# RishWijewardhena/vision-textile-inspection

Measured on AMD Instinct MI355X. Metric: frames/sec whole-node, YOLOv8n-seg 640x640 bs=64; mask IoU vs CPU ref, higher is better.
Workload: dtype f16x2

## Files before the change

include/vti.h:

```cpp
#ifndef VTI_H
#define VTI_H

#include <stddef.h>
#include <stdint.h>

#ifdef __cplusplus
extern "C" {
#endif

typedef struct vti_ctx vti_ctx;

typedef enum {
    VTI_OK = 0,
    VTI_ERR_ARG = -1,
    VTI_ERR_STATE = -2,
    VTI_ERR_WEIGHTS = -3,
    VTI_ERR_HIP = -4,
    VTI_ERR_NOMEM = -5,
    VTI_ERR_UNSUPPORTED = -6
} vti_status;

enum { VTI_F16 = 0, VTI_F32 = 1, VTI_H2 = 2 };
enum { VTI_MASK_LOGIT = 0,
       VTI_MASK_SIGMOID = 1 };
enum { VTI_PACK_U8 = 0, VTI_PACK_BITS = 1 };
#define VTI_MASK_NATIVE 0x10
#define VTI_MASK_SLOTS_PER_FRAME 512

typedef struct {
    char scale;
    int32_t nc;
    int32_t nm;
    int32_t reg_max;
    int32_t H, W;
    int32_t max_batch;
    int32_t dtype;
} vti_desc;

typedef struct {
    char name[48];
    int32_t c1, c2, k, s, kind;
    int32_t h_in, w_in, h_out, w_out;
    int64_t macs;
    int32_t tile_h, tile_w;
    int32_t waves_n, nrep;
    int32_t lds_bytes;
    int32_t fused;
    int32_t persistent;
} vti_conv_info;

int32_t vti_create(const vti_desc* desc, vti_ctx** out);
void vti_destroy(vti_ctx* ctx);
const char* vti_last_error(const vti_ctx* ctx);

int32_t vti_num_convs(const vti_ctx* ctx);
int32_t vti_conv_at(const vti_ctx* ctx, int32_t i, vti_conv_info* out);
int32_t vti_num_anchors(const vti_ctx* ctx);
int64_t vti_fused_params(const vti_ctx* ctx);
int64_t vti_macs_per_frame(const vti_ctx* ctx);
int64_t vti_workspace_bytes(const vti_ctx* ctx);
int32_t vti_num_launches(const vti_ctx* ctx);

int32_t vti_load_weights(vti_ctx* ctx, const void* host_blob, size_t nbytes, int32_t device);
int32_t vti_set_workspace(vti_ctx* ctx, void* dev_ws, size_t nbytes);

int32_t vti_letterbox(vti_ctx* ctx, const uint8_t* dev_frames, int32_t B, int32_t H0, int32_t W0,
                      uint8_t* dev_input, void* stream);
int32_t vti_forward(vti_ctx* ctx, const uint8_t* dev_input, int32_t B, int32_t swap_rb,
                    float* dev_pred, void* dev_proto, void* stream);
int32_t vti_nms(vti_ctx* ctx, const float* dev_pred, int32_t B, float conf, double iou,
                int32_t max_det, int32_t agnostic, float* dev_dets, int32_t* dev_counts, void* stream);
int32_t vti_forward_scored(vti_ctx* ctx, const uint8_t* dev_input, int32_t B, int32_t swap_rb,
                           float* dev_pred, void* dev_proto, float* dev_anchor_best, void* stream);
int32_t vti_nms_scored(vti_ctx* ctx, const float* dev_pred, const float* dev_anchor_best, int32_t B, float conf, double iou,
                       int32_t max_det, int32_t agnostic, float* dev_dets, int32_t* dev_counts, void* stream);
int32_t vti_masks(vti_ctx* ctx, const float* dev_dets, const int32_t* dev_counts, const void* dev_proto,
                  int32_t B, int32_t max_det, int32_t mode, int32_t packing,
                  uint8_t* dev_masks, int32_t capacity, int32_t* dev_offsets, void* stream);
int32_t vti_masks_native(vti_ctx* ctx, const float* dev_dets, const float* dev_xyxy, const int32_t* dev_counts,
                         const void* dev_proto, int32_t B, int32_t max_det, int32_t H0, int32_t W0, int32_t mode,
                         int32_t packing, uint8_t* dev_masks, int32_t capacity, int32_t* dev_offsets, void* stream);
int32_t vti_mask_native_layout(const vti_ctx* ctx, int32_t H0, int32_t W0, int32_t packing, int32_t out[6]);
int32_t vti_scale_boxes(vti_ctx* ctx, const float* dev_dets, const int32_t* dev_counts, int32_t B,
                        int32_t max_det, int32_t H0, int32_t W0, float* dev_xyxy, void* stream);
int32_t vti_predict(vti_ctx* ctx, const uint8_t* dev_frames, int32_t B, int32_t H0, int32_t W0,
                    int32_t swap_rb, float conf, double iou, int32_t max_det, int32_t agnostic,
                    int32_t mask_mode, int32_t packing, uint8_t* dev_input_scratch,
                    float* dev_pred, void* dev_proto, float* dev_dets, int32_t* dev_counts,
                    uint8_t* dev_masks, int32_t capacity, int32_t* dev_offsets, float* dev_xyxy,
                    void* stream);

int32_t vti_mask_to_frame(vti_ctx* ctx, const uint8_t* dev_masks, int32_t n, int32_t H, int32_t W,
                          int32_t H0, int32_t W0, uint8_t* dev_bitmaps, int32_t* dev_nonzero, void* stream);
int32_t vti_union_envelope(vti_ctx* ctx, const uint8_t* dev_bitmaps, const int32_t* dev_select, int32_t nsel,
                           int32_t H0, int32_t W0, uint8_t* dev_union, int32_t* dev_envelope, void* stream);
int32_t vti_mask_stats(vti_ctx* ctx, const uint8_t* dev_bitmaps, int32_t n, int32_t H0, int32_t W0,
                       int64_t* dev_stats, void* stream);

int32_t vti_mask_stats_bits(vti_ctx* ctx, const uint8_t* dev_masks_bits, int32_t n, const int32_t* dev_n_live,
                            int32_t H, int32_t W, int32_t H0, int32_t W0, int64_t* dev_stats, void* stream);
int32_t vti_envelope_bits(vti_ctx* ctx, const uint8_t* dev_masks_bits, const int32_t* dev_offsets, const float* dev_dets,
// ... 85 lines not shown
enum { VTI_POLY_OK = 0,
       VTI_POLY_ERR_BOUND = 1,
       VTI_POLY_ERR_RANGE = 2 };
int64_t vti_mask_polygons_scratch_bytes(const vti_ctx* ctx, int32_t H, int32_t W, int32_t row_bytes);
int32_t vti_mask_polygons(vti_ctx* ctx, const uint8_t* dev_masks_bits, int32_t n, const int32_t* dev_n_live, int32_t H, int32_t W,
                          int32_t row_bytes, int32_t H0, int32_t W0, int32_t strategy, void* dev_scratch, size_t scratch_bytes,
                          int32_t* dev_point_offsets, float* dev_points, int64_t max_points, void* stream);

enum { VTI_ANNOTATE_OUTLINE_SKIPPED = 1 };
int64_t vti_annotate_scratch_bytes(const vti_ctx* ctx, int32_t n_sel, int32_t max_det, int32_t H0, int32_t W0, int32_t max_points);
int32_t vti_annotate(vti_ctx* ctx, const uint8_t* dev_frames, int32_t B, int32_t H0, int32_t W0, const void* dev_cameras,
                     int32_t n_cams, const int32_t* dev_camera_of_frame, const uint8_t* dev_masks, int32_t native,
                     const float* dev_dets, const float* dev_xyxy, const int32_t* dev_counts, const int32_t* dev_offsets,
                     int32_t max_det, int32_t capacity, const int32_t* frame_i32, const double* stitch_f64, const int32_t* stitch_i32,
                     const int32_t* host_select, const int32_t* dev_select, int32_t n_sel, int32_t max_points, uint8_t* dev_out,
                     int32_t* dev_status, void* dev_scratch, size_t scratch_bytes, void* stream);
int64_t vti_annotate_frames_scratch_bytes(const vti_ctx* ctx, const void* host_out_table, int32_t max_det, int32_t max_points);
int32_t vti_annotate_frames(vti_ctx* ctx, const uint8_t* dev_frames, const void* host_table, const void* dev_table, int32_t B,
                            const void* dev_cameras, int32_t n_cams, const int32_t* dev_camera_of_frame, const uint8_t* dev_masks,
                            int32_t native, const float* dev_dets, const float* dev_xyxy, const int32_t* dev_counts,
                            const int32_t* dev_offsets, int32_t max_det, int32_t capacity, const int32_t* frame_i32,
                            const double* stitch_f64, const int32_t* stitch_i32, const int32_t* host_select, const int32_t* dev_select,
                            int32_t n_sel, int32_t max_points, const void* host_out_table, const void* dev_out_table, uint8_t* dev_out,
                            int32_t* dev_status, void* dev_scratch, size_t scratch_bytes, void* stream);

int64_t vti_encode_jpeg_scratch_bytes(const vti_ctx* ctx, int32_t n, int32_t H0, int32_t W0);
int64_t vti_encode_jpeg_max_bytes(int32_t n, int32_t H0, int32_t W0);
int32_t vti_encode_jpeg(vti_ctx* ctx, const uint8_t* dev_frames, int32_t n, int32_t H0, int32_t W0, int32_t rgb, int32_t quality,
                        void* dev_scratch, size_t scratch_bytes, int64_t* dev_byte_offsets, uint8_t* dev_out, int64_t max_bytes,
                        void* stream);
int64_t vti_encode_jpeg_frames_scratch_bytes(const vti_ctx* ctx, const void* host_table);
int64_t vti_encode_jpeg_frames_max_bytes(const void* host_table);
int32_t vti_encode_jpeg_frames(vti_ctx* ctx, const uint8_t* dev_frames, const void* host_table, const void* dev_table, int32_t n,
                               int32_t rgb, int32_t quality, void* dev_scratch, size_t scratch_bytes, int64_t* dev_byte_offsets,
                               uint8_t* dev_out, int64_t max_bytes, void* stream);

int64_t vti_decode_jpeg_table_bytes(int32_t n);
int32_t vti_decode_jpeg_plan(vti_ctx* ctx, const uint8_t* host_files, const int64_t* host_file_offsets, int32_t n,
                             int32_t segment_bytes, int32_t layout, void* host_table, size_t nbytes, int32_t* out_H0,
                             int32_t* out_W0, int64_t* out_byte_offsets, int64_t* out_scratch_bytes);
enum { VTI_JPEG_CORRUPT = 1 };
int32_t vti_decode_jpeg(vti_ctx* ctx, const uint8_t* dev_files, const void* host_table, const void* dev_table, int32_t n, int32_t rgb,
                        uint8_t* dev_out, int64_t out_bytes, int32_t* dev_info, void* dev_scratch, size_t scratch_bytes, void* stream);

int32_t vti_debug_conv_output(vti_ctx* ctx, int32_t i, int32_t B, float* dev_out, void* stream);

int32_t vti_debug_conv2d(int32_t dtype, const void* dev_in, int32_t B, int32_t H, int32_t W, int32_t in_ld,
                         int32_t in_coff, int32_t c1, const float* host_w, const float* host_b, int32_t c2,
                         int32_t k, int32_t s, int32_t kind, const void* dev_res, int32_t res_ld, int32_t res_coff,
                         void* dev_out, int32_t out_ld, int32_t out_coff, int32_t out_f32, int32_t swap_rb,
                         int32_t tile_h, int32_t tile_w, int32_t waves_n, int32_t nrep, int32_t iters,
                         float* ms_out, int32_t* cfg_out, void* stream);

#ifdef __cplusplus
}
#endif
#endif
```

vision-textile-inspection_amd/_lib.py:

```python
import ctypes as C
import os

_HERE = os.path.dirname(os.path.abspath(__file__))
_VARIANT = os.environ.get("VTI_LIB_VARIANT", "")
LIB_PATH = os.path.join(_HERE, f"libvti_{_VARIANT}.so" if _VARIANT else "libvti.so")

VTI_F16, VTI_F32, VTI_H2 = 0, 1, 2
VTI_MASK_LOGIT, VTI_MASK_SIGMOID = 0, 1
VTI_PACK_U8, VTI_PACK_BITS = 0, 1
VTI_MASK_NATIVE = 0x10


class VtiDesc(C.Structure):
    _fields_ = [("scale", C.c_char), ("nc", C.c_int32), ("nm", C.c_int32), ("reg_max", C.c_int32),
                ("H", C.c_int32), ("W", C.c_int32), ("max_batch", C.c_int32), ("dtype", C.c_int32)]


class VtiConvInfo(C.Structure):
    _fields_ = [("name", C.c_char * 48), ("c1", C.c_int32), ("c2", C.c_int32), ("k", C.c_int32),
                ("s", C.c_int32), ("kind", C.c_int32), ("h_in", C.c_int32), ("w_in", C.c_int32),
                ("h_out", C.c_int32), ("w_out", C.c_int32), ("macs", C.c_int64),
                ("tile_h", C.c_int32), ("tile_w", C.c_int32), ("waves_n", C.c_int32), ("nrep", C.c_int32),
                ("lds_bytes", C.c_int32), ("fused", C.c_int32), ("persistent", C.c_int32)]


class VtiMeasureParams(C.Structure):
    _fields_ = [("K", C.c_double * 9), ("dist", C.c_double * 5), ("R", C.c_double * 9), ("t", C.c_double * 3),
                ("max_px_distance", C.c_double), ("two_row_threshold_px", C.c_double),
                ("stitch_id", C.c_int32), ("fabric_id", C.c_int32), ("roi_enabled", C.c_int32), ("roi", C.c_int32 * 4),
                ("min_stitches", C.c_int32), ("envelope_neighborhood", C.c_int32), ("skip_cluster", C.c_int32),
                ("kmeans_iters", C.c_int32), ("drop_empty", C.c_int32), ("frame_buffer", C.c_int32)]


VTI_MEASURE_OK, VTI_MEASURE_NO_FABRIC, VTI_MEASURE_NO_STITCHES, VTI_MEASURE_BAD_CAMERA = 0, 1, 2, 3
VTI_STITCH_KEPT, VTI_STITCH_MASK, VTI_STITCH_SELECTED, VTI_STITCH_NEAR, VTI_STITCH_DIST, VTI_STITCH_WIDTH = 1, 2, 4, 8, 16, 32
VTI_MEASURE_MAX_DET = 1000

VTI_POLY_LARGEST, VTI_POLY_CONCAT = 0, 1
VTI_POLY_OK, VTI_POLY_ERR_BOUND, VTI_POLY_ERR_RANGE = 0, 1, 2
VTI_ANNOTATE_OUTLINE_SKIPPED = 1
VTI_JPEG_CORRUPT = 1
VTI_ERR_ARG, VTI_ERR_UNSUPPORTED = -1, -6


class VtiError(RuntimeError):

    def __init__(self, code, msg):
        super().__init__(f"libvti error {code}: {msg}")
        self.code = code


_P, _I32, _I64, _F, _D, _SZ = C.c_void_p, C.c_int32, C.c_int64, C.c_float, C.c_double, C.c_size_t

SIGNATURES = {
    "vti_create": (_I32, [C.POINTER(VtiDesc), C.POINTER(_P)]),
    "vti_destroy": (None, [_P]),
    "vti_last_error": (C.c_char_p, [_P]),
    "vti_num_convs": (_I32, [_P]),
    "vti_conv_at": (_I32, [_P, _I32, C.POINTER(VtiConvInfo)]),
    "vti_num_anchors": (_I32, [_P]),
    "vti_fused_params": (_I64, [_P]),
    "vti_macs_per_frame": (_I64, [_P]),
    "vti_workspace_bytes": (_I64, [_P]),
    "vti_num_launches": (_I32, [_P]),
    "vti_load_weights": (_I32, [_P, _P, _SZ, _I32]),
    "vti_set_workspace": (_I32, [_P, _P, _SZ]),
    "vti_letterbox": (_I32, [_P, _P, _I32, _I32, _I32, _P, _P]),
    "vti_forward": (_I32, [_P, _P, _I32, _I32, _P, _P, _P]),
    "vti_nms": (_I32, [_P, _P, _I32, _F, _D, _I32, _I32, _P, _P, _P]),
    "vti_forward_scored": (_I32, [_P, _P, _I32, _I32, _P, _P, _P, _P]),
    "vti_nms_scored": (_I32, [_P, _P, _P, _I32, _F, _D, _I32, _I32, _P, _P, _P]),
    "vti_masks": (_I32, [_P, _P, _P, _P, _I32, _I32, _I32, _I32, _P, _I32, _P, _P]),
    "vti_masks_native": (_I32, [_P, _P, _P, _P, _P, _I32, _I32, _I32, _I32, _I32, _I32, _P, _I32, _P, _P]),
    "vti_mask_native_layout": (_I32, [_P, _I32, _I32, _I32, C.POINTER(_I32)]),
    "vti_scale_boxes": (_I32, [_P, _P, _P, _I32, _I32, _I32, _I32, _P, _P]),
    "vti_predict": (_I32, [_P, _P, _I32, _I32, _I32, _I32, _F, _D, _I32, _I32, _I32, _I32,
                           _P, _P, _P, _P, _P, _P, _I32, _P, _P, _P]),
    "vti_mask_to_frame": (_I32, [_P, _P, _I32, _I32, _I32, _I32, _I32, _P, _P, _P]),
    "vti_union_envelope": (_I32, [_P, _P, _P, _I32, _I32, _I32, _P, _P, _P]),
    "vti_mask_stats": (_I32, [_P, _P, _I32, _I32, _I32, _P, _P]),
    "vti_mask_stats_bits": (_I32, [_P, _P, _I32, _P, _I32, _I32, _I32, _I32, _P, _P]),
    "vti_envelope_bits": (_I32, [_P, _P, _P, _P, _I32, _I32, _I32, _I32, _I32, _I32, _P, _P]),
    "vti_pixels_to_world": (_I32, [_P, _P, _I32, _P, _P, _P, _P, _P, _P, _P]),
    "vti_kmeans1d2": (_I32, [_P, _P, _P, _I32, _I32, _I32, _P, _P, _P]),
    "vti_measure_scratch_bytes": (_I64, [_P, _I32, _I32, _I32]),
    "vti_measure": (_I32, [_P, C.POINTER(VtiMeasureParams), _P, _I32, _P, _P, _P, _P, _I32, _I32, _I32, _I32, _I32, _P, _SZ,
                           _P, _P, _P, _P, _P]),
    "vti_measure_cameras_bytes": (_I64, [_I32]),
    "vti_measure_pack_cameras": (_I32, [_P, C.POINTER(VtiMeasureParams), _I32, _P, _SZ]),
    "vti_measure_cameras": (_I32, [_P, _P, _I32, _P, _P, _I32, _P, _P, _P, _P, _I32, _I32, _I32, _I32, _I32, _P, _SZ,
                                   _P, _P, _P, _P, _P]),
    "vti_frame_table_bytes": (_I64, [_I32]),
    "vti_pack_frames": (_I32, [_P, _I32, _I32, _P, _P, _P, _I32, _I64, _P, _SZ]),
    "vti_frame_table_info": (_I32, [_P, _I32, _P, _P]),
    "vti_letterbox_frames": (_I32, [_P, _P, _P, _P, _I32, _P, _P]),
    "vti_scale_boxes_frames": (_I32, [_P, _P, _P, _P, _P, _I32, _I32, _P, _P]),
    "vti_predict_frames": (_I32, [_P, _P, _P, _P, _I32, _I32, _F, _D, _I32, _I32, _I32, _I32,
                                  _P, _P, _P, _P, _P, _P, _I32, _P, _P, _P]),
    "vti_measure_frames": (_I32, [_P, _P, _I32, _P, _P, _I32, _P, _P, _P, _P, _P, _P, _I32, _I32, _I32, _P, _SZ,
                                  _P, _P, _P, _P, _P]),
    "vti_mask_native_frames_bytes": (_I64, [_P, _P, _I32]),
    "vti_masks_native_frames": (_I32, [_P, _P, _P, _P, _P, _P, _P, _I32, _I32, _I32, _I32, _P, _I64, _P, _P, _P]),
    "vti_predict_frames_native": (_I32, [_P, _P, _P, _P, _I32, _I32, _F, _D, _I32, _I32, _I32, _I32,
                                         _P, _P, _P, _P, _P, _P, _I64, _P, _P, _P, _P]),
    "vti_measure_frames_native": (_I32, [_P, _P, _I32, _P, _P, _P, _I64, _P, _P, _P, _P, _P, _P, _I32, _I32, _I32, _P, _SZ,
                                         _P, _P, _P, _P, _P]),
    "vti_mask_polygons_scratch_bytes": (_I64, [_P, _I32, _I32, _I32]),
    "vti_mask_polygons": (_I32, [_P, _P, _I32, _P, _I32, _I32, _I32, _I32, _I32, _I32, _P, _SZ, _P, _P, _I64, _P]),
    "vti_annotate_scratch_bytes": (_I64, [_P, _I32, _I32, _I32, _I32, _I32]),
    "vti_annotate": (_I32, [_P, _P, _I32, _I32, _I32, _P, _I32, _P, _P, _I32, _P, _P, _P, _P, _I32, _I32, _P, _P, _P, _P, _P, _I32,
                            _I32, _P, _P, _P, _SZ, _P]),
    "vti_annotate_frames_scratch_bytes": (_I64, [_P, _P, _I32, _I32]),
    "vti_annotate_frames": (_I32, [_P, _P, _P, _P, _I32, _P, _I32, _P, _P, _I32, _P, _P, _P, _P, _I32, _I32, _P, _P, _P, _P, _P, _I32,
                                   _I32, _P, _P, _P, _P, _P, _SZ, _P]),
    "vti_encode_jpeg_scratch_bytes": (_I64, [_P, _I32, _I32, _I32]),
    "vti_encode_jpeg_max_bytes": (_I64, [_I32, _I32, _I32]),
    "vti_encode_jpeg": (_I32, [_P, _P, _I32, _I32, _I32, _I32, _I32, _P, _SZ, _P, _P, _I64, _P]),
    "vti_encode_jpeg_frames_scratch_bytes": (_I64, [_P, _P]),
    "vti_encode_jpeg_frames_max_bytes": (_I64, [_P]),
    "vti_encode_jpeg_frames": (_I32, [_P, _P, _P, _P, _I32, _I32, _I32, _P, _SZ, _P, _P, _I64, _P]),
    "vti_decode_jpeg_table_bytes": (_I64, [_I32]),
    "vti_decode_jpeg_plan": (_I32, [_P, _P, _P, _I32, _I32, _I32, _P, _SZ, _P, _P, _P, _P]),
    "vti_decode_jpeg": (_I32, [_P, _P, _P, _P, _I32, _I32, _P, _I64, _P, _P, _SZ, _P]),
    "vti_debug_conv_output": (_I32, [_P, _I32, _I32, _P, _P]),
    "vti_debug_conv2d": (_I32, [_I32, _P, _I32, _I32, _I32, _I32, _I32, _I32, _P, _P, _I32, _I32, _I32, _I32,
                                _P, _I32, _I32, _P, _I32, _I32, _I32, _I32, _I32, _I32, _I32, _I32, _I32,
                                _P, _P, _P]),
}

_lib = None


def lib():
    global _lib
    if _lib is None:
        if not os.path.exists(LIB_PATH):
            raise ImportError(f"{LIB_PATH} not found: build it with `python -c 'import __graft_entry__ as g; "
                              f"g.build()'` (hipcc --offload-arch=gfx950); there is no CPU fallback")
        L = C.CDLL(LIB_PATH)
        for name, (res, args) in SIGNATURES.items():
            fn = getattr(L, name)
            fn.restype, fn.argtypes = res, args
        _lib = L
    return _lib


def check(ctx, rc):
    if rc != 0:
        msg = lib().vti_last_error(ctx)
        raise VtiError(rc, msg.decode() if msg else "")
```

vision-textile-inspection_amd/api.py:

```python
from ._lib import LIB_PATH, SIGNATURES, VtiError, lib
from .engine import Engine, FrameTable, debug_conv2d, h2_decode, h2_encode, kmeans1d2, pixels_to_world, unpack_bits
from .feeder import FrameFeeder
from .model import YOLO, Boxes, Masks, Results, letterbox_shape
from .weights import pack_container, random_weights, unpack_container
from .convert import convert_checkpoint, convert_state_dict
from .measure import MeasureParams, MultiCameraMeasurer, StitchMeasurer
from . import annotate, consumer, dataparallel, jpeg

__all__ = ["LIB_PATH", "SIGNATURES", "VtiError", "lib", "Engine", "FrameTable", "debug_conv2d", "h2_decode", "h2_encode", "kmeans1d2", "pixels_to_world", "unpack_bits", "FrameFeeder", "YOLO", "Boxes", "Masks",
           "Results", "letterbox_shape", "pack_container", "random_weights", "unpack_container", "convert_checkpoint", "convert_state_dict",
           "MeasureParams", "MultiCameraMeasurer", "StitchMeasurer", "annotate", "consumer", "dataparallel", "jpeg"]
```

vision-textile-inspection_amd/csrc/conv.hip:

```cpp
#include <algorithm>
#include <cstdlib>
#include <type_traits>

#include "conv_dev.h"

namespace vti {

__host__ __device__ inline int patch_dim(int t, int ks, int s, int mode) { return mode == 1 ? t : (t - 1) * s + ks; }

size_t stem_lds_bytes(int TH, int TW);

size_t conv_lds_bytes(int ks, int stride, int mode, int TH, int TW, int WN, int NREP) {
    if (mode == 1) return stem_lds_bytes(TH, TW);
    const int npix = patch_dim(TH, ks, stride, mode) * patch_dim(TW, ks, stride, mode);
    const size_t plane = (size_t)((npix + 15) & ~15) * 16;
    const int taps = mode == 1 ? 1 : ks * ks;
    size_t raw = 0;
    if (mode == 1) raw = (((size_t)(2 * TH + 1) * (2 * TW + 1) * 3) + 15) & ~(size_t)15;
    return 4 * plane + (size_t)WN * NREP * taps * 1024 + raw;
}

template <typename T, int KS, int S, int NREP, int WN, int NREP2 = 0, int NT = 256>
__global__ __launch_bounds__(NT, NT == 512 ? 1 : 2) void conv_kernel(const ConvParams p) {
    using vec = typename Tr<T>::vec;
    constexpr int VEC = Tr<T>::VEC, KC = Tr<T>::KC;
    constexpr int TAPS = KS * KS, PAD = KS / 2;
    constexpr int NTB = WN * NREP;
    constexpr int PP = NT / 4;
    constexpr int AR = NT == 512 ? 6 : (S == 2 ? 12 : 8);
    constexpr int BR = (NTB * TAPS * 64 + NT - 1) / NT;
    constexpr unsigned OOB = 0xFFFFFFFFu;
    extern __shared__ __attribute__((aligned(16))) char smem[];

    const int tid = threadIdx.x, lane = tid & 63, wave = tid >> 6;
    const int wn = wave % WN, wm = wave / WN;
    int t = blockIdx.x;
    const int tx = t % p.tiles_x; t /= p.tiles_x;
    const int ty = t % p.tiles_y;
    const int b = t / p.tiles_y;
    const int oy0 = ty * p.TH, ox0 = tx * p.TW;
    const int PH = (p.TH - 1) * S + KS, PW = (p.TW - 1) * S + KS;
    const int npix = PH * PW;
    const int plane_bytes = ((npix + 15) & ~15) * 16;
    char* smA = smem;
    char* smB = smem + 4 * plane_bytes;
    const int nt0 = blockIdx.y * NTB;
    const int tile_px = p.TH * p.TW;
    VTI_STAMP(0);

    int abase[MREP], opy[MREP], opx[MREP];
    bool pvalid[MREP];
#pragma unroll
    for (int m = 0; m < MREP; ++m) {
        const int pp = (wm * MREP + m) * 16 + (lane & 15);
        const bool v = pp < tile_px;
        const int pc = v ? pp : 0;
        const int py = (int)__umulhi((unsigned)pc, p.tw_magic), px = pc - py * p.TW;
        opy[m] = oy0 + py; opx[m] = ox0 + px;
        pvalid[m] = v && opy[m] < p.Hout && opx[m] < p.Wout;
        abase[m] = (lane >> 4) * plane_bytes + ((py * S) * PW + px * S) * 16;
    }

    f32x4 acc[MREP][NREP];
#pragma unroll
    for (int m = 0; m < MREP; ++m)
#pragma unroll
        for (int n = 0; n < NREP; ++n) acc[m][n] = (f32x4){0.f, 0.f, 0.f, 0.f};

    const size_t frame_elems = (size_t)p.Hin * p.Win * p.in_ld;
    const __amdgpu_buffer_rsrc_t rsA = __builtin_amdgcn_make_buffer_rsrc(
        (void*)((const T*)p.in + (size_t)b * frame_elems), 0, (int)(frame_elems * sizeof(T)), 0x00020000);
    const __amdgpu_buffer_rsrc_t rsB = __builtin_amdgcn_make_buffer_rsrc((void*)p.wpk, 0, (int)p.wpk_bytes, 0x00020000);

    const int iy0 = oy0 * S - PAD, ix0 = ox0 * S - PAD;
    const int q = (tid >> 3) & 3;
    const int pix0 = (tid >> 5) * 8 + (tid & 7);
    const int ldsA0 = q * plane_bytes + pix0 * 16;
    const int cvalid = (p.Cin - q * VEC + KC - 1) / KC;
    unsigned aoff[AR];
#pragma unroll
    for (int u = 0; u < AR; ++u) {
        const int pix = pix0 + PP * u;
        const int py = (int)__umulhi((unsigned)pix, p.pw_magic), px = pix - py * PW;
        const int y = iy0 + py, x = ix0 + px;
        const bool ok = pix < npix && (unsigned)y < (unsigned)p.Hin && (unsigned)x < (unsigned)p.Win;
        aoff[u] = ok ? (unsigned)(((y * p.Win + x) * p.in_ld + p.in_coff + q * VEC) * (int)sizeof(T)) : OOB;
    }
    constexpr bool BPRE = NREP < 5 || NT == 512;
    constexpr int PD = (KS == 1 && BPRE) ? 2 : 1;
    vec ra[PD][AR], rb[PD][BR];
    auto loadB = [&](int c, vec (&rbs)[BR]) {
        const unsigned sB = (unsigned)(((size_t)c * p.ntiles_n + nt0) * (TAPS * 1024));
#pragma unroll
        for (int u = 0; u < BR; ++u)
            if (tid + u * NT < NTB * TAPS * 64) rbs[u] = buf_load16<vec>(rsB, (unsigned)(tid + u * NT) * 16u, sB);
    };
    auto issue = [&](int c, vec (&ras)[AR], vec (&rbs)[BR]) {
        const bool qok = c < cvalid;
#pragma unroll
        for (int u = 0; u < AR; ++u)
            if (pix0 + PP * u < ((npix + 7) & ~7))
                ras[u] = buf_load16<vec>(rsA, qok ? aoff[u] : OOB, (unsigned)(c * KC * (int)sizeof(T)));
        if constexpr (BPRE) loadB(c, rbs);
    };
    auto commit = [&](int c, vec (&ras)[AR], vec (&rbs)[BR]) {
        if constexpr (!BPRE) loadB(c, rbs);
#pragma unroll
        for (int u = 0; u < AR; ++u)
            if (pix0 + PP * u < npix) *(vec*)(smA + ldsA0 + u * (PP * 16)) = ras[u];
#pragma unroll
        for (int u = 0; u < BR; ++u)
            if (tid + u * NT < NTB * TAPS * 64) *(vec*)(smB + (tid + u * NT) * 16) = rbs[u];
    };
    auto chunk = [&](int c, auto set_c) {
        constexpr int SET = decltype(set_c)::value;
        if (c < 2) VTI_STAMP(1 + 5 * c);
        commit(c, ra[SET], rb[SET]);
        if (c < 2) VTI_STAMP(3 + 5 * c);
        __syncthreads();
        if (c < 2) VTI_STAMP(4 + 5 * c);
        if (c + PD < p.nchunks) issue(c + PD, ra[SET], rb[SET]);
        {
            constexpr int NSTEP = TAPS * MREP;
            constexpr int XD = NREP >= 5 ? 2 : 3;
            constexpr int WD = NREP >= 5 ? 1 : 2;
            vec xq[XD];
            vec wq[WD][NREP];
            auto ldx = [&](int s_) -> vec {
                const int tp = s_ / MREP, mm = s_ % MREP;
                const int toff = ((tp / KS) * PW + (tp % KS)) * 16;
                return *(const vec*)(smA + abase[mm] + toff);
            };
            auto ldw = [&](int tp, vec (&w)[NREP]) {
#pragma unroll
                for (int n = 0; n < NREP; ++n)
                    w[n] = *(const vec*)(smB + ((wn * NREP + n) * TAPS + tp) * 1024 + lane * 16);
            };
            if constexpr (Tr<T>::H2 && TAPS > 1 && (NREP <= 3 || (NREP == 4 && NT == 512))) {
                auto ldw1 = [&](int tp, int n) -> vec { return *(const vec*)(smB + ((wn * NREP + n) * TAPS + tp) * 1024 + lane * 16); };
                h2_taps<NREP, MREP, TAPS, 3>(acc, ldx, ldw1);
            } else {
            ldw(0, wq[0]);
            xq[0] = ldx(0);
            if (XD > 2 && NSTEP > 1) xq[1] = ldx(1);
#pragma unroll
            for (int s_ = 0; s_ < NSTEP; ++s_) {
                const int tp = s_ / MREP, mm = s_ % MREP;
                if (s_ + XD - 1 < NSTEP) xq[(s_ + XD - 1) % XD] = ldx(s_ + XD - 1);
                if (WD == 2 && mm == 0 && tp + 1 < TAPS) ldw(tp + 1, wq[(tp + 1) % WD]);
                __builtin_amdgcn_sched_barrier(0);
#pragma unroll
                for (int n = 0; n < NREP; ++n) acc[mm][n] = mma(wq[tp % WD][n], xq[s_ % XD], acc[mm][n]);
                __builtin_amdgcn_sched_barrier(0);
                if (WD == 1 && mm == MREP - 1 && tp + 1 < TAPS) ldw(tp + 1, wq[0]);
            }
            }
        }
        if (c < 2) VTI_STAMP(5 + 5 * c);
        if (c + 1 < p.nchunks) __syncthreads();
    };

    issue(0, ra[0], rb[0]);
    if constexpr (PD == 2) {
        if (p.nchunks > 1) issue(1, ra[1], rb[1]);
        for (int c = 0; c < p.nchunks; c += 2) {
            chunk(c, std::integral_constant<int, 0>{});
            if (c + 1 < p.nchunks) chunk(c + 1, std::integral_constant<int, 1>{});
        }
    } else {
        for (int c = 0; c < p.nchunks; ++c) chunk(c, std::integral_constant<int, 0>{});
    }

    VTI_STAMP(11);
    if constexpr (NREP2 == 0) {
        conv_epilogue<T, NREP>(p, acc, pvalid, opy, opx, b, nt0, wn, lane);
    } else {
        static_assert(WN == 1, "fused stage needs the whole Cout in one wave");
        conv_stage2<T, NREP, NREP2>(p, acc, pvalid, opy, opx, b, lane);
    }
    VTI_STAMP(12);
}

size_t convfold_lds_bytes(int TH, int TW) {
    const int npix = (TH + 2) * (TW + 2);
    return 4 * (size_t)((npix + 15) & ~15) * 16 + (size_t)16 * 4 * 1024;
}
bool convfold_supported(int c_in, int c_mid, int c_out, int ntiles2) {
    return c_in == c_mid && c_mid % 16 == 0 && c_out == 64 && c_in % 16 == 0 && c_in <= 64 && combo_has(FoldN2{}, ntiles2);
}

template <typename T, int NREP2, int NT = 256>
__global__ __launch_bounds__(NT, NT == 512 ? 1 : 2) void convfold_kernel(const ConvParams p) {
    using vec = typename Tr<T>::vec;
    constexpr int VEC = Tr<T>::VEC, KC = Tr<T>::KC;
    constexpr int NREP = 4, TAPS = 4, NTB = 16, AR = 8;
    constexpr int BR = NTB * TAPS * 64 / NT;
    constexpr int PPP = NT / 4;
    constexpr unsigned OOB = 0xFFFFFFFFu;
    extern __shared__ __attribute__((aligned(16))) char smem[];

    const int tid = threadIdx.x, lane = tid & 63, wave = (tid >> 6) & 3, mgrp = tid >> 8;
    const int py = wave >> 1, px = wave & 1;
    int t = blockIdx.x;
    const int tx = t % p.tiles_x; t /= p.tiles_x;
    const int ty = t % p.tiles_y;
    const int b = t / p.tiles_y;
    const int oy0 = ty * p.TH, ox0 = tx * p.TW;
    const int PH = p.TH + 2, PW = p.TW + 2;
    const int npix = PH * PW;
    const int plane_bytes = ((npix + 15) & ~15) * 16;
    char* smA = smem;
    char* smB = smem + 4 * plane_bytes;
    const int tile_px = p.TH * p.TW;

    int abase[MREP], opy[MREP], opx[MREP];
    bool pvalid[MREP];
#pragma unroll
    for (int m = 0; m < MREP; ++m) {
        const int pp = (mgrp * MREP + m) * 16 + (lane & 15);
        const bool v = pp < tile_px;
        const int pc = v ? pp : 0;
        const int ly = (int)__umulhi((unsigned)pc, p.tw_magic), lx = pc - ly * p.TW;
        pvalid[m] = v && oy0 + ly < p.Hout && ox0 + lx < p.Wout;
        opy[m] = 2 * (oy0 + ly) + py; opx[m] = 2 * (ox0 + lx) + px;
        abase[m] = (lane >> 4) * plane_bytes + ((ly + py) * PW + lx + px) * 16;
    }
    f32x4 acc[MREP][NREP];
#pragma unroll
    for (int m = 0; m < MREP; ++m)
#pragma unroll
        for (int n = 0; n < NREP; ++n) acc[m][n] = (f32x4){0.f, 0.f, 0.f, 0.f};
// ... 424 lines not shown
        const int pp = (wave * MREP + m) * 16 + (lane & 15);
        const int py = pp / SL_TW, px = pp - py * SL_TW;
        opy[m] = oy0 + py; opx[m] = ox0 + px;
        pvalid[m] = opy[m] < p.Hout && opx[m] < p.Wout;
        sbase[m] = ((2 * py) * SL_SW + 2 * px) * 16 * ES;
    }
    f32x4 acc[MREP][2];
#pragma unroll
    for (int m = 0; m < MREP; ++m) { acc[m][0] = (f32x4){0.f, 0.f, 0.f, 0.f}; acc[m][1] = (f32x4){0.f, 0.f, 0.f, 0.f}; }
#pragma unroll
    for (int s = 0; s < NS1; ++s) {
        const int tap = sizeof(T) == 2 ? 2 * s + (g >> 1) : s;
        const int tc = tap < 9 ? tap : 8;
        const int toff = ((tc / 3) * SL_SW + (tc % 3)) * 16 * ES + (sizeof(T) == 2 ? (g & 1) * 8 : g * 4) * ES;
        vec w1[2];
#pragma unroll
        for (int n = 0; n < 2; ++n) w1[n] = w1all[s][n];
#pragma unroll
        for (int m = 0; m < MREP; ++m) {
            const vec x = *(const vec*)(sout + sbase[m] + toff);
#pragma unroll
            for (int n = 0; n < 2; ++n) acc[m][n] = mma(w1[n], x, acc[m][n]);
        }
    }
    VTI_STAMP(3);
    if (p.out2) conv_stage2<T, 2, 2, false, true>(p, acc, pvalid, opy, opx, b, lane, &s2r);
    else conv_epilogue<T, 2>(p, acc, pvalid, opy, opx, b, 0, 0, lane);
    VTI_STAMP(12);
    }
}

void stem_l1_tile(int* th, int* tw) { *th = SL_TH; *tw = SL_TW; }

int stem_l1_grid(int dtype, int ntiles) {
    const int wgpc = (int)std::min<size_t>(2, (160 * 1024) / stem_l1_lds_bytes(dtype));
    const char* np = getenv("VTI_STEM_NOT_PERSISTENT");
    if (np && np[0] == '1') return ntiles;
    return std::min(ntiles, 256 * std::max(1, wgpc));
}

hipError_t launch_stem_l1(int dtype, const ConvParams& p, hipStream_t st) {
    dim3 grid((unsigned)stem_l1_grid(dtype, p.B * p.tiles_y * p.tiles_x));
    if (grid.x == 0) return hipSuccess;
    const size_t lds = stem_l1_lds_bytes(dtype);
    return with_conv_type(dtype, [&](auto t) { return launch_lds<stem_l1_kernel<typename decltype(t)::type>>(grid, dim3(256), lds, st, p); });
}

size_t stem_lds_bytes(int TH, int TW) { return 1024 + (size_t)(2 * TH + 1) * ((((2 * TW + 1) * 3 + 6) >> 2) * 4); }

using ConvTile3 = Combos<Ints<1, 1>, Ints<2, 1>, Ints<3, 1>, Ints<4, 1>, Ints<5, 1>, Ints<1, 2>, Ints<2, 2>, Ints<1, 4>>;
using ConvTile1 = decltype(concat(ConvTile3{}, Combos<Ints<3, 2>, Ints<4, 2>, Ints<5, 2>, Ints<2, 4>, Ints<3, 4>, Ints<4, 4>, Ints<5, 4>>{}));
using StemNrep = Combos<Ints<1>, Ints<2>, Ints<3>, Ints<4>, Ints<5>>;

bool conv_cfg_fits(int ks, int stride, int mode, int TH, int TW, int WN, int NREP, int threads) {
    if (mode == 1) return WN == 1 && (2 * TH + 1) * (((2 * TW + 1) * 3 + 6) >> 2) < 65536;
    if (threads != 256 && !(threads == 512 && ks == 3 && stride == 1 && WN == 1)) return false;
    const int AR = threads == 512 ? 6 : (stride == 2 ? 12 : 8);
    const int npix = patch_dim(TH, ks, stride, mode) * patch_dim(TW, ks, stride, mode);
    if (((npix + 7) / 8) * 32 > threads * AR) return false;
    return ks == 1 ? combo_has(ConvTile1{}, NREP, WN) : combo_has(ConvTile3{}, NREP, WN);
}

bool conv_fusable(int nrep, int nrep2) { return combo_has(FusedPairs{}, nrep, nrep2); }

template <typename T, int KS, int S>
static hipError_t launch_ks(int nrep, const ConvParams& p, dim3 grid, size_t lds, hipStream_t st) {
    return combo_dispatch(std::conditional_t<KS == 1, ConvTile1, ConvTile3>{}, [&](auto c) {
        using C = decltype(c);
        return launch_lds<conv_kernel<T, KS, S, C::v[0], C::v[1]>>(grid, dim3(256), lds, st, p);
    }, nrep, p.WN);
}

template <typename T>
static hipError_t launch_t(int ks, int stride, int nrep, int mode, const ConvParams& p, dim3 grid, size_t lds,
                           hipStream_t st) {
    if (p.ntiles2 > 0) {
        if (!(ks == 3 && stride == 1 && p.WN == 1 && mode == 0)) return hipErrorInvalidValue;
        return combo_dispatch(FusedPairs{}, [&](auto c) {
            using C = decltype(c);
            return p.nt == 512 ? launch_lds<conv_kernel<T, 3, 1, C::v[0], 1, C::v[1], 512>>(grid, dim3(512), lds, st, p)
                               : launch_lds<conv_kernel<T, 3, 1, C::v[0], 1, C::v[1]>>(grid, dim3(256), lds, st, p);
        }, nrep, p.ntiles2);
    }
    if (mode == 1)
        return combo_dispatch(StemNrep{}, [&](auto c) {
            hipLaunchKernelGGL((stem_kernel<T, decltype(c)::v[0]>), grid, dim3(256), lds, st, p);
            return hipGetLastError();
        }, nrep);
    if (ks == 1 && stride == 1) return launch_ks<T, 1, 1>(nrep, p, grid, lds, st);
    if (ks == 3 && stride == 1) return launch_ks<T, 3, 1>(nrep, p, grid, lds, st);
    if (ks == 3 && stride == 2) return launch_ks<T, 3, 2>(nrep, p, grid, lds, st);
    return hipErrorInvalidValue;
}

hipError_t launch_conv(int dtype, int ks, int stride, int nrep, int mode, const ConvParams& p, size_t lds_bytes,
                       hipStream_t st) {
    if (p.pk == 4) return launch_conv_pk2(dtype, nrep, p, lds_bytes, st);
    if (p.pk == 3) return launch_bneck_pk(dtype, nrep, p, lds_bytes, st);
    if (p.pk == 2) return launch_conv1_pk(dtype, nrep, p, lds_bytes, st);
    if (p.pk) return launch_conv_pk(dtype, nrep, p, lds_bytes, st);
    const int NTB = p.WN * nrep;
    dim3 grid((unsigned)(p.B * p.tiles_y * p.tiles_x), (unsigned)((p.ntiles_n + NTB - 1) / NTB));
    if (grid.x == 0) return hipSuccess;
    const int nwaves = p.nt == 512 ? 8 : 4;
    if ((p.nt != 256 && p.nt != 512) || (p.nt == 512 && p.ntiles2 == 0)) return hipErrorInvalidValue;
    if (p.TH * p.TW > (nwaves / p.WN) * MREP * 16 || (p.WN != 1 && p.WN != 2 && p.WN != 4)) return hipErrorInvalidValue;
    return with_conv_type(dtype, [&](auto t) { return launch_t<typename decltype(t)::type>(ks, stride, nrep, mode, p, grid, lds_bytes, st); });
}

}
```

vision-textile-inspection_amd/csrc/conv_dev.h:

```cpp
#pragma once
#include "vti_internal.h"

namespace vti {

typedef _Float16 half_t;
typedef _Float16 half8 __attribute__((ext_vector_type(8)));
typedef _Float16 half4 __attribute__((ext_vector_type(4)));
typedef float f32x4 __attribute__((ext_vector_type(4)));

typedef unsigned u32x4 __attribute__((ext_vector_type(4)));

struct h2_t { unsigned u; };
struct h2x4 { u32x4 u; };
constexpr float H2_SX = 16.0f;

template <typename T> struct Tr;
template <> struct Tr<half_t> { typedef half8 vec; static constexpr int VEC = 8, KC = 32; static constexpr bool H16 = true, F32 = false, H2 = false; };
template <> struct Tr<float> { typedef f32x4 vec; static constexpr int VEC = 4, KC = 16; static constexpr bool H16 = false, F32 = true, H2 = false; };
template <> struct Tr<h2_t> { typedef h2x4 vec; static constexpr int VEC = 4, KC = 16; static constexpr bool H16 = false, F32 = false, H2 = true; };

typedef _Float16 half2v __attribute__((ext_vector_type(2)));
__device__ __forceinline__ unsigned h2_enc(float v) {
    half2v p;
    p[0] = (half_t)__builtin_fmaf(v, H2_SX, 0.0f);
// ... 3 lines not shown
__device__ __forceinline__ float h2_dec(unsigned u) {
    const half2v p = __builtin_bit_cast(half2v, u);
    return ((float)p[0] + (float)p[1]) * (1.0f / H2_SX);
}
template <typename T> __device__ __forceinline__ T to_T(float v) {
    if constexpr (Tr<T>::H2) return h2_t{h2_enc(v)};
    else return (T)v;
}
template <typename T> __device__ __forceinline__ void vset(typename Tr<T>::vec& x, int j, T e) {
    if constexpr (Tr<T>::H2) x.u[j] = e.u;
    else x[j] = e;
}
template <typename T> __device__ __forceinline__ u32x4 pack4(f32x4 v) {
    if constexpr (Tr<T>::H2) return (u32x4){h2_enc(v[0]), h2_enc(v[1]), h2_enc(v[2]), h2_enc(v[3])};
    else return __builtin_bit_cast(u32x4, v);
}
template <typename T> __device__ __forceinline__ f32x4 unpack4(u32x4 u) {
    if constexpr (Tr<T>::H2) return (f32x4){h2_dec(u[0]), h2_dec(u[1]), h2_dec(u[2]), h2_dec(u[3])};
    else return __builtin_bit_cast(f32x4, u);
}
template <typename T> __device__ __forceinline__ f32x4 acc_bias(f32x4 acc, f32x4 bias, float alpha) {
    if constexpr (Tr<T>::H2) return acc * (f32x4){alpha, alpha, alpha, alpha} + bias;
    else return acc + bias;
}

__device__ __forceinline__ f32x4 mma(half8 w, half8 x, f32x4 c) {
    return __builtin_amdgcn_mfma_f32_16x16x32_f16(w, x, c, 0, 0, 0);
}
__device__ __forceinline__ f32x4 mma(f32x4 w, f32x4 x, f32x4 c) {
    c = __builtin_amdgcn_mfma_f32_16x16x4f32(w[0], x[0], c, 0, 0, 0);
    c = __builtin_amdgcn_mfma_f32_16x16x4f32(w[1], x[1], c, 0, 0, 0);
    c = __builtin_amdgcn_mfma_f32_16x16x4f32(w[2], x[2], c, 0, 0, 0);
    c = __builtin_amdgcn_mfma_f32_16x16x4f32(w[3], x[3], c, 0, 0, 0);
    return c;
}

__device__ __forceinline__ f32x4 mma(h2x4 w, h2x4 x, f32x4 c) {
    u32x4 wh, wl;
#pragma unroll
    for (int i = 0; i < 4; ++i) {
        wh[i] = __builtin_amdgcn_perm(w.u[i], w.u[i], 0x01000100u);
        wl[i] = w.u[i] >> 16;
    }
    const half8 xv = __builtin_bit_cast(half8, x.u);
    c = __builtin_amdgcn_mfma_f32_16x16x32_f16(__builtin_bit_cast(half8, wh), xv, c, 0, 0, 0);
    c = __builtin_amdgcn_mfma_f32_16x16x32_f16(__builtin_bit_cast(half8, wl), xv, c, 0, 0, 0);
    return c;
}

template <int NREP, int M, int TAPS, int XD, class LDX, class LDW>
__device__ __forceinline__ void h2_taps(f32x4 (&acc)[M][NREP], LDX ldx, LDW ldw) {
    constexpr int NSTEP = TAPS * M;
    constexpr unsigned SEL_H = 0x01000100u;
    h2x4 xq[XD];
    u32x4 wraw[NREP];
    u32x4 wh[2][NREP], wl[2][NREP];
#pragma unroll
    for (int n = 0; n < NREP; ++n) wraw[n] = ldw(0, n).u;
#pragma unroll
    for (int i = 0; i < XD - 1; ++i) xq[i] = ldx(i);
#pragma unroll
    for (int n = 0; n < NREP; ++n)
#pragma unroll
        for (int i = 0; i < 4; ++i) {
            wh[0][n][i] = __builtin_amdgcn_perm(wraw[n][i], wraw[n][i], SEL_H);
            wl[0][n][i] = wraw[n][i] >> 16;
        }
#pragma unroll
    for (int s_ = 0; s_ < NSTEP; ++s_) {
        const int tp = s_ / M, mm = s_ % M, cur = tp & 1, nxt = cur ^ 1;
#ifdef H2_EXP_NOXREAD
        if (s_ + XD - 1 < NSTEP && s_ < XD) xq[(s_ + XD - 1) % XD] = ldx(s_ + XD - 1);
#else
        if (s_ + XD - 1 < NSTEP) xq[(s_ + XD - 1) % XD] = ldx(s_ + XD - 1);
#endif
        if (mm == 0 && tp + 1 < TAPS) {
#pragma unroll
            for (int n = 0; n < NREP; ++n) wraw[n] = ldw(tp + 1, n).u;
        }
        __builtin_amdgcn_sched_barrier(0);
        const half8 xv = __builtin_bit_cast(half8, xq[s_ % XD].u);
#pragma unroll
        for (int j = 0; j < 2 * NREP; ++j) {
            const int n = j >> 1;
#ifdef H2_EXP_SKIP
            if (!((j & 1) && (tp & 1)))
#endif
            acc[mm][n] = __builtin_amdgcn_mfma_f32_16x16x32_f16(__builtin_bit_cast(half8, (j & 1) ? wl[cur][n] : wh[cur][n]), xv, acc[mm][n], 0, 0, 0);
            const int k = (mm - 1) * 2 * NREP + j;
#ifdef H2_EXP_NOPERM
            if (mm == 1 && j == 0 && tp + 1 < TAPS) {
#pragma unroll
                for (int n2 = 0; n2 < NREP; ++n2) { wh[nxt][n2] = wraw[n2]; wl[nxt][n2] = wraw[n2]; }
            }
            if (false) {
#else
            if (mm >= 1 && k < 8 * NREP && tp + 1 < TAPS) {
#endif
                const int pn = k >> 3, r = k & 7, i = r & 3;
                if (r < 4) wh[nxt][pn][i] = __builtin_amdgcn_perm(wraw[pn][i], wraw[pn][i], SEL_H);
                else wl[nxt][pn][i] = wraw[pn][i] >> 16;
                __builtin_amdgcn_sched_group_barrier(0x008, 1, 0);
                __builtin_amdgcn_sched_group_barrier(0x002, 1, 0);
            }
        }
        __builtin_amdgcn_sched_barrier(0);
    }
}

template <int NREP, int M, int TAPS, class LDX, class LDW>
__device__ __forceinline__ void h2_taps_nmajor(f32x4 (&acc)[M][NREP], LDX ldx, LDW ldw) {
    constexpr int NU = TAPS * NREP;
    h2x4 x[2][M];
    u32x4 wraw[2], wh[2], wl[2];
#pragma unroll
    for (int m = 0; m < M; ++m) x[0][m] = ldx(m);
    wraw[0] = ldw(0, 0).u;
    if (NU > 1) wraw[1] = ldw(1 / NREP, 1 % NREP).u;
#pragma unroll
    for (int i = 0; i < 4; ++i) { wh[0][i] = __builtin_amdgcn_perm(wraw[0][i], wraw[0][i], 0x01000100u); wl[0][i] = wraw[0][i] >> 16; }
#pragma unroll
    for (int u = 0; u < NU; ++u) {
        const int tp = u / NREP, n = u % NREP, cur = u & 1, nxt = cur ^ 1;
        if (n == NREP - 1 && tp + 1 < TAPS) {
#pragma unroll
            for (int m = 0; m < M; ++m) x[(tp + 1) & 1][m] = ldx((tp + 1) * M + m);
        }
        const u32x4 wnext = wraw[nxt];
        if (u + 2 < NU) wraw[cur] = ldw((u + 2) / NREP, (u + 2) % NREP).u;
        __builtin_amdgcn_sched_barrier(0);
#pragma unroll
        for (int j = 0; j < 2 * M; ++j) {
            const int m = j >> 1;
            acc[m][n] = __builtin_amdgcn_mfma_f32_16x16x32_f16(__builtin_bit_cast(half8, (j & 1) ? wl[cur] : wh[cur]),
                                                               __builtin_bit_cast(half8, x[tp & 1][m].u), acc[m][n], 0, 0, 0);
            if (j < 8 && u + 1 < NU) {
                const int i = j & 3;
                if (j < 4) wh[nxt][i] = __builtin_amdgcn_perm(wnext[i], wnext[i], 0x01000100u);
                else wl[nxt][i] = wnext[i] >> 16;
                __builtin_amdgcn_sched_group_barrier(0x008, 1, 0);
                __builtin_amdgcn_sched_group_barrier(0x002, 1, 0);
            }
        }
        __builtin_amdgcn_sched_barrier(0);
    }
}

template <bool FAST> __device__ __forceinline__ float silu(float x) {
    if constexpr (FAST) return x * __builtin_amdgcn_rcpf(1.0f + __builtin_amdgcn_exp2f(x * -1.4426950408889634f));
    else return x / (1.0f + expf(-x));
}

template <bool FAST> __device__ __forceinline__ f32x4 silu4(f32x4 x) {
    if constexpr (FAST) {
        const f32x4 y = x * (f32x4){-1.4426950408889634f, -1.4426950408889634f, -1.4426950408889634f, -1.4426950408889634f};
        f32x4 e;
#pragma unroll
        for (int j = 0; j < 4; ++j) e[j] = __builtin_amdgcn_exp2f(y[j]);
        e = e + (f32x4){1.0f, 1.0f, 1.0f, 1.0f};
#pragma unroll
        for (int j = 0; j < 4; ++j) e[j] = __builtin_amdgcn_rcpf(e[j]);
        return x * e;
    } else {
        f32x4 r;
#pragma unroll
        for (int j = 0; j < 4; ++j) r[j] = silu<false>(x[j]);
        return r;
    }
}

constexpr int MREP = 5;

#ifdef VTI_STAMPS
#define VTI_STAMP(i)                                                                              \
    do {                                                                                          \
        if (p.stamps && tid == 0) {                                                               \
            unsigned long long t_;                                                                \
            asm volatile("s_memtime %0\n\ts_waitcnt lgkmcnt(0)" : "=s"(t_)::"memory");            \
            p.stamps[(size_t)(blockIdx.y * gridDim.x + blockIdx.x) * 16 + (i)] = t_;              \
            if ((i) == 0 || (i) == 12) {                                                          \
                asm volatile("s_memrealtime %0\n\ts_waitcnt lgkmcnt(0)" : "=s"(t_)::"memory");    \
                p.stamps[(size_t)(blockIdx.y * gridDim.x + blockIdx.x) * 16 + ((i) == 0 ? 14 : 15)] = t_; \
            }                                                                                     \
        }                                                                                         \
    } while (0)
#else
#define VTI_STAMP(i) do { } while (0)
#endif

template <typename T, int NREP>
__device__ __forceinline__ void conv_epilogue(const ConvParams& p, f32x4 (&acc)[MREP][NREP], const bool (&pvalid)[MREP],
                                              const int (&opy)[MREP], const int (&opx)[MREP], int b, int nt0, int wn,
                                              int lane) {
    constexpr bool FAST = !Tr<T>::F32;
    const int crun = (nt0 + wn * NREP) * 16 + (lane >> 4) * 4 * NREP;
    f32x4 bias_r[NREP];
#pragma unroll
    for (int n = 0; n < NREP; ++n) {
        const int cb = crun + 4 * n < p.ntiles_n * 16 ? crun + 4 * n : 0;
        bias_r[n] = *(const f32x4*)(p.bias + cb);
    }
    if (!p.scalar_store && !p.out_f32 && !p.deconv_c) {
        const bool has_res = __builtin_amdgcn_readfirstlane(p.has_res) != 0;
#pragma unroll
        for (int m = 0; m < MREP; ++m) {
            if (!pvalid[m]) continue;
            const size_t opix = ((size_t)(b * p.Hout + opy[m])) * p.Wout + opx[m];
            T* op = (T*)p.out + opix * p.out_ld + p.out_coff + crun;
            f32x4 res_r[NREP];
            if (has_res) {
                const T* rp = (const T*)p.res + opix * p.res_ld + p.res_coff + crun;
#pragma unroll
                for (int n = 0; n < NREP; ++n) {
                    res_r[n] = (f32x4){0.f, 0.f, 0.f, 0.f};
                    if (crun + 4 * n < p.Cout) {
                        if constexpr (sizeof(T) == 2) {
                            const half4 r = *(const half4*)(rp + 4 * n);
#pragma unroll
                            for (int j = 0; j < 4; ++j) res_r[n][j] = (float)r[j];
                        } else {
                            res_r[n] = unpack4<T>(*(const u32x4*)(rp + 4 * n));
                        }
                    }
                }
            }
            f32x4 v[NREP];
#pragma unroll
            for (int n = 0; n < NREP; ++n) {
                v[n] = acc_bias<T>(acc[m][n], bias_r[n], p.alpha);
                if (p.act) v[n] = silu4<FAST>(v[n]);
                if (has_res) v[n] += res_r[n];
            }
            if constexpr (sizeof(T) == 2) {
                if constexpr (NREP % 2 == 0) {
#pragma unroll
                    for (int n = 0; n < NREP; n += 2) {
                        if (crun + 4 * n + 8 <= p.Cout) {
                            half8 hv;
#pragma unroll
                            for (int j = 0; j < 4; ++j) { hv[j] = (half_t)v[n][j]; hv[4 + j] = (half_t)v[n + 1][j]; }
                            *(half8*)(op + 4 * n) = hv;
                        } else if (crun + 4 * n + 4 <= p.Cout) {
                            half4 hv;
#pragma unroll
                            for (int j = 0; j < 4; ++j) hv[j] = (half_t)v[n][j];
                            *(half4*)(op + 4 * n) = hv;
                        }
                    }
                } else {
#pragma unroll
                    for (int n = 0; n < NREP; ++n) {
                        if (crun + 4 * n >= p.Cout) continue;
                        half4 hv;
#pragma unroll
                        for (int j = 0; j < 4; ++j) hv[j] = (half_t)v[n][j];
                        *(half4*)(op + 4 * n) = hv;
                    }
                }
            } else {
#pragma unroll
                for (int n = 0; n < NREP; ++n)
                    if (crun + 4 * n < p.Cout) *(u32x4*)(op + 4 * n) = pack4<T>(v[n]);
            }
        }
        return;
    }
    if constexpr (sizeof(T) == 2 && NREP % 2 == 0) {
        if (p.deconv_c && !p.scalar_store && !p.out_f32 && !p.has_res) {
            const int qd = crun / p.deconv_c, co = crun - qd * p.deconv_c;
#pragma unroll
            for (int m = 0; m < MREP; ++m) {
                if (!pvalid[m] || crun >= p.Cout) continue;
                const size_t opix = ((size_t)(b * 2 * p.Hout + 2 * opy[m] + (qd >> 1))) * (2 * p.Wout) + 2 * opx[m] + (qd & 1);
                T* op = (T*)p.out + opix * p.out_ld + p.out_coff + co;
#pragma unroll
                for (int n = 0; n < NREP; n += 2) {
                    half8 hv;
#pragma unroll
                    for (int j = 0; j < 4; ++j) {
                        float a0 = acc[m][n][j] + bias_r[n][j], a1 = acc[m][n + 1][j] + bias_r[n + 1][j];
                        if (p.act) { a0 = silu<FAST>(a0); a1 = silu<FAST>(a1); }
                        hv[j] = (half_t)a0; hv[4 + j] = (half_t)a1;
                    }
                    *(half8*)(op + 4 * n) = hv;
                }
            }
            return;
        }
    }
#pragma unroll
    for (int m = 0; m < MREP; ++m) {
        if (!pvalid[m]) continue;
#pragma unroll
        for (int n = 0; n < NREP; ++n) {
            const int cout0 = crun + 4 * n;
            if (cout0 >= p.Cout) continue;
            f32x4 v = acc_bias<T>(acc[m][n], bias_r[n], p.alpha);
            if (p.act) v = silu4<FAST>(v);
            size_t opix;
            int co = cout0;
            if (p.deconv_c) {
                const int q = cout0 / p.deconv_c;
                co = cout0 - q * p.deconv_c;
                opix = ((size_t)(b * 2 * p.Hout + 2 * opy[m] + (q >> 1))) * (2 * p.Wout) + 2 * opx[m] + (q & 1);
            } else {
                opix = ((size_t)(b * p.Hout + opy[m])) * p.Wout + opx[m];
            }
            if (p.has_res) {
                const T* rp = (const T*)p.res + opix * p.res_ld + p.res_coff + co;
                if constexpr (sizeof(T) == 2) {
                    const half4 r = *(const half4*)rp;
#pragma unroll
                    for (int j = 0; j < 4; ++j) v[j] += (float)r[j];
                } else {
                    v += unpack4<T>(*(const u32x4*)rp);
                }
            }
            const size_t o = opix * p.out_ld + p.out_coff + co;
            if (p.scalar_store) {
#pragma unroll
                for (int j = 0; j < 4; ++j) {
                    if (cout0 + j < p.Cout) {
                        if (p.out_f32) ((float*)p.out)[o + j] = v[j];
                        else if constexpr (Tr<T>::H2) ((unsigned*)p.out)[o + j] = h2_enc(v[j]);
                        else ((T*)p.out)[o + j] = (T)v[j];
                    }
                }
            } else if (p.out_f32 || Tr<T>::F32) {
                *(f32x4*)((float*)p.out + o) = v;
            } else if constexpr (Tr<T>::H2) {
                *(u32x4*)((unsigned*)p.out + o) = pack4<T>(v);
            } else {
                half4 hv;
#pragma unroll
                for (int j = 0; j < 4; ++j) hv[j] = (half_t)v[j];
                *(half4*)((half_t*)p.out + o) = hv;
            }
        }
    }
}

template <typename V> __device__ __forceinline__ V buf_load16(__amdgpu_buffer_rsrc_t r, unsigned voff, unsigned soff) {
    const u32x4 v = __builtin_amdgcn_raw_buffer_load_b128(r, voff, soff, 0);
    return __builtin_bit_cast(V, v);
}

template <typename T, int NREP, int NREP2> struct Stage2Regs {
    using vec = typename Tr<T>::vec;
    static constexpr int KT = sizeof(T) == 2 ? (NREP + 1) / 2 : NREP;
    vec w2[KT][NREP2];
    f32x4 bias1[NREP];
    f32x4 bias2[NREP2];
};

template <typename T, int NREP, int NREP2>
__device__ __forceinline__ void stage2_preload(const ConvParams& p, int lane, bool fold, Stage2Regs<T, NREP, NREP2>& r) {
    using vec = typename Tr<T>::vec;
    const __amdgpu_buffer_rsrc_t rsW2 = __builtin_amdgcn_make_buffer_rsrc(
        (void*)p.w2, 0, (int)(Stage2Regs<T, NREP, NREP2>::KT * p.ntiles2 * 1024), 0x00020000);
#pragma unroll
    for (int t2 = 0; t2 < Stage2Regs<T, NREP, NREP2>::KT; ++t2)
#pragma unroll
        for (int n = 0; n < NREP2; ++n) r.w2[t2][n] = buf_load16<vec>(rsW2, (unsigned)(((t2 * p.ntiles2 + n) * 64 + lane) * 16), 0u);
    const float* b1 = p.bias + (fold ? 4 * (16 * NREP) : 0) + (lane >> 4) * 4 * NREP;
#pragma unroll
    for (int n = 0; n < NREP; ++n) r.bias1[n] = *(const f32x4*)(b1 + 4 * n);
    const int crun2 = p.nat2 ? (lane >> 4) * 4 : (lane >> 4) * 4 * NREP2, cstep2 = p.nat2 ? 16 : 4;
#pragma unroll
    for (int n = 0; n < NREP2; ++n) r.bias2[n] = *(const f32x4*)(p.bias2 + crun2 + cstep2 * n);
}

template <typename T, int NREP, int NREP2, bool FOLD = false, bool PRE = false>
__device__ __forceinline__ void conv_stage2(const ConvParams& p, f32x4 (&acc)[MREP][NREP], const bool (&pvalid)[MREP],
                                            const int (&opy)[MREP], const int (&opx)[MREP], int b, int lane,
                                            const Stage2Regs<T, NREP, NREP2>* pre = nullptr, bool interior = false) {
    const int OW = FOLD ? 2 * p.Wout : p.Wout;
    using vec = typename Tr<T>::vec;
    constexpr bool FAST = !Tr<T>::F32;
    constexpr int KT = sizeof(T) == 2 ? (NREP + 1) / 2 : NREP;
    const __amdgpu_buffer_rsrc_t rsW2 = __builtin_amdgcn_make_buffer_rsrc(
        (void*)p.w2, 0, (int)(KT * p.ntiles2 * 1024), 0x00020000);
    f32x4 bias1[FOLD ? MREP : 1][NREP];
    if (PRE && (!FOLD || interior)) {
#pragma unroll
        for (int m = 0; m < (FOLD ? MREP : 1); ++m)
#pragma unroll
            for (int n = 0; n < NREP; ++n) bias1[m][n] = pre->bias1[n];
    } else if constexpr (FOLD) {
#pragma unroll
        for (int m = 0; m < MREP; ++m) {
            const int cy = opy[m] == 0 ? 0 : (opy[m] == 2 * p.Hout - 1 ? 2 : 1), cx = opx[m] == 0 ? 0 : (opx[m] == OW - 1 ? 2 : 1);
            const float* bt = p.bias + (cy * 3 + cx) * (16 * NREP) + (lane >> 4) * 4 * NREP;
#pragma unroll
            for (int n = 0; n < NREP; ++n) bias1[m][n] = *(const f32x4*)(bt + 4 * n);
        }
    } else {
#pragma unroll
        for (int n = 0; n < NREP; ++n) bias1[0][n] = *(const f32x4*)(p.bias + (lane >> 4) * 4 * NREP + 4 * n);
    }
    f32x4 acc2[MREP][NREP2];
#pragma unroll
    for (int m = 0; m < MREP; ++m)
#pragma unroll
        for (int n = 0; n < NREP2; ++n) acc2[m][n] = (f32x4){0.f, 0.f, 0.f, 0.f};
#pragma unroll
    for (int t2 = 0; t2 < KT; ++t2) {
        vec w2[NREP2];
#pragma unroll
        for (int n = 0; n < NREP2; ++n) {
            if constexpr (PRE) w2[n] = pre->w2[t2][n];
            else w2[n] = buf_load16<vec>(rsW2, (unsigned)(((t2 * p.ntiles2 + n) * 64 + lane) * 16), 0u);
        }
#pragma unroll
        for (int m = 0; m < MREP; ++m) {
            vec x;
            if constexpr (sizeof(T) == 2) {
#pragma unroll
                for (int h = 0; h < 2; ++h) {
                    const int n1 = 2 * t2 + h;
                    f32x4 v = {0.f, 0.f, 0.f, 0.f};
                    if (n1 < NREP) {
                        v = acc_bias<T>(acc[m][n1 < NREP ? n1 : 0], bias1[FOLD ? m : 0][n1 < NREP ? n1 : 0], p.alpha);
                        if (p.act) v = silu4<FAST>(v);
                    }
#pragma unroll
                    for (int j = 0; j < 4; ++j) x[h * 4 + j] = (T)v[j];
                }
            } else {
                f32x4 v = acc_bias<T>(acc[m][t2], bias1[FOLD ? m : 0][t2], p.alpha);
                if (p.act) v = silu4<FAST>(v);
                if constexpr (Tr<T>::H2) x.u = pack4<T>(v);
                else {
#pragma unroll
                    for (int j = 0; j < 4; ++j) x[j] = v[j];
                }
            }
#pragma unroll
            for (int n = 0; n < NREP2; ++n) acc2[m][n] = mma(w2[n], x, acc2[m][n]);
        }
    }
    [[maybe_unused]] const int tid = threadIdx.x;
    VTI_STAMP(13);
    f32x4 bias2[NREP2];
    const int crun2 = p.nat2 ? (lane >> 4) * 4 : (lane >> 4) * 4 * NREP2;
    const int cstep2 = p.nat2 ? 16 : 4;
#pragma unroll
    for (int n = 0; n < NREP2; ++n) {
        if constexpr (PRE) bias2[n] = pre->bias2[n];
        else bias2[n] = *(const f32x4*)(p.bias2 + crun2 + cstep2 * n);
    }
    if constexpr (NREP2 == 4) {
        if (p.act2 == 3) {
            const int g = lane >> 4;
#pragma unroll
            for (int m = 0; m < MREP; ++m) {
                float d4[4];
#pragma unroll
                for (int n = 0; n < 4; ++n) {
                    const f32x4 v = acc_bias<T>(acc2[m][n], bias2[n], p.alpha2);
                    float mx = fmaxf(fmaxf(v[0], v[1]), fmaxf(v[2], v[3]));
                    mx = fmaxf(mx, __shfl_xor(mx, 16));
                    mx = fmaxf(mx, __shfl_xor(mx, 32));
                    float e[4];
#pragma unroll
                    for (int j = 0; j < 4; ++j) {
                        if constexpr (FAST) e[j] = __builtin_amdgcn_exp2f((v[j] - mx) * 1.4426950408889634f);
                        else e[j] = expf(v[j] - mx);
                    }
                    float s = (e[0] + e[1]) + (e[2] + e[3]);
                    float w = (e[0] * (float)(4 * g) + e[1] * (float)(4 * g + 1)) + (e[2] * (float)(4 * g + 2) + e[3] * (float)(4 * g + 3));
                    s += __shfl_xor(s, 16); w += __shfl_xor(w, 16);
                    s += __shfl_xor(s, 32); w += __shfl_xor(w, 32);
                    d4[n] = w / s;
                }
                const float ax = (float)opx[m] + 0.5f, ay = (float)opy[m] + 0.5f;
                const float x1 = ax - d4[0], y1 = ay - d4[1], x2 = ax + d4[2], y2 = ay + d4[3];
                const float comp = g == 0 ? ((x1 + x2) / 2.0f) * p.dfl_stride : g == 1 ? ((y1 + y2) / 2.0f) * p.dfl_stride
                                 : g == 2 ? (x2 - x1) * p.dfl_stride : (y2 - y1) * p.dfl_stride;
                if (pvalid[m])
                    ((float*)p.out2)[((size_t)b * p.out2_bstride + (size_t)opy[m] * OW + opx[m]) * p.out2_ld + p.out2_coff + g] = comp;
            }
            return;
        }
    }
    if constexpr (sizeof(T) == 2 && NREP2 % 2 == 0) {
        if (!p.nat2 && !p.out2_f32 && !p.scalar_store2 && (p.Cout2 & 7) == 0 && ((p.out2_ld | p.out2_coff) & 7) == 0) {
#pragma unroll
            for (int m = 0; m < MREP; ++m) {
                if (!pvalid[m]) continue;
                half_t* op = (half_t*)p.out2 + ((size_t)b * p.out2_bstride + (size_t)opy[m] * OW + opx[m]) * p.out2_ld + p.out2_coff + crun2;
#pragma unroll
                for (int n = 0; n < NREP2; n += 2) {
                    if (crun2 + 4 * n >= p.Cout2) continue;
                    f32x4 v0 = acc_bias<T>(acc2[m][n], bias2[n], p.alpha2), v1 = acc_bias<T>(acc2[m][n + 1], bias2[n + 1], p.alpha2);
                    if (p.act2 == 1) { v0 = silu4<FAST>(v0); v1 = silu4<FAST>(v1); }
                    half8 hv;
#pragma unroll
                    for (int j = 0; j < 4; ++j) { hv[j] = (half_t)v0[j]; hv[4 + j] = (half_t)v1[j]; }
                    *(half8*)(op + 4 * n) = hv;
                }
            }
            return;
        }
    }
    const bool want_best = p.act2 == 2 && p.best != nullptr;
#pragma unroll
    for (int m = 0; m < MREP; ++m) {
        const size_t pix = (size_t)b * p.out2_bstride + (size_t)opy[m] * OW + opx[m];
        const size_t o0 = pix * p.out2_ld + p.out2_coff;
        float bv = -INFINITY;
        int bc = 0x7fffffff;
        if (!want_best && !pvalid[m]) continue;
#pragma unroll
        for (int n = 0; n < NREP2; ++n) {
            const int cout0 = crun2 + cstep2 * n;
            if (cout0 >= p.Cout2) continue;
            f32x4 v = acc_bias<T>(acc2[m][n], bias2[n], p.alpha2);
            if (p.act2 == 1) v = silu4<FAST>(v);
            else if (p.act2 == 2) {
#pragma unroll
                for (int j = 0; j < 4; ++j) {
                    if constexpr (FAST) v[j] = __builtin_amdgcn_rcpf(1.0f + __builtin_amdgcn_exp2f(v[j] * -1.4426950408889634f));
                    else v[j] = 1.0f / (1.0f + expf(-v[j]));
                }
                if (want_best) {
                    if ((p.Cout2 & 3) == 0) {
#pragma unroll
                        for (int j = 0; j < 4; ++j)
                            if (v[j] > bv) { bv = v[j]; bc = cout0 + j; }
                    } else {
#pragma unroll
                        for (int j = 0; j < 4; ++j)
                            if (cout0 + j < p.Cout2 && v[j] > bv) { bv = v[j]; bc = cout0 + j; }
                    }
                }
            }
            if (!pvalid[m]) continue;
            const size_t o = o0 + cout0;
            if (p.scalar_store2) {
#pragma unroll
                for (int j = 0; j < 4; ++j) {
                    if (cout0 + j < p.Cout2) {
                        if (p.out2_f32) ((float*)p.out2)[o + j] = v[j];
                        else if constexpr (Tr<T>::H2) ((unsigned*)p.out2)[o + j] = h2_enc(v[j]);
                        else ((T*)p.out2)[o + j] = (T)v[j];
                    }
                }
            } else if (p.out2_f32 || Tr<T>::F32) {
                *(f32x4*)((float*)p.out2 + o) = v;
            } else if constexpr (Tr<T>::H2) {
                *(u32x4*)((unsigned*)p.out2 + o) = pack4<T>(v);
            } else {
                half4 hv;
#pragma unroll
                for (int j = 0; j < 4; ++j) hv[j] = (half_t)v[j];
                *(half4*)((half_t*)p.out2 + o) = hv;
            }
        }
        if (want_best) {
#pragma unroll
// ... 34 lines not shown
```

vision-textile-inspection_amd/csrc/plan.cpp:

```cpp
#include <algorithm>
#include <cmath>
#include <cstdio>
#include <cstdlib>
#include <cstring>

#include "vti_internal.h"

namespace vti {

namespace {

struct Scale { char tag; double depth, width; int maxc; };
const Scale kScales[] = {{'n', 0.33, 0.25, 1024}, {'s', 0.33, 0.50, 1024}, {'m', 0.67, 0.75, 768},
                         {'l', 1.00, 1.00, 512},  {'x', 1.00, 1.25, 512}};

int make_divisible(double x, int d) { return (int)std::ceil(x / d) * d; }
int py_round(double x) { return (int)std::nearbyint(x); }

struct Builder {
    Plan& P;
    int maxB;
    std::vector<Op>* cur;
    int lane = 0;
    explicit Builder(Plan& p) : P(p), maxB(p.desc.max_batch), cur(&p.ops) {}
// ... 194 lines not shown
    const long total_px = (long)max_batch * (deconv ? r.h_in * r.w_in : r.h_out * r.w_out);
    double best = 1e30;
    bool found = false;
    for (int WN = 1; WN <= 4; WN *= 2) {
        if (fwn && WN != fwn) continue;
        for (int NREP = 1; NREP <= 5; ++NREP) {
            if (fnrep && NREP != fnrep) continue;
            if (!conv1_pk_instantiated(NREP, WN)) continue;
            if (deconv && r.c2 % (16 * NREP)) continue;
            const int NTB = WN * NREP;
            const int gy = (c.ntiles_n + NTB - 1) / NTB;
            const double n_eff = (double)c.ntiles_n / (gy * NTB);
            if (n_eff < 0.74 && !fnrep) continue;
            for (int nwm = 1; nwm <= 4; ++nwm) {
                if (fth && nwm != fth) continue;
                const int ncomp = nwm * WN;
                if (ncomp > 4) continue;
                static const size_t wstat_max = getenv("VTI_PK1_WSTAT_KB") ? (size_t)atoi(getenv("VTI_PK1_WSTAT_KB")) * 1024 : 96 * 1024;
                const int wstat = (size_t)c.nchunks * NTB * 1024 <= wstat_max ? 1 : 0;
                static const bool no_w2 = getenv("VTI_PK1_NO_WGPC2") && getenv("VTI_PK1_NO_WGPC2")[0] == '1';
                static const bool force_w2 = getenv("VTI_PK1_FORCE_WGPC2") && getenv("VTI_PK1_FORCE_WGPC2")[0] == '1';
                for (int wgpc = (esize == 4 && force_w2) ? 2 : 1; wgpc <= ((esize == 4 && !no_w2) ? 2 : 1); ++wgpc) {
                    int depth = 0;
                    for (int dd = 8; dd >= 2; --dd)
                        if (conv1_pk_fits(nwm, WN, NREP, c.nchunks, dd, wstat, cps) &&
                            conv1_pk_lds_bytes(nwm, WN, NREP, c.nchunks, dd, wstat, cps) <= (size_t)(160 * 1024) / wgpc) { depth = dd; break; }
                    if (!depth) continue;
                    const long NT = (total_px + nwm * 80 - 1) / (nwm * 80);
                    const long G = pk_grid(NT, wgpc, gy);
                    const long rounds = (NT + G - 1) / G;
                    const double solo = esize == 4 ? ((ncomp * wgpc > 4) ? 1.1 : 1.45) : 1.0;
                    const double step_cyc = 5.0 * NREP * 16 * solo * (esize == 4 ? 2.0 : 1.0) + 250.0 / cps;
                    const double t_comp = rounds * (c.nchunks * step_cyc + 1100.0 * NREP) * ((ncomp * wgpc + 3) / 4) / 1.9e9;
                    const double bytes = (double)total_px * ((double)gy * r.c1 + (double)c.gemm_n) * esize +
                                         (wstat ? 0.0 : (double)NT * gy * c.nchunks * NTB * 1024 * 0.25);
                    const double inflight = (double)wgpc * (depth - 1) * nwm * 80 * 64 * cps;
                    static const double inflight_full = getenv("VTI_PK1_INFLIGHT_KB") ? atof(getenv("VTI_PK1_INFLIGHT_KB")) * 1e3 : 50e3;
                    const double t_mem = bytes / (5.0e12 * std::min(1.0, inflight / inflight_full));
                    const double cost = std::max(t_comp, t_mem) + 0.15 * std::min(t_comp, t_mem) + 4e-6;
                    if (cost < best) {
                        best = cost; found = true;
                        c.TH = nwm; c.TW = 80; c.WN = WN; c.NREP = NREP; c.pk = 2; c.pk_wgpc = wgpc; c.pk_depth = depth; c.pk_wstat = wstat; c.pk_cps = cps;
                        c.lds = conv1_pk_lds_bytes(nwm, WN, NREP, c.nchunks, depth, wstat, cps);
                    }
                }
            }
        }
    }
    if (found) c.ntiles_n = (c.ntiles_n + c.WN * c.NREP - 1) / (c.WN * c.NREP) * (c.WN * c.NREP);
    return found;
}

void choose_conv_cfg(int dtype, const ConvRow& r, bool conv0, int max_batch, ConvCfg& c, int fth, int ftw, int fwn,
                     int fnrep, bool allow_pk) {
    const bool f16 = dtype == VTI_F16;
    const int KC = f16 ? 32 : 16;
    const bool deconv = r.kind == 2;
    c.gemm_n = deconv ? 4 * r.c2 : r.c2;
    c.ntiles_n = (c.gemm_n + 15) / 16;
    c.nchunks = conv0 ? (32 / KC) : (r.c1 + KC - 1) / KC;
    c.pk = 0;
    if (allow_pk && !conv0 && (!ftw || ftw == 80) && (!fth || fth <= 4) && choose_pk1_cfg(f16 ? 2 : 4, r, max_batch, c, fth, fwn, fnrep)) return;
    c.pk_wstat = 0;
    if (allow_pk && !conv0 && (!ftw || ftw == 20) && (!fth || fth % 4 == 0) && choose_pk_cfg(dtype, r, max_batch, c, fth, fwn, fnrep)) {
        return;
    }
    if (allow_pk && !conv0 && (!ftw || ftw == 20) && (!fth || fth % 4 == 0) && choose_pk2_cfg(dtype, r, max_batch, c, fth, fwn, fnrep)) return;
    const int ks = deconv ? 1 : r.k, st = deconv ? 1 : r.s;
    const int Ho = deconv ? r.h_in : r.h_out, Wo = deconv ? r.w_in : r.w_out;
    c.TH = c.TW = 0;

    double best = -1;
    for (int WN = 1; WN <= 4; WN *= 2) {
        if (fwn && WN != fwn) continue;
        for (int NREP = 1; NREP <= 5; ++NREP) {
            if (fnrep && NREP != fnrep) continue;
            if (deconv && r.c2 % (16 * NREP)) continue;
            const int BN = WN * NREP;
            const int gy = (c.ntiles_n + BN - 1) / BN;
            const double n_eff = (double)c.ntiles_n / (gy * BN);
            if (n_eff < 0.74 && !fnrep) continue;
            const int BM = (4 / WN) * 80;
            for (int TW = std::min(Wo, BM); TW >= 1; --TW) {
                if (ftw && TW != ftw) continue;
                int TH = std::min(Ho, BM / TW);
                if (fth) { if (fth * TW > BM) continue; TH = fth; }
                if (TH < 1) continue;
                const int tiles = ((Ho + TH - 1) / TH) * ((Wo + TW - 1) / TW);
                const double m_eff = (double)Ho * Wo / ((double)tiles * BM);
                const int PH = conv0 ? TH : (TH - 1) * st + ks, PW = conv0 ? TW : (TW - 1) * st + ks;
                const size_t lds = conv_lds_bytes(ks, st, conv0 ? 1 : 0, TH, TW, WN, NREP);
                if (lds > ((fth || ftw) ? 160u : 80u) * 1024) continue;
                if (!conv_cfg_fits(ks, st, conv0 ? 1 : 0, TH, TW, WN, NREP)) continue;
                const double halo = conv0 ? (double)(4 * TH * TW) / ((2 * TH + 1) * (2 * TW + 1))
                                          : (double)(TH * TW * st * st) / (PH * PW);
                const double lds_traffic = 1.0 / NREP + 1.0 / 5;
                const double rowb = std::min(1.0, (double)TW * 64.0 / 1024.0);
                double score = m_eff * n_eff * (0.6 + 0.4 * halo) * (0.8 + 0.2 * rowb) / (0.35 + lds_traffic);
                if (lds > 64 * 1024) score *= 0.9;
                if (ks == 1 && WN >= 2) score *= 1.12;
                const double wgs = (double)tiles * gy * max_batch;
                if (wgs < 512) score *= 0.5 + 0.5 * wgs / 512;
                if (score > best) {
                    best = score;
                    c.TH = TH; c.TW = TW; c.WN = WN; c.NREP = NREP; c.lds = lds;
                }
            }
        }
    }
    if (c.TH) c.ntiles_n = (c.ntiles_n + c.NREP - 1) / c.NREP * c.NREP;
}

std::string Plan::build(const vti_desc& d) {
    desc = d;
    const Scale* sc = nullptr;
    for (const Scale& s : kScales) if (s.tag == d.scale) sc = &s;
    if (!sc) return "unknown scale (expected one of n,s,m,l,x)";
    if (d.nc < 1 || d.nm < 1 || d.reg_max < 1 || d.nm % 4 || d.nm > 64) return "bad nc/nm/reg_max";
    if (d.reg_max != 16) return "only reg_max=16 is supported";
    if (d.H < 32 || d.W < 32 || d.H % 32 || d.W % 32) return "H and W must be positive multiples of 32";
    if (d.max_batch < 1) return "max_batch must be >= 1";
    if (d.dtype != VTI_F16 && d.dtype != VTI_F32 && d.dtype != VTI_H2) return "dtype must be VTI_F16, VTI_F32 or VTI_H2";
    esize = d.dtype == VTI_F16 ? 2 : 4;

    auto ch = [&](int c) { return make_divisible(std::min(c, sc->maxc) * sc->width, 8); };
    auto rep = [&](int n) { return std::max(py_round(n * sc->depth), 1); };
    const int c0 = ch(64), c1 = ch(128), c2 = ch(256), c3 = ch(512), c4 = ch(1024);
    const int r0 = rep(3), r1 = rep(6), r2 = rep(6), r3 = rep(3), rn = rep(3);
    const int npr = ch(256);
    const int c_box = std::max(std::max(16, c2 / 4), 4 * d.reg_max);
    const int c_cls = std::max(c2, std::min(d.nc, 100));
    const int c_mc = std::max(c2 / 4, d.nm);
    for (int c : {c0, c1, c2, c3, c4, npr, c_box, c_cls, c_mc})
        if (c % 16) return "channel count not a multiple of 16 for this scale";

    Builder b(*this);
    std::vector<Op> g_p3, g_proto, g_head[3], g_p4, g_p5;
    b.cur = &g_p3;
    const int H = d.H, W = d.W;
    const int in_u8 = b.new_buf(3, H, W, EL_U8);
    const int B0 = b.new_buf(c0, H / 2, W / 2);
    const int B1 = b.new_buf(c1, H / 4, W / 4);
    const int B2 = b.new_buf(c1, H / 4, W / 4);
    const int B3 = b.new_buf(c2, H / 8, W / 8);
    const int CAT14 = b.new_buf(c3 + c2, H / 8, W / 8);
    const int B5 = b.new_buf(c3, H / 16, W / 16);
    const int CAT11 = b.new_buf(c4 + c3, H / 16, W / 16);
    const int B7 = b.new_buf(c4, H / 32, W / 32);
    const int B8 = b.new_buf(c4, H / 32, W / 32);
    const int SP = b.new_buf(2 * c4, H / 32, W / 32);
    const int CAT20 = b.new_buf(c3 + c4, H / 32, W / 32);
    const int CAT17 = b.new_buf(c2 + c3, H / 16, W / 16);
    const int P3 = b.new_buf(c2, H / 8, W / 8);
    const int P4 = b.new_buf(c3, H / 16, W / 16);
    const int P5 = b.new_buf(c4, H / 32, W / 32);

    b.conv("model.0", b.whole(in_u8), b.whole(B0), 3, 2, 0);
    b.conv("model.1", b.whole(B0), b.whole(B1), 3, 2, 0);
// ... 258 lines not shown
                    op.pred_mode = 3; op.pred_cbase = 0; op.pred_a0 = a0[l]; op.dfl_stride = levels[l].stride;
                    conv_out[op.fused].buf = -1;
                }
                for (size_t i = 0; i < ops.size(); ++i)
                    if (ops[i].kind == OP_DECODE) { ops.erase(ops.begin() + i); break; }
            }
        }
    }

    macs = 0; fused_params = d.reg_max;
    size_t woff = 0, boff = 0;
    for (Op& op : ops) {
        if (op.kind != OP_CONV && op.kind != OP_CONV0) continue;
        const ConvRow& r = convs[op.conv];
        macs += r.macs(); fused_params += r.fused_params();
        size_t pk_limit = 0x80000000ull;
        if (const char* pl = getenv("VTI_PK_LIMIT_BYTES")) pk_limit = (size_t)atoll(pl);
        const bool pk_ok = bufs[op.in.buf].bytes < pk_limit && bufs[op.out.buf].bytes < pk_limit &&
                           (!op.has_res || bufs[op.res.buf].bytes < pk_limit);
        if (op.pair >= 0) {
            const ConvRow& rb = convs[op.pair];
            macs += rb.macs(); fused_params += rb.fused_params();
            const int KC = d.dtype == VTI_F16 ? 32 : 16;
            op.cfg = ConvCfg();
            const long tiles16 = (long)d.max_batch * ((r.h_out + 15) / 16) * ((r.w_out + 19) / 20);
            op.cfg.TH = tiles16 >= 256 ? 16 : 8; op.cfg.TW = 20; op.cfg.WN = 1; op.cfg.NREP = r.c2 / 16;
            op.cfg.nchunks = (r.c1 + KC - 1) / KC; op.cfg.gemm_n = r.c2; op.cfg.ntiles_n = r.c2 / 16;
            op.cfg.pk = 3; op.cfg.pk_wgpc = 1;
            op.cfg.pk_depth = bneck_pk_depth(op.cfg.TH, op.cfg.NREP);
            op.cfg.lds = bneck_pk_lds_bytes(op.cfg.TH, op.cfg.NREP, op.cfg.pk_depth);
            if (!bneck_pk_fits(op.cfg.TH, op.cfg.NREP) || op.cfg.nchunks != 1) return "no launch configuration for the fused bottleneck " + r.name;
        }
        else if (op.fold >= 0) {
            const ConvRow& ru = convs[op.fold];
            macs += ru.macs(); fused_params += ru.fused_params();
            const int KC = d.dtype == VTI_F16 ? 32 : 16;
            op.cfg = ConvCfg();
            op.cfg.TH = 4; op.cfg.TW = 20; op.cfg.WN = 4; op.cfg.NREP = r.c2 / 16;
            op.cfg.nchunks = (ru.c1 + KC - 1) / KC; op.cfg.gemm_n = 4 * r.c2; op.cfg.ntiles_n = 4 * (r.c2 / 16);
            const char* f8 = getenv("VTI_FOLD512");
            const char* nf8 = getenv("VTI_NO_FOLD512");
            const bool fold8 = f8 ? f8[0] == '1' : (d.dtype == VTI_H2 && !(nf8 && nf8[0] == '1'));
            if (d.dtype != VTI_F16 && fold8 && ru.h_in >= 8) { op.cfg.TH = 8; op.cfg.threads = 512; }
            op.cfg.lds = convfold_lds_bytes(op.cfg.TH, op.cfg.TW);
            const char* npf = getenv("VTI_NO_PK_FOLD");
            if (pk_ok && op.cfg.nchunks <= 2 && !(npf && npf[0] == '1')) { op.cfg.pk = 1; op.cfg.pk_wgpc = 1; op.cfg.pk_depth = conv_pk_fold_depth(op.cfg.nchunks);
                                                                          op.cfg.lds = conv_pk_fold_lds_bytes(op.cfg.nchunks, op.cfg.pk_depth); }
        }
        else if (op.fused_l1 >= 0) choose_conv_cfg(d.dtype, r, true, d.max_batch, op.cfg, 0, 0, 1, 1);
        else if (op.fused >= 0) {
            const char* pf = getenv("VTI_PK_FUSED");
            const bool pkf = pf ? (pf[0] == '1' || (pf[0] == '2' && r.c2 / 16 <= 4)) : (d.dtype == VTI_H2 && r.c2 / 16 == 4);
            choose_conv_cfg(d.dtype, r, false, d.max_batch, op.cfg, 0, 0, 1, r.c2 / 16, pk_ok && pkf);
            const char* n5 = getenv("VTI_NO_T512");
            if (!(n5 && n5[0] == '1') && !op.cfg.pk && op.cfg.TH && r.k == 3 && r.s == 1 && r.kind == 0) {
                const int TH = 16, TW = 40;
                const double eff_now = (double)r.h_out * r.w_out / ((double)((r.h_out + op.cfg.TH - 1) / op.cfg.TH) * ((r.w_out + op.cfg.TW - 1) / op.cfg.TW) * op.cfg.TH * op.cfg.TW);
                const double eff_512 = (double)r.h_out * r.w_out / ((double)((r.h_out + TH - 1) / TH) * ((r.w_out + TW - 1) / TW) * TH * TW);
                const size_t lds = conv_lds_bytes(3, 1, 0, TH, TW, 1, op.cfg.NREP);
                const size_t wgs = (size_t)((r.h_out + TH - 1) / TH) * ((r.w_out + TW - 1) / TW) * d.max_batch;
                if (eff_512 >= eff_now - 1e-9 && lds <= 160 * 1024 && wgs >= 512 && conv_cfg_fits(3, 1, 0, TH, TW, 1, op.cfg.NREP, 512)) {
                    op.cfg.TH = TH; op.cfg.TW = TW; op.cfg.threads = 512; op.cfg.lds = lds;
                }
            }
        }
        else choose_conv_cfg(d.dtype, r, op.kind == OP_CONV0, d.max_batch, op.cfg, 0, 0, 0, 0, pk_ok);
        if (op.cfg.TH == 0) return "no launch configuration for conv " + r.name;
        op.nat2 = (op.fused >= 0 && op.fused_l1 < 0 && (op.pred_mode || op.out2_f32)) ? 1 : 0;
        op.cfg.wpk_off = woff;
        op.cfg.bias_off = boff;
        if (op.fold >= 0) { woff += packed_fold_bytes(op.cfg); boff += (size_t)9 * r.c2; }
        else if (op.kind == OP_CONV0 && op.fused_l1 >= 0) { woff += packed_stem_toeplitz_bytes(d.dtype); boff += 16; }
        else { woff += packed_conv_bytes(r, op.kind == OP_CONV0, op.cfg); boff += (size_t)op.cfg.ntiles_n * 16; }
        if (op.pair >= 0) {
            op.cfg.wpk_off2 = woff; op.cfg.bias_off2 = boff;
            woff += packed_conv_bytes(convs[op.pair], false, op.cfg);
            boff += (size_t)op.cfg.ntiles_n * 16;
        }
        if (op.tail >= 0) {
            const ConvRow& rt = convs[op.tail];
            macs += rt.macs(); fused_params += rt.fused_params();
            op.cfg.wpk_off3 = woff; op.cfg.bias_off3 = boff;
            woff += (d.dtype == VTI_F16 ? 4 : 6) * 1024; boff += 32;
        }
        if (op.fused_l1 >= 0) {
            const ConvRow& r1 = convs[op.fused_l1];
            macs += r1.macs(); fused_params += r1.fused_params();
            op.cfg.wpk_off2 = woff; op.cfg.bias_off2 = boff;
            woff += packed_l1pairs_bytes(d.dtype);
            boff += 32;
        }
        if (op.fused >= 0) {
            const ConvRow& r2 = convs[op.fused];
            macs += r2.macs(); fused_params += r2.fused_params();
            op.cfg.ntiles2 = (r2.c2 + 15) / 16; op.cfg.gemm_n2 = r2.c2;
            if (op.fused_l1 >= 0) {
                op.cfg.wpk_off3 = woff; op.cfg.bias_off3 = boff;
                woff += packed_stage2_bytes(d.dtype, r2, 2);
            } else {
                op.cfg.wpk_off2 = woff; op.cfg.bias_off2 = boff;
                woff += packed_stage2_bytes(d.dtype, r2, op.cfg.NREP);
            }
            boff += (size_t)op.cfg.ntiles2 * 16;
        }
    }
    wpk_bytes = woff; bias_floats = boff;

    {
// ... 28 lines not shown
```

vision-textile-inspection_amd/csrc/vti_api.cpp:

```cpp
#include <algorithm>
#include <cmath>
#include <cstdio>
#include <cstdlib>
#include <cstring>
#include <new>

#include "vti_internal.h"

using namespace vti;

struct vti_ctx {
    Plan plan;
    std::string err;
    int device = -1;
    void* d_wpk = nullptr;
    float* d_bias = nullptr;
    std::vector<float> alpha;
    char* ws = nullptr;
    size_t ws_bytes = 0;
    size_t act_bytes = 0;
    const void* last_input = nullptr;
    void* last_proto = nullptr;
    hipStream_t side[kNumLanes] = {};
    hipEvent_t ev_fork[kNumLanes] = {};
    hipEvent_t ev_join[kNumLanes] = {};
    bool multi_stream = false;
};

static std::string g_create_err;
static const int kMaskSlotsPerFrame = VTI_MASK_SLOTS_PER_FRAME;

static int32_t fail(vti_ctx* c, int32_t code, const std::string& msg) {
    if (c) c->err = msg; else g_create_err = msg;
    return code;
}
static int32_t hip_fail(vti_ctx* c, hipError_t e, const char* what) {
    return fail(c, VTI_ERR_HIP, std::string(what) + ": " + hipGetErrorString(e));
}
#define VTI_HIP(c, call, what) do { hipError_t e_ = (call); if (e_ != hipSuccess) return hip_fail((c), e_, (what)); } while (0)

#ifdef VTI_STAMPS
static void report_stamps(const std::vector<unsigned long long>& h, size_t nwg, bool pk) {
    const char* names[16] = {"start", "c0:top", "c0:A staged", "c0:B staged", "c0:barrier", "c0:mfma done",
                             "c1:top", "c1:A staged", "c1:B staged", "c1:barrier", "c1:mfma done", "epilogue start", "end", "stage2: mfma done", "stage2: stores issued", ""};
    const char* pkn[16] = {"start", "c0:before barrier", "c0:after barrier", "c0:sub-tile A done", "c0:sub-tile B done",
                           "c1:before barrier", "c1:after barrier", "c1:sub-tile A done", "c1:sub-tile B done", "", "", "epilogue start", "end", "", "", ""};
    if (pk) for (int i = 0; i < 16; ++i) names[i] = pkn[i];
    fprintf(stderr, "[stamps] %zu workgroups; median cycles since previous stamp (100 MHz s_memtime ticks x clock)\n", nwg);
    int prev = 0;
    const int order[13] = {1, 2, 3, 4, 5, 6, 7, 8, 9, 10, 11, 13, 12};
    for (int oi = 0; oi < 13; ++oi) {
        const int i = order[oi];
        std::vector<long long> d;
        for (size_t w = 0; w < nwg; ++w) if (h[w * 16 + i] && h[w * 16 + prev]) d.push_back((long long)(h[w * 16 + i] - h[w * 16 + prev]));
        if (d.empty()) continue;
        std::sort(d.begin(), d.end());
        fprintf(stderr, "[stamps] %-16s median %8lld  p10 %8lld  p90 %8lld\n", names[i], d[d.size() / 2], d[d.size() / 10], d[d.size() * 9 / 10]);
        prev = i;
    }
    std::vector<long long> tot;
    for (size_t w = 0; w < nwg; ++w) tot.push_back((long long)(h[w * 16 + 12] - h[w * 16]));
    std::sort(tot.begin(), tot.end());
    fprintf(stderr, "[stamps] whole workgroup   median %8lld\n", tot[tot.size() / 2]);
    std::vector<double> clk;
    for (size_t w = 0; w < nwg; ++w)
        if (h[w * 16 + 15] > h[w * 16 + 14]) clk.push_back((double)(h[w * 16 + 12] - h[w * 16]) / (double)(h[w * 16 + 15] - h[w * 16 + 14]) * 0.1);
    if (!clk.empty()) { std::sort(clk.begin(), clk.end()); fprintf(stderr, "[stamps] in-kernel clock    median %.3f GHz (p10 %.3f, p90 %.3f)\n", clk[clk.size() / 2], clk[clk.size() / 10], clk[clk.size() * 9 / 10]); }
}

template <typename L>
static bool stamped_launch(ConvParams& p, size_t nwg, bool pk, hipStream_t st, const char* header, L&& launch) {
    unsigned long long* d_st = nullptr;
    if (hipMalloc((void**)&d_st, nwg * 16 * 8) != hipSuccess) return false;
    (void)hipMemset(d_st, 0, nwg * 16 * 8);
    p.stamps = d_st;
    (void)launch();
    (void)hipStreamSynchronize(st);
    std::vector<unsigned long long> h(nwg * 16);
    (void)hipMemcpy(h.data(), d_st, nwg * 16 * 8, hipMemcpyDeviceToHost);
    (void)hipFree(d_st);
    p.stamps = nullptr;
    if (header) fprintf(stderr, "%s\n", header);
    report_stamps(h, nwg, pk);
    return true;
}

static size_t conv_workgroups(const ConvParams& p, const ConvCfg& g, int B) {
    const int NTB = g.WN * g.NREP;
    return (p.pk ? (size_t)p.pk_wgs : (size_t)B * p.tiles_y * p.tiles_x) * ((g.ntiles_n + NTB - 1) / NTB);
}
#endif

extern "C" {

int32_t vti_create(const vti_desc* desc, vti_ctx** out) {
    if (!desc || !out) return fail(nullptr, VTI_ERR_ARG, "vti_create: null argument");
    *out = nullptr;
    vti_ctx* c = new (std::nothrow) vti_ctx();
    if (!c) return fail(nullptr, VTI_ERR_NOMEM, "vti_create: out of host memory");
    std::string e;
    try { e = c->plan.build(*desc); } catch (const std::exception& ex) { e = ex.what(); }
    if (!e.empty()) { delete c; return fail(nullptr, VTI_ERR_ARG, "vti_create: " + e); }
    c->act_bytes = c->plan.ws_bytes;
    *out = c;
    return VTI_OK;
}

void vti_destroy(vti_ctx* c) {
    if (!c) return;
    if (c->d_wpk) (void)hipFree(c->d_wpk);
    if (c->d_bias) (void)hipFree(c->d_bias);
    for (int l = 1; l < kNumLanes; ++l) {
        if (c->side[l]) (void)hipStreamDestroy(c->side[l]);
        if (c->ev_fork[l]) (void)hipEventDestroy(c->ev_fork[l]);
        if (c->ev_join[l]) (void)hipEventDestroy(c->ev_join[l]);
    }
    delete c;
}

const char* vti_last_error(const vti_ctx* c) { return c ? c->err.c_str() : g_create_err.c_str(); }

int32_t vti_num_convs(const vti_ctx* c) { return c ? (int32_t)c->plan.convs.size() : 0; }

int32_t vti_conv_at(const vti_ctx* c, int32_t i, vti_conv_info* o) {
    if (!c || !o || i < 0 || i >= (int32_t)c->plan.convs.size()) return VTI_ERR_ARG;
    const ConvRow& r = c->plan.convs[i];
    memset(o, 0, sizeof *o);
    snprintf(o->name, sizeof o->name, "%s", r.name.c_str());
    o->c1 = r.c1; o->c2 = r.c2; o->k = r.k; o->s = r.s; o->kind = r.kind;
    o->h_in = r.h_in; o->w_in = r.w_in; o->h_out = r.h_out; o->w_out = r.w_out;
    o->macs = r.macs();
    for (const Op& op : c->plan.ops) {
        if (op.kind != OP_CONV && op.kind != OP_CONV0) continue;
        if (op.conv == i) {
            o->tile_h = op.cfg.TH; o->tile_w = op.cfg.TW; o->waves_n = op.cfg.WN; o->nrep = op.cfg.NREP;
            o->lds_bytes = (int32_t)op.cfg.lds; o->persistent = op.cfg.pk;
        } else if (op.tail == i) {
            o->tile_h = op.cfg.TH; o->tile_w = op.cfg.TW; o->waves_n = 1; o->nrep = 2; o->lds_bytes = 0; o->fused = 1; o->persistent = 1;
        } else if (op.pair == i) {
            o->tile_h = op.cfg.TH; o->tile_w = op.cfg.TW; o->waves_n = 1; o->nrep = op.cfg.NREP; o->lds_bytes = 0; o->fused = 1;
            o->persistent = 1;
        } else if (op.fold == i) {
            o->tile_h = op.cfg.TH; o->tile_w = op.cfg.TW; o->persistent = op.cfg.pk; o->waves_n = 4; o->nrep = op.cfg.NREP; o->lds_bytes = 0;
        } else if (op.fused_l1 == i) {
            stem_l1_tile(&o->tile_h, &o->tile_w); o->waves_n = 1; o->nrep = 2; o->lds_bytes = 0; o->fused = 1;
        } else if (op.fused == i) {
            o->tile_h = op.cfg.TH; o->tile_w = op.cfg.TW; o->waves_n = 1; o->nrep = op.cfg.ntiles2;
            if (op.fused_l1 >= 0) stem_l1_tile(&o->tile_h, &o->tile_w);
            o->lds_bytes = 0; o->fused = 1;
        }
    }
    return VTI_OK;
}

int32_t vti_num_anchors(const vti_ctx* c) { return c ? c->plan.num_anchors : 0; }
int64_t vti_fused_params(const vti_ctx* c) { return c ? c->plan.fused_params : 0; }
int64_t vti_macs_per_frame(const vti_ctx* c) { return c ? c->plan.macs : 0; }
int64_t vti_workspace_bytes(const vti_ctx* c) {
    if (!c) return 0;
    const vti_desc& d = c->plan.desc;
    return (int64_t)(c->plan.ws_bytes + nms_workspace_bytes(d.max_batch, c->plan.num_anchors) +
                     masks_workspace_bytes(d.max_batch * kMaskSlotsPerFrame, d.H, d.W));
}
int32_t vti_num_launches(const vti_ctx* c) {
    if (!c) return 0;
    int32_t n = 0;
    for (const Op& op : c->plan.ops) n += (op.kind != OP_FORK && op.kind != OP_JOIN);
    return n;
}

int32_t vti_load_weights(vti_ctx* c, const void* blob, size_t nbytes, int32_t device) {
    if (!c) return VTI_ERR_ARG;
    std::vector<uint8_t> wpk;
    std::vector<float> bias;
    std::string e;
    try { e = pack_weights(c->plan, blob, nbytes, wpk, bias, c->alpha); } catch (const std::exception& ex) { e = ex.what(); }
    if (!e.empty()) return fail(c, VTI_ERR_WEIGHTS, e);
    VTI_HIP(c, hipSetDevice(device), "hipSetDevice");
    if (c->d_wpk) { (void)hipFree(c->d_wpk); c->d_wpk = nullptr; }
    if (c->d_bias) { (void)hipFree(c->d_bias); c->d_bias = nullptr; }
    VTI_HIP(c, hipMalloc(&c->d_wpk, wpk.size()), "hipMalloc(weights)");
    VTI_HIP(c, hipMalloc((void**)&c->d_bias, bias.size() * sizeof(float)), "hipMalloc(bias)");
    VTI_HIP(c, hipMemcpy(c->d_wpk, wpk.data(), wpk.size(), hipMemcpyHostToDevice), "hipMemcpy(weights)");
    VTI_HIP(c, hipMemcpy(c->d_bias, bias.data(), bias.size() * sizeof(float), hipMemcpyHostToDevice), "hipMemcpy(bias)");
    c->device = device;
    const char* ss = getenv("VTI_SINGLE_STREAM");
    if (!(ss && ss[0] == '1') && !c->side[1]) {
        bool ok = true;
        for (int l = 1; l < kNumLanes && ok; ++l) {
            ok = hipStreamCreateWithFlags(&c->side[l], hipStreamNonBlocking) == hipSuccess &&
                 hipEventCreateWithFlags(&c->ev_fork[l], hipEventDisableTiming) == hipSuccess &&
                 hipEventCreateWithFlags(&c->ev_join[l], hipEventDisableTiming) == hipSuccess;
        }
        c->multi_stream = ok;
    }
    return VTI_OK;
}

int32_t vti_set_workspace(vti_ctx* c, void* dev_ws, size_t nbytes) {
    if (!c) return VTI_ERR_ARG;
// ... 113 lines not shown
    char msg[200];
    auto bad = [&](const char* what) { snprintf(msg, sizeof msg, "%s: %s", fn, what); return fail(c, VTI_ERR_ARG, msg); };
    if (!c) return VTI_ERR_ARG;
    if (!host_table || !dev_table) return bad("null frame table (host copy or device copy)");
    if ((uintptr_t)dev_table & 15) return bad("the device frame table must be 16-byte aligned");
    int32_t frame;
    if (B < 1) {
        memcpy(&h, host_table, sizeof h);
        return bad(h.magic != kFrameTableMagic ? "host_table is not a table of vti_pack_frames" : "the frame table was packed for another B");
    }
    if (const char* e = frame_table_problem(c, host_table, B, h, frame)) {
        if (frame < 0) return bad(e);
        snprintf(msg, sizeof msg, "%s: frame %d of host_table: %s", fn, frame, e);
        return fail(c, VTI_ERR_ARG, msg);
    }
    return VTI_OK;
}

static const FrameRow* frame_rows(const void* dev_table) { return (const FrameRow*)((const char*)dev_table + sizeof(FrameTableHeader)); }

int32_t vti_letterbox_frames(vti_ctx* c, const uint8_t* frames, const void* host_table, const void* dev_table, int32_t B,
                             uint8_t* out, void* stream) {
    FrameTableHeader h;
    if (int32_t rc = frames_check("vti_letterbox_frames", c, host_table, dev_table, B, h)) return rc;
    if (!frames || !out) return fail(c, VTI_ERR_ARG, "vti_letterbox_frames: null frames or output");
    if (((uintptr_t)frames & 15) || ((uintptr_t)out & 3))
        return fail(c, VTI_ERR_ARG, "vti_letterbox_frames: dev_frames must be 16-byte aligned, dev_input 4-byte aligned");
    if (B > c->plan.desc.max_batch) return fail(c, VTI_ERR_ARG, "vti_letterbox_frames: B above max_batch");
    if (int32_t drc = check_device(c, "vti_letterbox_frames")) return drc;
    VTI_HIP(c, launch_letterbox(frames, B, 0, 0, frame_rows(dev_table), out, h.H, h.W, (hipStream_t)stream), "letterbox kernel");
    return VTI_OK;
}

static void* buf_ptr(vti_ctx* c, int buf, const void* input, void* proto) {
    if (buf == 0) return (void*)input;
    if (buf == c->plan.proto_buf_c) return proto;
    return c->ws + c->plan.bufs[buf].off;
}

static int stagger_units(int dtype) {
    static const int v = getenv("VTI_PK_STAGGER") ? std::max(0, std::min(255, atoi(getenv("VTI_PK_STAGGER")))) : -1;
    return v >= 0 ? v : (dtype == VTI_H2 ? 10 : 0);
}

static int pk_linear_map() {
    static const int v = getenv("VTI_PK_LINEAR_MAP") && getenv("VTI_PK_LINEAR_MAP")[0] == '1';
    return v;
}

static int scalar_store(int n, int ld, int coff) { return (n % 4 || ld % 4 || coff % 4) ? 1 : 0; }

static void fill_conv_params(int conv_elem_size, ConvParams& p, const ConvRow& r, const ConvCfg& g, int B, const void* in, int in_ld,
                             int in_coff, void* out, int out_ld, int out_coff, const void* res, int res_ld,
                             int res_coff, const void* wpk, const float* bias, bool out_f32, int swap_rb) {
    const bool deconv = r.kind == 2;
    memset(&p, 0, sizeof p);
    p.in = in; p.out = out; p.wpk = wpk; p.bias = bias;
    p.B = B; p.Hin = r.h_in; p.Win = r.w_in;
    p.Hout = deconv ? r.h_in : r.h_out; p.Wout = deconv ? r.w_in : r.w_out;
    p.Cin = r.c1; p.in_ld = in_ld; p.in_coff = in_coff;
    p.Cout = g.gemm_n; p.out_ld = out_ld; p.out_coff = out_coff;
    if (res) { p.res = res; p.res_ld = res_ld; p.res_coff = res_coff; p.has_res = 1; }
    p.TH = g.TH; p.TW = g.TW;
    p.tiles_y = (p.Hout + g.TH - 1) / g.TH; p.tiles_x = (p.Wout + g.TW - 1) / g.TW;
    p.WN = g.WN;
    p.nt = g.threads;
    p.pk_lin = pk_linear_map();
    p.act = r.kind == 0; p.out_f32 = out_f32 ? 1 : 0;
    p.deconv_c = deconv ? r.c2 : 0;
    p.swap_rb = swap_rb ? 1 : 0;
    p.nchunks = g.nchunks; p.ntiles_n = g.ntiles_n;
    p.scalar_store = scalar_store(g.gemm_n, out_ld, out_coff);
    const bool conv0 = r.c1 == 3;
    const int ks = deconv ? 1 : r.k, st = deconv ? 1 : r.s;
    const unsigned PW = conv0 ? (unsigned)g.TW : (unsigned)((g.TW - 1) * st + ks);
    p.pw_magic = (unsigned)((0x100000000ull + PW - 1) / PW);
    const unsigned RWD = ((unsigned)(2 * g.TW + 1) * 3 + 6) >> 2;
    p.rw_magic = (unsigned)((0x100000000ull + RWD - 1) / RWD);
    p.tw_magic = (unsigned)((0x100000000ull + (unsigned)g.TW - 1) / (unsigned)g.TW);
    p.wpk_bytes = (unsigned)packed_conv_bytes(r, conv0, g);
    if (g.pk == 2) {
        const size_t es = conv_elem_size;
        const size_t npx = (size_t)B * p.Hout * p.Wout;
        const size_t ib = npx * in_ld * es;
        const size_t ob = (deconv ? 4 * npx : npx) * out_ld * (out_f32 ? 4 : es);
        p.pk = (ib < 0x80000000ull && ob < 0x80000000ull && !res) ? 2 : 0;
        p.in_bytes = (unsigned)ib; p.out_bytes = (unsigned)ob; p.res_bytes = 0;
        p.pk_depth = g.pk_depth; p.pk_wstat = g.pk_wstat; p.pk_cps = g.pk_cps;
        p.pk_tiles = (int)((npx + (size_t)g.TH * 80 - 1) / ((size_t)g.TH * 80));
        p.pk_wgs = pk_grid(p.pk_tiles, g.pk_wgpc, g.ntiles_n / (g.WN * g.NREP), getenv("VTI_PK_MAX_WGS"));
        p.pk_xcd = p.pk_wgs >= 8 ? 1 : 0;
    } else if (g.pk) {
        const size_t es = conv_elem_size;
        const size_t ib = (size_t)B * r.h_in * r.w_in * in_ld * es, ob = (size_t)B * p.Hout * p.Wout * out_ld * (out_f32 ? 4 : es);
        const size_t rb = res ? (size_t)B * p.Hout * p.Wout * res_ld * es : 0;
        p.pk = (ib < 0x80000000ull && ob < 0x80000000ull && rb < 0x80000000ull) ? g.pk : 0;
        p.in_bytes = (unsigned)ib; p.out_bytes = (unsigned)ob; p.res_bytes = (unsigned)rb;
        p.pk_tiles = B * p.tiles_y * p.tiles_x;
        p.pk_depth = g.pk_depth; p.pk_wstat = g.pk_wstat;
        const int gy = g.ntiles_n / (g.WN * g.NREP);
        p.pk_wgs = pk_grid(p.pk_tiles, g.pk_wgpc, gy, getenv("VTI_PK_MAX_WGS"));
        p.pk_xcd = p.pk_wgs >= 8 ? 1 : 0;
        p.pk_stagger = ((g.pk == 1 || g.pk == 4) && p.pk_tiles >= std::max(1, 256 * g.pk_wgpc / gy) && p.pk_wgs >= 16) ? 1 : 0;
    }
}

static void fill_stage2(vti_ctx* c, ConvParams& p, const Op& op, const void* input, void* proto) {
    const Plan& P = c->plan;
    const ConvCfg& g = op.cfg;
    const Buf& o2 = P.bufs[op.out2.buf];
    p.w2 = (const char*)c->d_wpk + g.wpk_off2; p.bias2 = c->d_bias + g.bias_off2; p.alpha2 = c->alpha[op.fused];
    p.out2 = buf_ptr(c, op.out2.buf, input, proto);
    p.Cout2 = g.gemm_n2; p.ntiles2 = g.ntiles2; p.out2_ld = o2.C; p.out2_coff = op.out2.coff;
    p.act2 = P.convs[op.fused].kind == 0; p.out2_f32 = op.out2_f32 ? 1 : 0;
    p.scalar_store2 = scalar_store(g.gemm_n2, o2.C, op.out2.coff);
    p.nat2 = op.nat2;
    p.out2_bstride = P.convs[op.conv].h_out * P.convs[op.conv].w_out;
}

static int32_t forward_impl(vti_ctx* c, const uint8_t* input, int32_t B, int32_t swap_rb, float* pred, void* proto, float* best, void* stream);

int32_t vti_forward(vti_ctx* c, const uint8_t* input, int32_t B, int32_t swap_rb, float* pred, void* proto, void* stream) {
    return forward_impl(c, input, B, swap_rb, pred, proto, nullptr, stream);
}

int32_t vti_forward_scored(vti_ctx* c, const uint8_t* input, int32_t B, int32_t swap_rb, float* pred, void* proto, float* anchor_best,
                           void* stream) {
    if (!anchor_best) return fail(c, VTI_ERR_ARG, "vti_forward_scored: null pointer");
    return forward_impl(c, input, B, swap_rb, pred, proto, anchor_best, stream);
}

static int32_t forward_impl(vti_ctx* c, const uint8_t* input, int32_t B, int32_t swap_rb, float* pred, void* proto, float* best, void* stream) {
    int32_t rc = check_ready(c, B, "vti_forward");
    if (rc) return rc;
    if (!input || !pred || !proto) return fail(c, VTI_ERR_ARG, "vti_forward: null pointer");
    if (B == 0) return VTI_OK;
    const Plan& P = c->plan;
    hipStream_t main_st = (hipStream_t)stream;
    const int dt = P.desc.dtype;
    static const bool list_ops = getenv("VTI_LIST_OPS") != nullptr;
    if (list_ops) {
        int i = 0;
        for (const Op& op : P.ops) {
            if (op.kind == OP_FORK || op.kind == OP_JOIN) continue;
            const bool cv = op.kind == OP_CONV || op.kind == OP_CONV0;
            fprintf(stderr, "[op %2d] lane %d %s%s%s\n", i++, op.lane,
                    cv ? P.convs[op.conv].name.c_str() : op.kind == OP_POOL ? "sppf_pool" : op.kind == OP_UP2 ? "upsample2x" : "decode",
                    cv && op.fused_l1 >= 0 ? (" + " + P.convs[op.fused_l1].name).c_str() : cv && op.fold >= 0 ? (" (folded: " + P.convs[op.fold].name + ")").c_str() : cv && op.pair >= 0 ? (" + " + P.convs[op.pair].name + (op.tail >= 0 ? " + " + P.convs[op.tail].name : "")).c_str() : "",
                    cv && op.fused >= 0 ? (" + " + P.convs[op.fused].name).c_str() : "");
        }
    }
    for (const Op& op : P.ops) {
        hipStream_t st = (c->multi_stream && op.lane > 0) ? c->side[op.lane] : main_st;
        switch (op.kind) {
// ... 12 lines not shown
        case OP_CONV0:
        case OP_CONV: {
            const ConvRow& r = P.convs[op.conv];
            const ConvCfg& g = op.cfg;
            const Buf& ib = P.bufs[op.in.buf];
            const Buf& ob = P.bufs[op.out.buf];
            if (op.fused_l1 >= 0) {
                const ConvRow& r1 = P.convs[op.fused_l1];
                const Buf& o1 = P.bufs[op.out2.buf];
                ConvParams q;
                memset(&q, 0, sizeof q);
                q.in = input; q.B = B; q.Hin = r.h_in; q.Win = r.w_in; q.Hout = r1.h_out; q.Wout = r1.w_out;
                q.Cin = 16; q.Cout = r1.c2; q.ntiles_n = 2; q.act = 1; q.swap_rb = swap_rb ? 1 : 0;
                q.out = buf_ptr(c, op.out2.buf, input, proto); q.out_ld = o1.C; q.out_coff = op.out2.coff;
                q.wpk = (const char*)c->d_wpk + g.wpk_off2; q.bias = c->d_bias + g.bias_off2;
                q.w0 = (const char*)c->d_wpk + g.wpk_off; q.bias0 = c->d_bias + g.bias_off;
                q.alpha = c->alpha[op.fused_l1]; q.alpha0 = c->alpha[op.conv]; q.alpha2 = op.fused >= 0 ? c->alpha[op.fused] : 1.f;
                if (op.fused >= 0) {
                    q.out = nullptr;
                    q.w2 = (const char*)c->d_wpk + g.wpk_off3; q.bias2 = c->d_bias + g.bias_off3;
                    q.out2 = buf_ptr(c, op.out2.buf, input, proto);
                    q.Cout2 = g.gemm_n2; q.ntiles2 = g.ntiles2; q.out2_ld = o1.C; q.out2_coff = op.out2.coff;
                    q.act2 = 1; q.out2_bstride = r1.h_out * r1.w_out;
                    q.scalar_store2 = scalar_store(g.gemm_n2, o1.C, op.out2.coff);
                }
                stem_l1_tile(&q.TH, &q.TW);
                q.tiles_y = (q.Hout + q.TH - 1) / q.TH; q.tiles_x = (q.Wout + q.TW - 1) / q.TW; q.WN = 1;
                q.scalar_store = scalar_store(q.Cout, q.out_ld, q.out_coff);
#ifdef VTI_STAMPS
                if (const char* so = getenv("VTI_STAMP_OP"); so && r.name == so)
                    stamped_launch(q, (size_t)stem_l1_grid(dt, B * q.tiles_y * q.tiles_x), false, st,
                                   ("[stamps] op " + r.name + " + layer 1 (1: patch staged, 2: stem done, 3: layer-1 MFMAs done, 12: end)").c_str(),
                                   [&] { return launch_stem_l1(dt, q, st); });
#endif
                VTI_HIP(c, launch_stem_l1(dt, q, st), "stem + layer 1");
                break;
            }
            if (op.fold >= 0) {
                const ConvRow& ru = P.convs[op.fold];
                ConvParams q;
                memset(&q, 0, sizeof q);
                q.in = buf_ptr(c, op.in.buf, input, proto); q.B = B; q.Hin = ru.h_in; q.Win = ru.w_in; q.Hout = ru.h_in; q.Wout = ru.w_in;
                q.Cin = ru.c1; q.in_ld = ib.C; q.in_coff = op.in.coff; q.Cout = g.gemm_n; q.act = 1; q.fold = 1; q.pk_lin = pk_linear_map();
                q.TH = g.TH; q.TW = g.TW; q.tiles_y = (q.Hout + g.TH - 1) / g.TH; q.tiles_x = (q.Wout + g.TW - 1) / g.TW; q.WN = 4; q.nt = g.threads;
                q.nchunks = g.nchunks; q.ntiles_n = g.ntiles_n;
                q.pw_magic = (unsigned)((0x100000000ull + (unsigned)(g.TW + 2) - 1) / (unsigned)(g.TW + 2));
                q.tw_magic = (unsigned)((0x100000000ull + (unsigned)g.TW - 1) / (unsigned)g.TW);
                q.wpk = (const char*)c->d_wpk + g.wpk_off; q.bias = c->d_bias + g.bias_off; q.wpk_bytes = (unsigned)packed_fold_bytes(g);
                q.alpha = c->alpha[op.conv]; q.alpha0 = 1.f;
                fill_stage2(c, q, op, input, proto);
                if (g.pk) {
                    q.pk = 1; q.pk_depth = g.pk_depth; q.in_bytes = (unsigned)((size_t)B * q.Hin * q.Win * q.in_ld * P.esize);
                    q.pk_tiles = B * q.tiles_y * q.tiles_x;
                    q.pk_wgs = pk_grid(q.pk_tiles, 1, 1, getenv("VTI_PK_MAX_WGS"));
                    q.pk_xcd = q.pk_wgs >= 8 ? 1 : 0;
                    VTI_HIP(c, launch_conv_pk_fold(dt, q, g.lds, st), r.name.c_str());
                } else {
                    VTI_HIP(c, launch_convfold(dt, q, g.lds, st), r.name.c_str());
                }
                break;
            }
            ConvParams p;
            fill_conv_params(P.esize, p, r, g, B, buf_ptr(c, op.in.buf, input, proto), ib.C, op.in.coff,
                             buf_ptr(c, op.out.buf, input, proto), ob.C, op.out.coff,
                             op.has_res ? buf_ptr(c, op.res.buf, input, proto) : nullptr,
                             op.has_res ? P.bufs[op.res.buf].C : 0, op.res.coff,
                             (const char*)c->d_wpk + g.wpk_off, c->d_bias + g.bias_off, op.out_f32, swap_rb);
            p.alpha = c->alpha[op.conv]; p.alpha0 = 1.f;
            p.pk_stagger *= stagger_units(dt);
            p.alpha2 = op.pair >= 0 ? c->alpha[op.pair] : 1.f;
            if (op.fused >= 0) {
                fill_stage2(c, p, op, input, proto);
                if (op.pred_mode) {
                    const int no = 4 + P.desc.nc + P.desc.nm;
                    p.out2 = pred + (size_t)op.pred_a0 * no;
                    p.out2_ld = no; p.out2_coff = op.pred_cbase; p.out2_f32 = 1; p.out2_bstride = P.num_anchors;
                    p.act2 = op.pred_mode == 2 ? 2 : op.pred_mode == 3 ? 3 : 0;
                    p.dfl_stride = (float)op.dfl_stride;
                    p.scalar_store2 = scalar_store(g.gemm_n2, no, op.pred_cbase);
                    p.best = (op.pred_mode == 2 && best) ? best + (size_t)op.pred_a0 * 2 : nullptr;
                }
            }
            if (op.pair >= 0) {
                p.w2 = (const char*)c->d_wpk + g.wpk_off2;
                p.bias2 = c->d_bias + g.bias_off2;
                if (p.pk != 3) return fail(c, VTI_ERR_UNSUPPORTED, "fused bottleneck needs the persistent kernel (tensor too large?)");
                if (op.tail >= 0) {
                    const Buf& o2 = P.bufs[op.out2.buf];
                    if (dt == VTI_F16) p.in_coff -= r.c1;
                    p.alpha0 = c->alpha[op.tail];
                    p.w0 = (const char*)c->d_wpk + g.wpk_off3; p.bias0 = c->d_bias + g.bias_off3;
                    p.out2 = buf_ptr(c, op.out2.buf, input, proto); p.out2_ld = o2.C; p.out2_coff = op.out2.coff; p.Cout2 = P.convs[op.tail].c2;
                    const size_t o2b = (size_t)B * p.Hout * p.Wout * o2.C * P.esize;
                    if (o2b >= 0x80000000ull) return fail(c, VTI_ERR_UNSUPPORTED, "fused bottleneck tail: output tensor too large");
                    p.out2_bytes = (unsigned)o2b;
                }
            }
            if (op.up_C > 0) {
                const Buf& ub = P.bufs[op.up_src.buf];
                p.in2 = buf_ptr(c, op.up_src.buf, input, proto); p.in2_ld = ub.C; p.in2_coff = op.up_src.coff; p.up_C = op.up_C;
                p.in2_bytes = (unsigned)((size_t)B * ub.H * ub.W * ub.C * P.esize);
                if (p.pk != 2) return fail(c, VTI_ERR_UNSUPPORTED, "folded upsample needs the persistent 1x1 kernel (tensor too large?)");
            }
            const bool deconv = r.kind == 2;
            const int ks = deconv ? 1 : r.k, s = deconv ? 1 : r.s;
#ifdef VTI_STAMPS
            if (const char* so = getenv("VTI_STAMP_OP"); so && r.name == so &&
                stamped_launch(p, conv_workgroups(p, g, B), p.pk != 0, st, ("[stamps] op " + r.name).c_str(),
                               [&] { return launch_conv(dt, ks, s, g.NREP, op.kind == OP_CONV0 ? 1 : 0, p, g.lds, st); }))
                break;
#endif
            VTI_HIP(c, launch_conv(dt, ks, s, g.NREP, op.kind == OP_CONV0 ? 1 : 0, p, g.lds, st), r.name.c_str());
            break;
        }
        case OP_POOL: {
            const Buf& ib = P.bufs[op.in.buf];
            PoolParams p;
            p.in = buf_ptr(c, op.in.buf, input, proto); p.out = p.in ? (void*)p.in : nullptr;
            p.B = B; p.H = ib.H; p.W = ib.W; p.C = op.in.C; p.ld = ib.C; p.in_coff = op.in.coff; p.out_coff = op.out.coff;
            VTI_HIP(c, launch_sppf_pool(dt, p, st), "sppf pool");
// ... 794 lines not shown
int32_t vti_debug_conv_output(vti_ctx* c, int32_t i, int32_t B, float* out, void* stream) {
    int32_t rc = check_ready(c, B, "vti_debug_conv_output");
    if (rc) return rc;
    if (i < 0 || i >= (int32_t)c->plan.convs.size() || !out) return fail(c, VTI_ERR_ARG, "vti_debug_conv_output: bad argument");
    const View& v = c->plan.conv_out[i];
    if (v.buf < 0) return fail(c, VTI_ERR_UNSUPPORTED, "vti_debug_conv_output: this conv is fused into the next one; its output is never materialised");
    const Buf& b = c->plan.bufs[v.buf];
    const void* src = buf_ptr(c, v.buf, c->last_input, c->last_proto);
    if (!src) return fail(c, VTI_ERR_STATE, "vti_debug_conv_output: run vti_forward first");
    const int is_f32 = (b.elem == EL_F32 || (b.elem == EL_T && c->plan.desc.dtype == VTI_F32)) ? 1
                       : (b.elem == EL_T && c->plan.desc.dtype == VTI_H2) ? 2 : 0;
    VTI_HIP(c, launch_debug_nchw(is_f32, src, B, b.H, b.W, v.C, b.C, v.coff, out, (hipStream_t)stream), "debug copy");
    return VTI_OK;
}

int32_t vti_debug_conv2d(int32_t dtype, const void* dev_in, int32_t B, int32_t H, int32_t W, int32_t in_ld, int32_t in_coff,
                         int32_t c1, const float* host_w, const float* host_b, int32_t c2, int32_t k, int32_t s, int32_t kind,
                         const void* dev_res, int32_t res_ld, int32_t res_coff, void* dev_out, int32_t out_ld, int32_t out_coff,
                         int32_t out_f32, int32_t swap_rb, int32_t tile_h, int32_t tile_w, int32_t waves_n, int32_t nrep,
                         int32_t iters, float* ms_out, int32_t* cfg_out, void* stream) {
    if (!dev_in || !host_w || !host_b || !dev_out || B < 1 || H < 1 || W < 1 || c1 < 1 || c2 < 1 || iters < 1)
        return fail(nullptr, VTI_ERR_ARG, "vti_debug_conv2d: bad argument");
    if ((dtype != VTI_F16 && dtype != VTI_F32 && dtype != VTI_H2) || (kind < 0 || kind > 2))
        return fail(nullptr, VTI_ERR_ARG, "vti_debug_conv2d: bad dtype/kind");
    const bool conv0 = (c1 == 3);
    if (conv0 ? !(k == 3 && s == 2 && kind == 0) : (c1 % 16 != 0))
        return fail(nullptr, VTI_ERR_ARG, "vti_debug_conv2d: c1 must be 3 (stem) or a multiple of 16");
    if (!((k == 1 && s == 1) || (k == 3 && (s == 1 || s == 2)) || (kind == 2 && k == 2 && s == 2)))
        return fail(nullptr, VTI_ERR_ARG, "vti_debug_conv2d: unsupported kernel/stride");
    ConvRow r;
    r.name = "debug"; r.c1 = c1; r.c2 = c2; r.k = k; r.s = s; r.kind = kind; r.h_in = H; r.w_in = W;
    if (kind == 2) { r.h_out = 2 * H; r.w_out = 2 * W; }
    else { r.h_out = (H + 2 * (k / 2) - k) / s + 1; r.w_out = (W + 2 * (k / 2) - k) / s + 1; }
    ConvCfg g;
    choose_conv_cfg(dtype, r, conv0, B, g, tile_h, tile_w, waves_n, nrep);
    if (g.TH == 0) return fail(nullptr, VTI_ERR_ARG, "vti_debug_conv2d: no launch configuration fits");
    if (cfg_out) { cfg_out[0] = g.TH; cfg_out[1] = g.TW; cfg_out[2] = g.WN; cfg_out[3] = g.NREP; cfg_out[4] = (int32_t)g.lds * (g.pk ? -1 : 1); }
    std::vector<uint8_t> wpk(packed_conv_bytes(r, conv0, g));
    std::vector<float> bias((size_t)g.ntiles_n * 16);
    float alpha = 1.f;
    pack_conv(dtype, r, conv0, g, host_w, host_b, wpk.data(), bias.data(), 0, &alpha);
    void* d_w = nullptr; float* d_b = nullptr;
    hipStream_t st = (hipStream_t)stream;
    VTI_HIP(nullptr, hipMalloc(&d_w, wpk.size()), "hipMalloc");
    hipError_t e = hipMalloc((void**)&d_b, bias.size() * 4);
    if (e == hipSuccess) e = hipMemcpy(d_w, wpk.data(), wpk.size(), hipMemcpyHostToDevice);
    if (e == hipSuccess) e = hipMemcpy(d_b, bias.data(), bias.size() * 4, hipMemcpyHostToDevice);
    hipEvent_t e0 = nullptr, e1 = nullptr;
    if (e == hipSuccess) e = hipEventCreate(&e0);
    if (e == hipSuccess) e = hipEventCreate(&e1);
    if (e == hipSuccess) {
        ConvParams p;
        fill_conv_params(dtype == VTI_F16 ? 2 : 4, p, r, g, B, dev_in, in_ld, in_coff, dev_out, out_ld, out_coff, dev_res, res_ld, res_coff, d_w, d_b,
                         out_f32 != 0, swap_rb);
        p.alpha = alpha; p.alpha2 = p.alpha0 = 1.f;
        p.pk_stagger *= stagger_units(dtype);
        const int ks = kind == 2 ? 1 : k, ss = kind == 2 ? 1 : s;
#ifdef VTI_STAMPS
        (void)launch_conv(dtype, ks, ss, g.NREP, conv0 ? 1 : 0, p, g.lds, st);
        stamped_launch(p, conv_workgroups(p, g, B), p.pk != 0, st, nullptr,
                       [&] { return launch_conv(dtype, ks, ss, g.NREP, conv0 ? 1 : 0, p, g.lds, st); });
#endif
        e = launch_conv(dtype, ks, ss, g.NREP, conv0 ? 1 : 0, p, g.lds, st);
        if (e == hipSuccess) e = hipEventRecord(e0, st);
        for (int i = 1; i < iters && e == hipSuccess; ++i) e = launch_conv(dtype, ks, ss, g.NREP, conv0 ? 1 : 0, p, g.lds, st);
        if (e == hipSuccess) e = hipEventRecord(e1, st);
        if (e == hipSuccess) e = hipStreamSynchronize(st);
        float ms = 0.f;
        if (e == hipSuccess && iters > 1) e = hipEventElapsedTime(&ms, e0, e1);
        if (ms_out) *ms_out = iters > 1 ? ms / (iters - 1) : 0.f;
    }
    if (e0) (void)hipEventDestroy(e0);
    if (e1) (void)hipEventDestroy(e1);
    (void)hipFree(d_w);
    if (d_b) (void)hipFree(d_b);
    if (e != hipSuccess) return hip_fail(nullptr, e, "vti_debug_conv2d");
    return VTI_OK;
}

}
```

vision-textile-inspection_amd/csrc/vti_internal.h:

```cpp
#pragma once
#include <hip/hip_runtime.h>
#include <stddef.h>
#include <stdint.h>
#include <algorithm>
#include <cstdlib>
#include <string>
#include <vector>

#include "../../include/vti.h"
#include "jpeg_decode_dev.h"

namespace vti {

constexpr int kMaxDevices = 64;
inline int current_device_slot() { int d = 0; (void)hipGetDevice(&d); return (unsigned)d < (unsigned)kMaxDevices ? d : 0; }

template <auto K, typename... A>
hipError_t launch_lds(dim3 grid, dim3 block, size_t lds, hipStream_t st, const A&... args) {
    static size_t opted_dev[kMaxDevices] = {};
    size_t& opted = opted_dev[current_device_slot()];
    if (lds > 64 * 1024 && lds > opted) {
        hipError_t e = hipFuncSetAttribute((const void*)K, hipFuncAttributeMaxDynamicSharedMemorySize, (int)lds);
        if (e != hipSuccess) return e;
        opted = lds;
    }
    hipLaunchKernelGGL(K, grid, block, lds, st, args...);
    return hipGetLastError();
}

template <auto K>
int resident_per_cu(int threads, int fallback, int cap) {
    static int per_cu_dev[kMaxDevices] = {};
    int& per_cu = per_cu_dev[current_device_slot()];
    if (!per_cu) {
        int nb = 0;
        if (hipOccupancyMaxActiveBlocksPerMultiprocessor(&nb, (const void*)K, threads, 0) != hipSuccess || nb < 1) nb = fallback;
        per_cu = nb > cap ? cap : nb;
    }
    return per_cu;
}

inline int pk_grid(long tiles, int wgpc, int gy, const char* cap = nullptr) {
    long G = std::min<long>(tiles, std::max(1, 256 * wgpc / gy));
    if (cap) G = std::max<long>(1, std::min<long>(G, atoi(cap)));
    return (int)(G >= 8 ? G & ~7L : G);
}

enum ElemKind { EL_T = 0, EL_F32 = 1, EL_U8 = 2 };

struct Buf {
    int C, H, W;
    int elem;
    size_t off;
    size_t bytes;
};

struct View {
    int buf = -1, coff = 0, C = 0;
};

struct ConvRow {
    std::string name;
    int c1, c2, k, s, kind;
    int h_in, w_in, h_out, w_out;
    int64_t macs() const {
        const int64_t hw = (kind == 2) ? (int64_t)h_in * w_in : (int64_t)h_out * w_out;
        return hw * c1 * c2 * k * k;
    }
    int64_t fused_params() const { return (int64_t)c1 * c2 * k * k + c2; }
};

enum OpKind { OP_CONV0, OP_CONV, OP_POOL, OP_UP2, OP_DECODE, OP_FORK, OP_JOIN };
constexpr int kNumLanes = 10;

struct ConvCfg {
    int TH = 0, TW = 0;
    int WN = 1;
    int NREP = 1;
    int nchunks = 0;
    int ntiles_n = 0;
    int gemm_n = 0;
    size_t lds = 0;
    size_t wpk_off = 0;
    size_t bias_off = 0;
    int ntiles2 = 0, gemm_n2 = 0;
    size_t wpk_off2 = 0, bias_off2 = 0;
    size_t wpk_off3 = 0, bias_off3 = 0;
    int pk = 0, pk_wgpc = 1;
    int pk_depth = 2, pk_wstat = 0;
    int pk_cps = 1;
    int threads = 256;
};

struct Op {
    OpKind kind;
    int conv = -1;
    View in, out, res;
    bool has_res = false;
    bool out_f32 = false;
    int fused = -1;
    int tail = -1;
    int pair = -1;
    int fold = -1;
    int fused_l1 = -1;
    int pred_mode = 0, pred_cbase = 0, pred_a0 = 0;
    int dfl_stride = 0;
    int nat2 = 0;
    View out2;
    bool out2_f32 = false;
    View up_src; int up_C = 0;
    int lane = 0;
    ConvCfg cfg;
};

struct Level { int C, H, W, stride; int box_buf, cls_buf, mc_buf; };

struct Plan {
    vti_desc desc;
    int esize = 2;
    std::vector<ConvRow> convs;
    std::vector<View> conv_out;
    std::vector<Buf> bufs;
    std::vector<Op> ops;
    std::vector<Level> levels;
    int proto_buf_c = 0;
    View proto_src;
    int num_anchors = 0;
    bool pred_scatter = false;
    bool dfl_fused = false;
    size_t ws_bytes = 0;
    size_t wpk_bytes = 0, bias_floats = 0;
    int64_t macs = 0, fused_params = 0;
    std::string build(const vti_desc& d);
};

struct ConvParams {
    const void* in; void* out; const void* res; const void* wpk; const float* bias;
    int B, Hin, Win, Hout, Wout;
    int Cin, in_ld, in_coff;
    int Cout;
    int out_ld, out_coff, res_ld, res_coff;
    int TH, TW, tiles_y, tiles_x, WN;
    int act, out_f32, deconv_c, swap_rb, nchunks, ntiles_n, has_res, scalar_store;
    unsigned pw_magic, rw_magic, tw_magic;
    unsigned wpk_bytes;
    const void* w2; const float* bias2; void* out2;
    int Cout2, ntiles2, out2_ld, out2_coff, act2 , out2_f32, scalar_store2, nat2, out2_bstride;
    int nt;
    float* best;
    float dfl_stride;
    int pk, pk_tiles, pk_wgs, pk_xcd, pk_depth, pk_wstat, pk_lin ;
    int pk_cps;
    int pk_stagger;
    unsigned in_bytes, out_bytes, res_bytes, out2_bytes;
    const void* in2; int in2_ld, in2_coff, up_C; unsigned in2_bytes;
    int fold;
    const void* w0; const float* bias0;
    float alpha, alpha2, alpha0;
    unsigned long long* stamps;
};

hipError_t launch_conv(int dtype, int ks, int stride, int nrep, int mode, const ConvParams& p,
                       size_t lds_bytes, hipStream_t st);
bool conv_fusable(int nrep, int nrep2);
size_t conv_lds_bytes(int ks, int stride, int mode, int TH, int TW, int WN, int NREP);
bool conv_cfg_fits(int ks, int stride, int mode, int TH, int TW, int WN, int NREP, int threads = 256);
hipError_t launch_stem_l1(int dtype, const ConvParams& p, hipStream_t st);
size_t stem_l1_lds_bytes(int dtype);
void stem_l1_tile(int* th, int* tw);
int stem_l1_grid(int dtype, int ntiles);
void pack_stem_toeplitz(int dtype, const ConvRow& r0, const float* w, const float* b, uint8_t* dst_w, float* dst_b, float* alpha = nullptr);
size_t packed_stem_toeplitz_bytes(int dtype);
hipError_t launch_convfold(int dtype, const ConvParams& p, size_t lds_bytes, hipStream_t st);
size_t convfold_lds_bytes(int TH, int TW);
bool convfold_supported(int c_in, int c_mid, int c_out, int ntiles2);
void pack_conv_fold(int dtype, const ConvRow& rU, const ConvRow& rV, const ConvCfg& c, const float* wU, const float* bU,
                    const float* wV, const float* bV, uint8_t* dst_w, float* dst_b, float* alpha = nullptr);
size_t packed_fold_bytes(const ConvCfg& c);
hipError_t launch_conv_pk_fold(int dtype, const ConvParams& p, size_t lds_bytes, hipStream_t st);
size_t conv_pk_fold_lds_bytes(int nchunks, int depth);
int conv_pk_fold_depth(int nchunks);
void pack_conv_l1pairs(int dtype, const ConvRow& r1, const float* w, const float* b, uint8_t* dst_w, float* dst_b, float* alpha = nullptr);
size_t packed_l1pairs_bytes(int dtype);
hipError_t launch_conv_pk(int dtype, int nrep, const ConvParams& p, size_t lds_bytes, hipStream_t st);
size_t conv_pk_lds_bytes(int TH, int WN, int NREP, int nchunks);
size_t conv_pk_lds_bytes(int TH, int WN, int NREP, int nchunks, int depth, int wstat = 0);
int conv_pk_depth(int TH, int WN, int NREP, int nchunks, int wstat = 0);
hipError_t launch_conv_pk2(int dtype, int nrep, const ConvParams& p, size_t lds_bytes, hipStream_t st);
size_t conv_pk2_lds_bytes(int TH, int WN, int NREP, int nchunks, int depth, int wstat = 0);
bool conv_pk2_fits(int TH, int WN, int NREP, int nchunks, int wstat = 0);
bool conv_pk2_instantiated(int nrep, int wn);
int conv_pk2_depth(int TH, int WN, int NREP, int nchunks, int wstat = 0);
bool conv_pk_fits(int TH, int WN, int NREP, int nchunks, int wstat = 0);
bool conv_pk_instantiated(int nrep, int wn);
hipError_t launch_conv1_pk(int dtype, int nrep, const ConvParams& p, size_t lds_bytes, hipStream_t st);
size_t conv1_pk_lds_bytes(int nwm, int WN, int NREP, int nchunks, int depth, int wstat, int cps = 1);
bool conv1_pk_fits(int nwm, int WN, int NREP, int nchunks, int depth, int wstat, int cps = 1);
bool conv1_pk_instantiated(int nrep, int wn);
hipError_t launch_bneck_pk(int dtype, int nrep, const ConvParams& p, size_t lds_bytes, hipStream_t st);
size_t bneck_pk_lds_bytes(int TH, int NREP);
size_t bneck_pk_lds_bytes(int TH, int NREP, int depth);
int bneck_pk_depth(int TH, int NREP);
bool bneck_pk_fits(int TH, int NREP);

struct PoolParams { const void* in; void* out; int B, H, W, C, ld, in_coff, out_coff; };
hipError_t launch_sppf_pool(int dtype, const PoolParams& p, hipStream_t st);

struct Up2Params { const void* in; void* out; int B, H, W, C, in_ld, in_coff, out_ld, out_coff; };
hipError_t launch_upsample2x(int dtype, const Up2Params& p, hipStream_t st);

struct DecodeParams {
    const float* box[3]; const float* cls[3]; const float* mc[3];
    int H[3], W[3], stride[3], a0[3];
    int B, A, nc, nm, reg_max;
    float* pred;
};
hipError_t launch_decode(const DecodeParams& p, hipStream_t st);
hipError_t launch_box_decode(const DecodeParams& p, hipStream_t st);

// ... 66 lines not shown
#define VTI_POLY_WORKGROUPS 128
struct PolyLayout {
    int WW;
    bool in_lds;
    size_t img_bytes, off_runs, off_rows, off_img, area_bytes, total;
};
void mask_polygons_layout(int H, int W, int row_bytes, PolyLayout& L);
hipError_t launch_mask_polygons(const uint8_t* masks, int n, const int* n_live, int H, int W, int row_bytes, double gain,
                                double padx, double pady, int H0, int W0, int strategy, void* scratch, int* offsets, float* points,
                                long long max_points, hipStream_t st);

struct AnnotateLayout {
    int WW;
    bool in_lds;
    size_t off_recs, off_meta, off_env, off_cont, off_union, off_areas, area_bytes, off_runs, off_rows, total;
};
void annotate_layout(int n_sel, int max_det, int H0, int W0, int max_points, AnnotateLayout& L);
struct AnnotateFrames { const FrameRow* rows_in; const FrameRow* rows_out; bool any_lds, any_global; long long max_px; };
hipError_t launch_annotate(const uint8_t* frames, int B, int H0, int W0, const void* cameras, int n_cams, const int* cam_of_frame,
                           const uint8_t* masks, int native, const float* dets, const float* xyxy, const int* counts,
                           const int* offsets, int max_det, int nm, int capacity, int H, int W, const int* frame_i32,
                           const double* stitch_f64, const int* stitch_i32, const int* select, int n_sel, int max_points, uint8_t* out,
                           int* status, void* scratch, hipStream_t st, const AnnotateFrames* fr = nullptr);

struct JpegLayout {
    int mr, mc;
    long long nblk;
    long long stream_bytes;
    long long NC;
    long long max_file;
    size_t off_fbits, off_fsize, off_coef, off_bitpos, off_stream, off_chunk, total;
};
bool encode_jpeg_layout(long long n, int H0, int W0, JpegLayout& L);
void encode_jpeg_header(int H0, int W0, int quality, uint8_t out[624]);
hipError_t launch_encode_jpeg(const uint8_t* frames, int n, int H0, int W0, int rgb, int quality, void* scratch, long long* offsets,
                              uint8_t* out, long long max_bytes, hipStream_t st);
struct JpegFramesLayout {
    int n;
    long long n_mcu, n_chunk;
    long long max_bytes;
    size_t off_pm, off_pc, off_fbits, off_fsize, off_coef, off_bitpos, off_stream, off_chunk, total;
};
bool encode_jpeg_frames_layout(const void* host_table, JpegFramesLayout& L);
hipError_t launch_encode_jpeg_frames(const uint8_t* frames, const void* host_table, const FrameRow* rows, int rgb, int quality,
                                     void* scratch, long long* offsets, uint8_t* out, long long max_bytes, hipStream_t st);

int decode_jpeg_parse(const uint8_t* d, long long n, JpegDecRow& R, std::string& err);
size_t decode_jpeg_scratch_of(JpegDecRow& R, size_t at);
bool decode_jpeg_row_ok(const JpegDecRow& R, const JpegDecHeader& H, size_t& scratch_at, std::string& why);
hipError_t launch_decode_jpeg(const uint8_t* files, const void* host_table, const void* dev_table, int n, int rgb, uint8_t* out, int* info,
                              void* scratch, hipStream_t st);

void choose_conv_cfg(int dtype, const ConvRow& r, bool conv0, int max_batch, ConvCfg& c,
                     int th = 0, int tw = 0, int wn = 0, int nrep = 0, bool allow_pk = true);
void pack_conv(int dtype, const ConvRow& r, bool conv0, const ConvCfg& c, const float* w, const float* b,
               uint8_t* dst_w, float* dst_b, int cin_off = 0, float* alpha = nullptr);
size_t packed_conv_bytes(const ConvRow& r, bool conv0, const ConvCfg& c);
void pack_conv_stage2(int dtype, const ConvRow& r2, int nrep1, const float* w, const float* b, uint8_t* dst_w, float* dst_b,
                      bool natural_rows = false, float* alpha = nullptr);
size_t packed_stage2_bytes(int dtype, const ConvRow& r2, int nrep1);
std::string pack_weights(const Plan& plan, const void* blob, size_t nbytes,
                         std::vector<uint8_t>& wpk, std::vector<float>& bias, std::vector<float>& alpha);

}
```

vision-textile-inspection_amd/engine.py:

```python
import ctypes as C

import numpy as np
import torch

from . import _lib
from ._lib import VtiConvInfo, VtiDesc, VtiMeasureParams, check, lib

DTYPES = {"fp16": _lib.VTI_F16, "f16": _lib.VTI_F16, "half": _lib.VTI_F16,
          "fp32": _lib.VTI_F32, "f32": _lib.VTI_F32, "float": _lib.VTI_F32,
          "h2": _lib.VTI_H2, "fp16x2": _lib.VTI_H2, "split": _lib.VTI_H2}
_DTYPE_NAME = {_lib.VTI_F16: "fp16", _lib.VTI_F32: "fp32", _lib.VTI_H2: "h2"}
MASK_MODES = {"logit": _lib.VTI_MASK_LOGIT, "sigmoid": _lib.VTI_MASK_SIGMOID}
PACKINGS = {"u8": _lib.VTI_PACK_U8, "bits": _lib.VTI_PACK_BITS}
POLY_STRATEGIES = {"largest": _lib.VTI_POLY_LARGEST, "concat": _lib.VTI_POLY_CONCAT}


def _ptr(t):
    return C.c_void_p(t.data_ptr()) if t is not None else C.c_void_p(0)


def _stream():
    return C.c_void_p(torch.cuda.current_stream().cuda_stream)


class FrameTable:

    def __init__(self, host, dev, shapes, byte_offsets, total_bytes, H, W):
        self.host, self.dev, self.shapes, self.byte_offsets, self.total_bytes = host, dev, shapes, byte_offsets, total_bytes
        self.H, self.W, self.B = H, W, len(shapes)
        self.max_H0, self.max_W0 = max(h for h, _ in shapes), max(w for _, w in shapes)

    def _ptrs(self):
        return C.c_void_p(self.host.data_ptr()), C.c_void_p(self.dev.data_ptr())

    def row(self, b):
        i32, f64 = (C.c_int32 * 8)(), (C.c_double * 5)()
        check(None, lib().vti_frame_table_info(C.c_void_p(self.host.data_ptr()), int(b), i32, f64))
        d = dict(zip(("H0", "W0", "new_h", "new_w", "top", "left"), (int(v) for v in i32[:6])))
        d["offset"] = (i32[6] & 0xFFFFFFFF) | (i32[7] << 32)
        d.update(zip(("scale_x", "scale_y", "gain", "padx", "pady"), (float(v) for v in f64)))
        return d


class Engine:

    def __init__(self, scale="n", nc=80, nm=32, reg_max=16, H=640, W=640, max_batch=1, dtype="fp16"):
        self.scale, self.nc, self.nm, self.reg_max = scale, nc, nm, reg_max
        self.H, self.W, self.max_batch = H, W, max_batch
        self.dtype = _DTYPE_NAME[DTYPES[dtype]]
        self._ctx = C.c_void_p(0)
        desc = VtiDesc(scale.encode()[:1], nc, nm, reg_max, H, W, max_batch, DTYPES[dtype])
        rc = lib().vti_create(C.byref(desc), C.byref(self._ctx))
        if rc != 0:
            raise _lib.VtiError(rc, lib().vti_last_error(None).decode())
        self.device = None
        self._ws = None

    def __del__(self):
        try:
            if getattr(self, "_ctx", None) and self._ctx.value:
                lib().vti_destroy(self._ctx)
                self._ctx = C.c_void_p(0)
        except Exception:
            pass

    def conv_table(self):
        out = []
        info = VtiConvInfo()
        for i in range(lib().vti_num_convs(self._ctx)):
            check(self._ctx, lib().vti_conv_at(self._ctx, i, C.byref(info)))
            out.append(dict(name=info.name.decode(), c1=info.c1, c2=info.c2, k=info.k, s=info.s, kind=info.kind,
                            h_in=info.h_in, w_in=info.w_in, h_out=info.h_out, w_out=info.w_out, macs=info.macs,
                            tile=(info.tile_h, info.tile_w), waves_n=info.waves_n, nrep=info.nrep, lds=info.lds_bytes,
                            fused=bool(info.fused), persistent=bool(info.persistent)))
        return out

    @property
    def num_anchors(self):
        return lib().vti_num_anchors(self._ctx)

    @property
    def fused_params(self):
        return lib().vti_fused_params(self._ctx)

    @property
    def macs_per_frame(self):
        return lib().vti_macs_per_frame(self._ctx)

    @property
    def workspace_bytes(self):
        return lib().vti_workspace_bytes(self._ctx)

    @property
    def num_launches(self):
        return lib().vti_num_launches(self._ctx)

    @property
    def no(self):
        return 4 + self.nc + self.nm

    @property
    def torch_dtype(self):
        return torch.float16 if self.dtype == "fp16" else torch.float32

    def load_weights(self, blob, device=0):
        if not torch.cuda.is_available():
            raise RuntimeError("vti_amd needs a ROCm GPU: torch.cuda.is_available() is False (no CPU fallback)")
        dev = torch.device("cuda", device) if isinstance(device, int) else torch.device(device)
        torch.cuda.set_device(dev)
        buf = (C.c_char * len(blob)).from_buffer_copy(blob)
        check(self._ctx, lib().vti_load_weights(self._ctx, buf, len(blob), dev.index or 0))
        self.device = dev
        self._ws = torch.empty(self.workspace_bytes + 256, dtype=torch.uint8, device=dev)
        base = self._ws.data_ptr()
        aligned = (base + 255) & ~255
        check(self._ctx, lib().vti_set_workspace(self._ctx, C.c_void_p(aligned), self.workspace_bytes))
        return self

    def letterbox(self, frames, out=None):
        B, H0, W0, _ = frames.shape
        if out is None:
            out = torch.empty((B, self.H, self.W, 3), dtype=torch.uint8, device=frames.device)
        check(self._ctx, lib().vti_letterbox(self._ctx, _ptr(frames), B, H0, W0, _ptr(out), _stream()))
        return out

    def pack_frames(self, shapes, device=None):
        shapes = [(int(h), int(w)) for h, w in (tuple(x)[:2] for x in shapes)]
# ... 659 lines not shown
H2_SCALE = 16.0


def h2_encode(t):
    s = t.float() * H2_SCALE
    hi = s.half()
    lo = (s - hi.float()).half()
    bits = hi.view(torch.int16).to(torch.int32) & 0xFFFF | (lo.view(torch.int16).to(torch.int32) << 16)
    return bits.view(torch.float32)


def h2_decode(t):
    bits = t.view(torch.int32)
    hi = (bits & 0xFFFF).to(torch.int16).view(torch.float16).float()
    lo = (bits >> 16).to(torch.int16).view(torch.float16).float()
    return (hi + lo) / H2_SCALE


def unpack_bits(bits, W):
    b = bits.unsqueeze(-1)
    sh = torch.arange(8, device=bits.device, dtype=torch.uint8)
    full = ((b >> sh) & 1).reshape(*bits.shape[:-1], bits.shape[-1] * 8)
    return full if full.shape[-1] == W else full[..., :W]


def to_numpy(t):
    return t.detach().cpu().numpy() if isinstance(t, torch.Tensor) else np.asarray(t)


def debug_conv2d(x, w, b, k, s, kind=0, dtype="fp16", res=None, out=None, in_coff=0, c1=None, out_coff=0, out_ld=None,
                 out_f32=False, swap_rb=False, tile=(0, 0), waves_n=0, nrep=0, iters=1):
    B, H, W, ld = x.shape
    w = np.ascontiguousarray(to_numpy(w), dtype=np.float32)
    b = np.ascontiguousarray(to_numpy(b), dtype=np.float32)
    c2 = w.shape[1] if kind == 2 else w.shape[0]
    if c1 is None:
        c1 = w.shape[0] if kind == 2 else w.shape[1]
    Ho, Wo = (2 * H, 2 * W) if kind == 2 else ((H + 2 * (k // 2) - k) // s + 1, (W + 2 * (k // 2) - k) // s + 1)
    tdt = torch.float32 if (out_f32 or DTYPES[dtype] != _lib.VTI_F16) else torch.float16
    if out is None:
        out_ld = out_ld or (out_coff + c2)
        out = torch.zeros((B, Ho, Wo, out_ld), dtype=tdt, device=x.device)
    else:
        out_ld = out.shape[3]
    ms = C.c_float(0)
    cfg = (C.c_int32 * 5)()
    rc = lib().vti_debug_conv2d(DTYPES[dtype], _ptr(x), B, H, W, ld, in_coff, c1, w.ctypes.data_as(C.c_void_p),
                                b.ctypes.data_as(C.c_void_p), c2, k, s, kind, _ptr(res), res.shape[3] if res is not None else 0,
                                0, _ptr(out), out_ld, out_coff, int(out_f32), int(swap_rb), tile[0], tile[1], waves_n, nrep,
                                iters, C.byref(ms), cfg, _stream())
    if rc != 0:
        raise _lib.VtiError(rc, lib().vti_last_error(None).decode())
    return out, ms.value, dict(tile=(cfg[0], cfg[1]), waves_n=cfg[2], nrep=cfg[3], lds=abs(cfg[4]), pk=cfg[4] < 0)
```

Measured before the change: 16220.

## Add fused tower conv variant with three pixel repeats per wave

Templates the conv kernel, epilogue and fused second stage on the per-wave pixel repeat count instead of a fixed five. It instantiates a three-repeat variant for the H2 fused 3x3→1x1 tower with 80 output channels in both stages. That variant runs stage 2 one pixel row at a time and spreads the next-tap weight unpacking over fewer steps. The intent is to cut accumulator register pressure so more waves can be resident, at the cost of smaller tiles and more launches or workgroups per layer. It also adds a debug entry point for the fused tower and exposes mrep/threads in the conv table.

```diff
diff --git a/include/vti.h b/include/vti.h
--- a/include/vti.h
+++ b/include/vti.h
@@ -47,6 +47,7 @@
     int32_t lds_bytes;
     int32_t fused;
     int32_t persistent;
+    int32_t mrep, threads;
 } vti_conv_info;
 
 int32_t vti_create(const vti_desc* desc, vti_ctx** out);
@@ -238,6 +239,11 @@
                          int32_t tile_h, int32_t tile_w, int32_t waves_n, int32_t nrep, int32_t iters,
                          float* ms_out, int32_t* cfg_out, void* stream);
 
+int32_t vti_debug_tower2d(int32_t dtype, const void* dev_in, int32_t B, int32_t H, int32_t W, int32_t in_ld, int32_t in_coff,
+                          int32_t c1, const float* host_w1, const float* host_b1, int32_t c_mid, const float* host_w2,
+                          const float* host_b2, int32_t c2, int32_t act2, float* dev_out, int32_t out_ld, int32_t out_coff,
+                          int32_t mrep, int32_t* cfg_out, void* stream);
+
 #ifdef __cplusplus
 }
 #endif
diff --git a/vision-textile-inspection_amd/_lib.py b/vision-textile-inspection_amd/_lib.py
--- a/vision-textile-inspection_amd/_lib.py
+++ b/vision-textile-inspection_amd/_lib.py
@@ -21,7 +21,8 @@
                 ("s", C.c_int32), ("kind", C.c_int32), ("h_in", C.c_int32), ("w_in", C.c_int32),
                 ("h_out", C.c_int32), ("w_out", C.c_int32), ("macs", C.c_int64),
                 ("tile_h", C.c_int32), ("tile_w", C.c_int32), ("waves_n", C.c_int32), ("nrep", C.c_int32),
-                ("lds_bytes", C.c_int32), ("fused", C.c_int32), ("persistent", C.c_int32)]
+                ("lds_bytes", C.c_int32), ("fused", C.c_int32), ("persistent", C.c_int32),
+                ("mrep", C.c_int32), ("threads", C.c_int32)]
 
 
 class VtiMeasureParams(C.Structure):
@@ -126,6 +127,8 @@
     "vti_debug_conv2d": (_I32, [_I32, _P, _I32, _I32, _I32, _I32, _I32, _I32, _P, _P, _I32, _I32, _I32, _I32,
                                 _P, _I32, _I32, _P, _I32, _I32, _I32, _I32, _I32, _I32, _I32, _I32, _I32,
                                 _P, _P, _P]),
+    "vti_debug_tower2d": (_I32, [_I32, _P, _I32, _I32, _I32, _I32, _I32, _I32, _P, _P, _I32, _P, _P, _I32, _I32, _P, _I32, _I32,
+                                 _I32, _P, _P]),
 }
 
 _lib = None
diff --git a/vision-textile-inspection_amd/api.py b/vision-textile-inspection_amd/api.py
--- a/vision-textile-inspection_amd/api.py
+++ b/vision-textile-inspection_amd/api.py
@@ -1,5 +1,5 @@
 from ._lib import LIB_PATH, SIGNATURES, VtiError, lib
-from .engine import Engine, FrameTable, debug_conv2d, h2_decode, h2_encode, kmeans1d2, pixels_to_world, unpack_bits
+from .engine import Engine, FrameTable, debug_conv2d, debug_tower2d, h2_decode, h2_encode, kmeans1d2, pixels_to_world, unpack_bits
 from .feeder import FrameFeeder
 from .model import YOLO, Boxes, Masks, Results, letterbox_shape
 from .weights import pack_container, random_weights, unpack_container
@@ -7,6 +7,6 @@
 from .measure import MeasureParams, MultiCameraMeasurer, StitchMeasurer
 from . import annotate, consumer, dataparallel, jpeg
 
-__all__ = ["LIB_PATH", "SIGNATURES", "VtiError", "lib", "Engine", "FrameTable", "debug_conv2d", "h2_decode", "h2_encode", "kmeans1d2", "pixels_to_world", "unpack_bits", "FrameFeeder", "YOLO", "Boxes", "Masks",
+__all__ = ["LIB_PATH", "SIGNATURES", "VtiError", "lib", "Engine", "FrameTable", "debug_conv2d", "debug_tower2d", "h2_decode", "h2_encode", "kmeans1d2", "pixels_to_world", "unpack_bits", "FrameFeeder", "YOLO", "Boxes", "Masks",
            "Results", "letterbox_shape", "pack_container", "random_weights", "unpack_container", "convert_checkpoint", "convert_state_dict",
            "MeasureParams", "MultiCameraMeasurer", "StitchMeasurer", "annotate", "consumer", "dataparallel", "jpeg"]
diff --git a/vision-textile-inspection_amd/csrc/conv.hip b/vision-textile-inspection_amd/csrc/conv.hip
--- a/vision-textile-inspection_amd/csrc/conv.hip
+++ b/vision-textile-inspection_amd/csrc/conv.hip
@@ -20,7 +20,7 @@
     return 4 * plane + (size_t)WN * NREP * taps * 1024 + raw;
 }
 
-template <typename T, int KS, int S, int NREP, int WN, int NREP2 = 0, int NT = 256>
+template <typename T, int KS, int S, int NREP, int WN, int NREP2 = 0, int NT = 256, int MR = MREP>
 __global__ __launch_bounds__(NT, NT == 512 ? 1 : 2) void conv_kernel(const ConvParams p) {
     using vec = typename Tr<T>::vec;
     constexpr int VEC = Tr<T>::VEC, KC = Tr<T>::KC;
@@ -48,11 +48,11 @@
     const int tile_px = p.TH * p.TW;
     VTI_STAMP(0);
 
-    int abase[MREP], opy[MREP], opx[MREP];
-    bool pvalid[MREP];
-#pragma unroll
-    for (int m = 0; m < MREP; ++m) {
-        const int pp = (wm * MREP + m) * 16 + (lane & 15);
+    int abase[MR], opy[MR], opx[MR];
+    bool pvalid[MR];
+#pragma unroll
+    for (int m = 0; m < MR; ++m) {
+        const int pp = (wm * MR + m) * 16 + (lane & 15);
         const bool v = pp < tile_px;
         const int pc = v ? pp : 0;
         const int py = (int)__umulhi((unsigned)pc, p.tw_magic), px = pc - py * p.TW;
@@ -61,9 +61,9 @@
         abase[m] = (lane >> 4) * plane_bytes + ((py * S) * PW + px * S) * 16;
     }
 
-    f32x4 acc[MREP][NREP];
-#pragma unroll
-    for (int m = 0; m < MREP; ++m)
+    f32x4 acc[MR][NREP];
+#pragma unroll
+    for (int m = 0; m < MR; ++m)
 #pragma unroll
         for (int n = 0; n < NREP; ++n) acc[m][n] = (f32x4){0.f, 0.f, 0.f, 0.f};
 
@@ -121,13 +121,13 @@
         if (c < 2) VTI_STAMP(4 + 5 * c);
         if (c + PD < p.nchunks) issue(c + PD, ra[SET], rb[SET]);
         {
-            constexpr int NSTEP = TAPS * MREP;
+            constexpr int NSTEP = TAPS * MR;
             constexpr int XD = NREP >= 5 ? 2 : 3;
             constexpr int WD = NREP >= 5 ? 1 : 2;
             vec xq[XD];
             vec wq[WD][NREP];
             auto ldx = [&](int s_) -> vec {
-                const int tp = s_ / MREP, mm = s_ % MREP;
+                const int tp = s_ / MR, mm = s_ % MR;
                 const int toff = ((tp / KS) * PW + (tp % KS)) * 16;
                 return *(const vec*)(smA + abase[mm] + toff);
             };
@@ -136,23 +136,23 @@
                 for (int n = 0; n < NREP; ++n)
                     w[n] = *(const vec*)(smB + ((wn * NREP + n) * TAPS + tp) * 1024 + lane * 16);
             };
-            if constexpr (Tr<T>::H2 && TAPS > 1 && (NREP <= 3 || (NREP == 4 && NT == 512))) {
+            if constexpr (Tr<T>::H2 && TAPS > 1 && (NREP <= 3 || (NREP == 4 && NT == 512) || MR < MREP)) {
                 auto ldw1 = [&](int tp, int n) -> vec { return *(const vec*)(smB + ((wn * NREP + n) * TAPS + tp) * 1024 + lane * 16); };
-                h2_taps<NREP, MREP, TAPS, 3>(acc, ldx, ldw1);
+                h2_taps<NREP, MR, TAPS, 3>(acc, ldx, ldw1);
             } else {
             ldw(0, wq[0]);
             xq[0] = ldx(0);
             if (XD > 2 && NSTEP > 1) xq[1] = ldx(1);
 #pragma unroll
             for (int s_ = 0; s_ < NSTEP; ++s_) {
-                const int tp = s_ / MREP, mm = s_ % MREP;
+                const int tp = s_ / MR, mm = s_ % MR;
                 if (s_ + XD - 1 < NSTEP) xq[(s_ + XD - 1) % XD] = ldx(s_ + XD - 1);
                 if (WD == 2 && mm == 0 && tp + 1 < TAPS) ldw(tp + 1, wq[(tp + 1) % WD]);
                 __builtin_amdgcn_sched_barrier(0);
 #pragma unroll
                 for (int n = 0; n < NREP; ++n) acc[mm][n] = mma(wq[tp % WD][n], xq[s_ % XD], acc[mm][n]);
                 __builtin_amdgcn_sched_barrier(0);
-                if (WD == 1 && mm == MREP - 1 && tp + 1 < TAPS) ldw(tp + 1, wq[0]);
+                if (WD == 1 && mm == MR - 1 && tp + 1 < TAPS) ldw(tp + 1, wq[0]);
             }
             }
         }
@@ -176,7 +176,19 @@
         conv_epilogue<T, NREP>(p, acc, pvalid, opy, opx, b, nt0, wn, lane);
     } else {
         static_assert(WN == 1, "fused stage needs the whole Cout in one wave");
-        conv_stage2<T, NREP, NREP2>(p, acc, pvalid, opy, opx, b, lane);
+        if constexpr (MR < MREP) {
+#pragma unroll
+            for (int m = 0; m < MR; ++m) {
+                f32x4 acc1[1][NREP];
+#pragma unroll
+                for (int n = 0; n < NREP; ++n) acc1[0][n] = acc[m][n];
+                const bool pv1[1] = {pvalid[m]};
+                const int oy1[1] = {opy[m]}, ox1[1] = {opx[m]};
+                conv_stage2<T, NREP, NREP2>(p, acc1, pv1, oy1, ox1, b, lane);
+            }
+        } else {
+            conv_stage2<T, NREP, NREP2>(p, acc, pvalid, opy, opx, b, lane);
+        }
     }
     VTI_STAMP(12);
 }
@@ -707,9 +719,12 @@
 using ConvTile1 = decltype(concat(ConvTile3{}, Combos<Ints<3, 2>, Ints<4, 2>, Ints<5, 2>, Ints<2, 4>, Ints<3, 4>, Ints<4, 4>, Ints<5, 4>>{}));
 using StemNrep = Combos<Ints<1>, Ints<2>, Ints<3>, Ints<4>, Ints<5>>;
 
-bool conv_cfg_fits(int ks, int stride, int mode, int TH, int TW, int WN, int NREP, int threads) {
-    if (mode == 1) return WN == 1 && (2 * TH + 1) * (((2 * TW + 1) * 3 + 6) >> 2) < 65536;
+bool conv_cfg_fits(int ks, int stride, int mode, int TH, int TW, int WN, int NREP, int threads, int mrep) {
+    if (mode == 1) return WN == 1 && mrep == MREP && (2 * TH + 1) * (((2 * TW + 1) * 3 + 6) >> 2) < 65536;
     if (threads != 256 && !(threads == 512 && ks == 3 && stride == 1 && WN == 1)) return false;
+    if (WN != 1 && WN != 2 && WN != 4) return false;
+    if (mrep != MREP && !(mrep == kTowerMrep && threads == 256 && ks == 3 && stride == 1 && WN == 1 && NREP == 5)) return false;
+    if (TH < 1 || TW < 1 || TH * TW > (threads / 64 / WN) * mrep * 16) return false;
     const int AR = threads == 512 ? 6 : (stride == 2 ? 12 : 8);
     const int npix = patch_dim(TH, ks, stride, mode) * patch_dim(TW, ks, stride, mode);
     if (((npix + 7) / 8) * 32 > threads * AR) return false;
@@ -733,6 +748,11 @@
         if (!(ks == 3 && stride == 1 && p.WN == 1 && mode == 0)) return hipErrorInvalidValue;
         return combo_dispatch(FusedPairs{}, [&](auto c) {
             using C = decltype(c);
+            if (p.mrep != MREP) {
+                if constexpr (Tr<T>::H2 && C::v[0] == 5 && C::v[1] == 5)
+                    if (p.mrep == kTowerMrep && p.nt == 256) return launch_lds<conv_kernel<T, 3, 1, 5, 1, 5, 256, kTowerMrep>>(grid, dim3(256), lds, st, p);
+                return hipErrorInvalidValue;
+            }
             return p.nt == 512 ? launch_lds<conv_kernel<T, 3, 1, C::v[0], 1, C::v[1], 512>>(grid, dim3(512), lds, st, p)
                                : launch_lds<conv_kernel<T, 3, 1, C::v[0], 1, C::v[1]>>(grid, dim3(256), lds, st, p);
         }, nrep, p.ntiles2);
@@ -759,7 +779,8 @@
     if (grid.x == 0) return hipSuccess;
     const int nwaves = p.nt == 512 ? 8 : 4;
     if ((p.nt != 256 && p.nt != 512) || (p.nt == 512 && p.ntiles2 == 0)) return hipErrorInvalidValue;
-    if (p.TH * p.TW > (nwaves / p.WN) * MREP * 16 || (p.WN != 1 && p.WN != 2 && p.WN != 4)) return hipErrorInvalidValue;
+    if (p.mrep != MREP && !(p.mrep == kTowerMrep && p.ntiles2 > 0 && p.nt == 256)) return hipErrorInvalidValue;
+    if (p.TH * p.TW > (nwaves / p.WN) * p.mrep * 16 || (p.WN != 1 && p.WN != 2 && p.WN != 4)) return hipErrorInvalidValue;
     return with_conv_type(dtype, [&](auto t) { return launch_t<typename decltype(t)::type>(ks, stride, nrep, mode, p, grid, lds_bytes, st); });
 }
 
diff --git a/vision-textile-inspection_amd/csrc/conv_dev.h b/vision-textile-inspection_amd/csrc/conv_dev.h
--- a/vision-textile-inspection_amd/csrc/conv_dev.h
+++ b/vision-textile-inspection_amd/csrc/conv_dev.h
@@ -79,6 +79,8 @@
 __device__ __forceinline__ void h2_taps(f32x4 (&acc)[M][NREP], LDX ldx, LDW ldw) {
     constexpr int NSTEP = TAPS * M;
     constexpr unsigned SEL_H = 0x01000100u;
+    static_assert(M >= 2, "h2_taps prepares the next tap under steps 1 .. M-1");
+    constexpr int PR = M >= 5 ? 1 : (4 + M - 2) / (M - 1);
     h2x4 xq[XD];
     u32x4 wraw[NREP];
     u32x4 wh[2][NREP], wl[2][NREP];
@@ -122,13 +124,16 @@
             }
             if (false) {
 #else
-            if (mm >= 1 && k < 8 * NREP && tp + 1 < TAPS) {
+            if (mm >= 1 && k * PR < 8 * NREP && tp + 1 < TAPS) {
 #endif
-                const int pn = k >> 3, r = k & 7, i = r & 3;
-                if (r < 4) wh[nxt][pn][i] = __builtin_amdgcn_perm(wraw[pn][i], wraw[pn][i], SEL_H);
-                else wl[nxt][pn][i] = wraw[pn][i] >> 16;
+#pragma unroll
+                for (int e = 0; e < PR; ++e) {
+                    const int kk = k * PR + e, pn = kk >> 3, r = kk & 7, i = r & 3;
+                    if (r < 4) wh[nxt][pn][i] = __builtin_amdgcn_perm(wraw[pn][i], wraw[pn][i], SEL_H);
+                    else wl[nxt][pn][i] = wraw[pn][i] >> 16;
+                }
                 __builtin_amdgcn_sched_group_barrier(0x008, 1, 0);
-                __builtin_amdgcn_sched_group_barrier(0x002, 1, 0);
+                __builtin_amdgcn_sched_group_barrier(0x002, PR, 0);
             }
         }
         __builtin_amdgcn_sched_barrier(0);
@@ -196,7 +201,7 @@
     }
 }
 
-constexpr int MREP = 5;
+constexpr int MREP = kMrep;
 
 #ifdef VTI_STAMPS
 #define VTI_STAMP(i)                                                                              \
@@ -215,9 +220,9 @@
 #define VTI_STAMP(i) do { } while (0)
 #endif
 
-template <typename T, int NREP>
-__device__ __forceinline__ void conv_epilogue(const ConvParams& p, f32x4 (&acc)[MREP][NREP], const bool (&pvalid)[MREP],
-                                              const int (&opy)[MREP], const int (&opx)[MREP], int b, int nt0, int wn,
+template <typename T, int NREP, int M>
+__device__ __forceinline__ void conv_epilogue(const ConvParams& p, f32x4 (&acc)[M][NREP], const bool (&pvalid)[M],
+                                              const int (&opy)[M], const int (&opx)[M], int b, int nt0, int wn,
                                               int lane) {
     constexpr bool FAST = !Tr<T>::F32;
     const int crun = (nt0 + wn * NREP) * 16 + (lane >> 4) * 4 * NREP;
@@ -230,7 +235,7 @@
     if (!p.scalar_store && !p.out_f32 && !p.deconv_c) {
         const bool has_res = __builtin_amdgcn_readfirstlane(p.has_res) != 0;
 #pragma unroll
-        for (int m = 0; m < MREP; ++m) {
+        for (int m = 0; m < M; ++m) {
             if (!pvalid[m]) continue;
             const size_t opix = ((size_t)(b * p.Hout + opy[m])) * p.Wout + opx[m];
             T* op = (T*)p.out + opix * p.out_ld + p.out_coff + crun;
@@ -296,7 +301,7 @@
         if (p.deconv_c && !p.scalar_store && !p.out_f32 && !p.has_res) {
             const int qd = crun / p.deconv_c, co = crun - qd * p.deconv_c;
 #pragma unroll
-            for (int m = 0; m < MREP; ++m) {
+            for (int m = 0; m < M; ++m) {
                 if (!pvalid[m] || crun >= p.Cout) continue;
                 const size_t opix = ((size_t)(b * 2 * p.Hout + 2 * opy[m] + (qd >> 1))) * (2 * p.Wout) + 2 * opx[m] + (qd & 1);
                 T* op = (T*)p.out + opix * p.out_ld + p.out_coff + co;
@@ -316,7 +321,7 @@
         }
     }
 #pragma unroll
-    for (int m = 0; m < MREP; ++m) {
+    for (int m = 0; m < M; ++m) {
         if (!pvalid[m]) continue;
 #pragma unroll
         for (int n = 0; n < NREP; ++n) {
@@ -397,9 +402,9 @@
     for (int n = 0; n < NREP2; ++n) r.bias2[n] = *(const f32x4*)(p.bias2 + crun2 + cstep2 * n);
 }
 
-template <typename T, int NREP, int NREP2, bool FOLD = false, bool PRE = false>
-__device__ __forceinline__ void conv_stage2(const ConvParams& p, f32x4 (&acc)[MREP][NREP], const bool (&pvalid)[MREP],
-                                            const int (&opy)[MREP], const int (&opx)[MREP], int b, int lane,
+template <typename T, int NREP, int NREP2, bool FOLD = false, bool PRE = false, int M = MREP>
+__device__ __forceinline__ void conv_stage2(const ConvParams& p, f32x4 (&acc)[M][NREP], const bool (&pvalid)[M],
+                                            const int (&opy)[M], const int (&opx)[M], int b, int lane,
                                             const Stage2Regs<T, NREP, NREP2>* pre = nullptr, bool interior = false) {
     const int OW = FOLD ? 2 * p.Wout : p.Wout;
     using vec = typename Tr<T>::vec;
@@ -407,15 +412,15 @@
     constexpr int KT = sizeof(T) == 2 ? (NREP + 1) / 2 : NREP;
     const __amdgpu_buffer_rsrc_t rsW2 = __builtin_amdgcn_make_buffer_rsrc(
         (void*)p.w2, 0, (int)(KT * p.ntiles2 * 1024), 0x00020000);
-    f32x4 bias1[FOLD ? MREP : 1][NREP];
+    f32x4 bias1[FOLD ? M : 1][NREP];
     if (PRE && (!FOLD || interior)) {
 #pragma unroll
-        for (int m = 0; m < (FOLD ? MREP : 1); ++m)
+        for (int m = 0; m < (FOLD ? M : 1); ++m)
 #pragma unroll
             for (int n = 0; n < NREP; ++n) bias1[m][n] = pre->bias1[n];
     } else if constexpr (FOLD) {
 #pragma unroll
-        for (int m = 0; m < MREP; ++m) {
+        for (int m = 0; m < M; ++m) {
             const int cy = opy[m] == 0 ? 0 : (opy[m] == 2 * p.Hout - 1 ? 2 : 1), cx = opx[m] == 0 ? 0 : (opx[m] == OW - 1 ? 2 : 1);
             const float* bt = p.bias + (cy * 3 + cx) * (16 * NREP) + (lane >> 4) * 4 * NREP;
 #pragma unroll
@@ -425,9 +430,9 @@
 #pragma unroll
         for (int n = 0; n < NREP; ++n) bias1[0][n] = *(const f32x4*)(p.bias + (lane >> 4) * 4 * NREP + 4 * n);
     }
-    f32x4 acc2[MREP][NREP2];
-#pragma unroll
-    for (int m = 0; m < MREP; ++m)
+    f32x4 acc2[M][NREP2];
+#pragma unroll
+    for (int m = 0; m < M; ++m)
 #pragma unroll
         for (int n = 0; n < NREP2; ++n) acc2[m][n] = (f32x4){0.f, 0.f, 0.f, 0.f};
 #pragma unroll
@@ -439,7 +444,7 @@
             else w2[n] = buf_load16<vec>(rsW2, (unsigned)(((t2 * p.ntiles2 + n) * 64 + lane) * 16), 0u);
         }
 #pragma unroll
-        for (int m = 0; m < MREP; ++m) {
+        for (int m = 0; m < M; ++m) {
             vec x;
             if constexpr (sizeof(T) == 2) {
 #pragma unroll
@@ -480,7 +485,7 @@
         if (p.act2 == 3) {
             const int g = lane >> 4;
 #pragma unroll
-            for (int m = 0; m < MREP; ++m) {
+            for (int m = 0; m < M; ++m) {
                 float d4[4];
 #pragma unroll
                 for (int n = 0; n < 4; ++n) {
@@ -513,7 +518,7 @@
     if constexpr (sizeof(T) == 2 && NREP2 % 2 == 0) {
         if (!p.nat2 && !p.out2_f32 && !p.scalar_store2 && (p.Cout2 & 7) == 0 && ((p.out2_ld | p.out2_coff) & 7) == 0) {
 #pragma unroll
-            for (int m = 0; m < MREP; ++m) {
+            for (int m = 0; m < M; ++m) {
                 if (!pvalid[m]) continue;
                 half_t* op = (half_t*)p.out2 + ((size_t)b * p.out2_bstride + (size_t)opy[m] * OW + opx[m]) * p.out2_ld + p.out2_coff + crun2;
 #pragma unroll
@@ -532,7 +537,7 @@
     }
     const bool want_best = p.act2 == 2 && p.best != nullptr;
 #pragma unroll
-    for (int m = 0; m < MREP; ++m) {
+    for (int m = 0; m < M; ++m) {
         const size_t pix = (size_t)b * p.out2_bstride + (size_t)opy[m] * OW + opx[m];
         const size_t o0 = pix * p.out2_ld + p.out2_coff;
         float bv = -INFINITY;
diff --git a/vision-textile-inspection_amd/csrc/plan.cpp b/vision-textile-inspection_amd/csrc/plan.cpp
--- a/vision-textile-inspection_amd/csrc/plan.cpp
+++ b/vision-textile-inspection_amd/csrc/plan.cpp
@@ -270,7 +270,7 @@
 }
 
 void choose_conv_cfg(int dtype, const ConvRow& r, bool conv0, int max_batch, ConvCfg& c, int fth, int ftw, int fwn,
-                     int fnrep, bool allow_pk) {
+                     int fnrep, bool allow_pk, int mrep) {
     const bool f16 = dtype == VTI_F16;
     const int KC = f16 ? 32 : 16;
     const bool deconv = r.kind == 2;
@@ -298,7 +298,7 @@
             const int gy = (c.ntiles_n + BN - 1) / BN;
             const double n_eff = (double)c.ntiles_n / (gy * BN);
             if (n_eff < 0.74 && !fnrep) continue;
-            const int BM = (4 / WN) * 80;
+            const int BM = (4 / WN) * 16 * mrep;
             for (int TW = std::min(Wo, BM); TW >= 1; --TW) {
                 if (ftw && TW != ftw) continue;
                 int TH = std::min(Ho, BM / TW);
@@ -309,7 +309,7 @@
                 const int PH = conv0 ? TH : (TH - 1) * st + ks, PW = conv0 ? TW : (TW - 1) * st + ks;
                 const size_t lds = conv_lds_bytes(ks, st, conv0 ? 1 : 0, TH, TW, WN, NREP);
                 if (lds > ((fth || ftw) ? 160u : 80u) * 1024) continue;
-                if (!conv_cfg_fits(ks, st, conv0 ? 1 : 0, TH, TW, WN, NREP)) continue;
+                if (!conv_cfg_fits(ks, st, conv0 ? 1 : 0, TH, TW, WN, NREP, 256, mrep)) continue;
                 const double halo = conv0 ? (double)(4 * TH * TW) / ((2 * TH + 1) * (2 * TW + 1))
                                           : (double)(TH * TW * st * st) / (PH * PW);
                 const double lds_traffic = 1.0 / NREP + 1.0 / 5;
@@ -321,7 +321,7 @@
                 if (wgs < 512) score *= 0.5 + 0.5 * wgs / 512;
                 if (score > best) {
                     best = score;
-                    c.TH = TH; c.TW = TW; c.WN = WN; c.NREP = NREP; c.lds = lds;
+                    c.TH = TH; c.TW = TW; c.WN = WN; c.NREP = NREP; c.lds = lds; c.mrep = mrep;
                 }
             }
         }
@@ -686,8 +686,18 @@
             const char* pf = getenv("VTI_PK_FUSED");
             const bool pkf = pf ? (pf[0] == '1' || (pf[0] == '2' && r.c2 / 16 <= 4)) : (d.dtype == VTI_H2 && r.c2 / 16 == 4);
             choose_conv_cfg(d.dtype, r, false, d.max_batch, op.cfg, 0, 0, 1, r.c2 / 16, pk_ok && pkf);
+            const char* tm = getenv("VTI_TOWER_MREP");
+            const int tower_mrep = tm ? atoi(tm) : kTowerMrep;
+            bool small_tiles = false;
+            if (d.dtype == VTI_H2 && tower_mrep == kTowerMrep && !op.cfg.pk && r.k == 3 && r.s == 1 && r.kind == 0 && r.c2 == 80 &&
+                (convs[op.fused].c2 + 15) / 16 == 5) {
+                ConvCfg s3 = op.cfg;
+                s3.TH = 0;
+                choose_conv_cfg(d.dtype, r, false, d.max_batch, s3, 0, 0, 1, 5, false, kTowerMrep);
+                if (s3.TH && 2 * s3.lds <= 160 * 1024) { op.cfg = s3; small_tiles = true; }
+            }
             const char* n5 = getenv("VTI_NO_T512");
-            if (!(n5 && n5[0] == '1') && !op.cfg.pk && op.cfg.TH && r.k == 3 && r.s == 1 && r.kind == 0) {
+            if (!small_tiles && !(n5 && n5[0] == '1') && !op.cfg.pk && op.cfg.TH && r.k == 3 && r.s == 1 && r.kind == 0) {
                 const int TH = 16, TW = 40;
                 const double eff_now = (double)r.h_out * r.w_out / ((double)((r.h_out + op.cfg.TH - 1) / op.cfg.TH) * ((r.w_out + op.cfg.TW - 1) / op.cfg.TW) * op.cfg.TH * op.cfg.TW);
                 const double eff_512 = (double)r.h_out * r.w_out / ((double)((r.h_out + TH - 1) / TH) * ((r.w_out + TW - 1) / TW) * TH * TW);
diff --git a/vision-textile-inspection_amd/csrc/vti_api.cpp b/vision-textile-inspection_amd/csrc/vti_api.cpp
--- a/vision-textile-inspection_amd/csrc/vti_api.cpp
+++ b/vision-textile-inspection_amd/csrc/vti_api.cpp
@@ -25,7 +25,13 @@
     hipEvent_t ev_fork[kNumLanes] = {};
     hipEvent_t ev_join[kNumLanes] = {};
     bool multi_stream = false;
+    int pk_max_wgs = -1;
 };
+
+static int env_pk_max_wgs() {
+    const char* e = getenv("VTI_PK_MAX_WGS");
+    return e ? std::max(0, atoi(e)) : -1;
+}
 
 static std::string g_create_err;
 static const int kMaskSlotsPerFrame = VTI_MASK_SLOTS_PER_FRAME;
@@ -102,6 +108,7 @@
     try { e = c->plan.build(*desc); } catch (const std::exception& ex) { e = ex.what(); }
     if (!e.empty()) { delete c; return fail(nullptr, VTI_ERR_ARG, "vti_create: " + e); }
     c->act_bytes = c->plan.ws_bytes;
+    c->pk_max_wgs = env_pk_max_wgs();
     *out = c;
     return VTI_OK;
 }
@@ -135,6 +142,7 @@
         if (op.conv == i) {
             o->tile_h = op.cfg.TH; o->tile_w = op.cfg.TW; o->waves_n = op.cfg.WN; o->nrep = op.cfg.NREP;
             o->lds_bytes = (int32_t)op.cfg.lds; o->persistent = op.cfg.pk;
+            if (!op.cfg.pk && op.fold < 0 && op.fused_l1 < 0) { o->mrep = op.cfg.mrep; o->threads = op.cfg.threads; }
         } else if (op.tail == i) {
             o->tile_h = op.cfg.TH; o->tile_w = op.cfg.TW; o->waves_n = 1; o->nrep = 2; o->lds_bytes = 0; o->fused = 1; o->persistent = 1;
         } else if (op.pair == i) {
@@ -146,6 +154,7 @@
             stem_l1_tile(&o->tile_h, &o->tile_w); o->waves_n = 1; o->nrep = 2; o->lds_bytes = 0; o->fused = 1;
         } else if (op.fused == i) {
             o->tile_h = op.cfg.TH; o->tile_w = op.cfg.TW; o->waves_n = 1; o->nrep = op.cfg.ntiles2;
+            if (!op.cfg.pk && op.fold < 0 && op.fused_l1 < 0) { o->mrep = op.cfg.mrep; o->threads = op.cfg.threads; }
             if (op.fused_l1 >= 0) stem_l1_tile(&o->tile_h, &o->tile_w);
             o->lds_bytes = 0; o->fused = 1;
         }
@@ -365,7 +374,7 @@
 
 static void fill_conv_params(int conv_elem_size, ConvParams& p, const ConvRow& r, const ConvCfg& g, int B, const void* in, int in_ld,
                              int in_coff, void* out, int out_ld, int out_coff, const void* res, int res_ld,
-                             int res_coff, const void* wpk, const float* bias, bool out_f32, int swap_rb) {
+                             int res_coff, const void* wpk, const float* bias, bool out_f32, int swap_rb, int pk_max_wgs) {
     const bool deconv = r.kind == 2;
     memset(&p, 0, sizeof p);
     p.in = in; p.out = out; p.wpk = wpk; p.bias = bias;
@@ -377,7 +386,7 @@
     p.TH = g.TH; p.TW = g.TW;
     p.tiles_y = (p.Hout + g.TH - 1) / g.TH; p.tiles_x = (p.Wout + g.TW - 1) / g.TW;
     p.WN = g.WN;
-    p.nt = g.threads;
+    p.nt = g.threads; p.mrep = g.mrep;
     p.pk_lin = pk_linear_map();
     p.act = r.kind == 0; p.out_f32 = out_f32 ? 1 : 0;
     p.deconv_c = deconv ? r.c2 : 0;
@@ -401,7 +410,7 @@
         p.in_bytes = (unsigned)ib; p.out_bytes = (unsigned)ob; p.res_bytes = 0;
         p.pk_depth = g.pk_depth; p.pk_wstat = g.pk_wstat; p.pk_cps = g.pk_cps;
         p.pk_tiles = (int)((npx + (size_t)g.TH * 80 - 1) / ((size_t)g.TH * 80));
-        p.pk_wgs = pk_grid(p.pk_tiles, g.pk_wgpc, g.ntiles_n / (g.WN * g.NREP), getenv("VTI_PK_MAX_WGS"));
+        p.pk_wgs = pk_grid(p.pk_tiles, g.pk_wgpc, g.ntiles_n / (g.WN * g.NREP), pk_max_wgs);
         p.pk_xcd = p.pk_wgs >= 8 ? 1 : 0;
     } else if (g.pk) {
         const size_t es = conv_elem_size;
@@ -412,7 +421,7 @@
         p.pk_tiles = B * p.tiles_y * p.tiles_x;
         p.pk_depth = g.pk_depth; p.pk_wstat = g.pk_wstat;
         const int gy = g.ntiles_n / (g.WN * g.NREP);
-        p.pk_wgs = pk_grid(p.pk_tiles, g.pk_wgpc, gy, getenv("VTI_PK_MAX_WGS"));
+        p.pk_wgs = pk_grid(p.pk_tiles, g.pk_wgpc, gy, pk_max_wgs);
         p.pk_xcd = p.pk_wgs >= 8 ? 1 : 0;
         p.pk_stagger = ((g.pk == 1 || g.pk == 4) && p.pk_tiles >= std::max(1, 256 * g.pk_wgpc / gy) && p.pk_wgs >= 16) ? 1 : 0;
     }
@@ -531,7 +540,7 @@
                 if (g.pk) {
                     q.pk = 1; q.pk_depth = g.pk_depth; q.in_bytes = (unsigned)((size_t)B * q.Hin * q.Win * q.in_ld * P.esize);
                     q.pk_tiles = B * q.tiles_y * q.tiles_x;
-                    q.pk_wgs = pk_grid(q.pk_tiles, 1, 1, getenv("VTI_PK_MAX_WGS"));
+                    q.pk_wgs = pk_grid(q.pk_tiles, 1, 1, c->pk_max_wgs);
                     q.pk_xcd = q.pk_wgs >= 8 ? 1 : 0;
                     VTI_HIP(c, launch_conv_pk_fold(dt, q, g.lds, st), r.name.c_str());
                 } else {
@@ -544,7 +553,7 @@
                              buf_ptr(c, op.out.buf, input, proto), ob.C, op.out.coff,
                              op.has_res ? buf_ptr(c, op.res.buf, input, proto) : nullptr,
                              op.has_res ? P.bufs[op.res.buf].C : 0, op.res.coff,
-                             (const char*)c->d_wpk + g.wpk_off, c->d_bias + g.bias_off, op.out_f32, swap_rb);
+                             (const char*)c->d_wpk + g.wpk_off, c->d_bias + g.bias_off, op.out_f32, swap_rb, c->pk_max_wgs);
             p.alpha = c->alpha[op.conv]; p.alpha0 = 1.f;
             p.pk_stagger *= stagger_units(dt);
             p.alpha2 = op.pair >= 0 ? c->alpha[op.pair] : 1.f;
@@ -1445,7 +1454,7 @@
     if (e == hipSuccess) {
         ConvParams p;
         fill_conv_params(dtype == VTI_F16 ? 2 : 4, p, r, g, B, dev_in, in_ld, in_coff, dev_out, out_ld, out_coff, dev_res, res_ld, res_coff, d_w, d_b,
-                         out_f32 != 0, swap_rb);
+                         out_f32 != 0, swap_rb, env_pk_max_wgs());
         p.alpha = alpha; p.alpha2 = p.alpha0 = 1.f;
         p.pk_stagger *= stagger_units(dtype);
         const int ks = kind == 2 ? 1 : k, ss = kind == 2 ? 1 : s;
@@ -1471,4 +1480,60 @@
     return VTI_OK;
 }
 
-}
+int32_t vti_debug_tower2d(int32_t dtype, const void* dev_in, int32_t B, int32_t H, int32_t W, int32_t in_ld, int32_t in_coff, int32_t c1,
+                          const float* host_w1, const float* host_b1, int32_t c_mid, const float* host_w2, const float* host_b2,
+                          int32_t c2, int32_t act2, float* dev_out, int32_t out_ld, int32_t out_coff, int32_t mrep, int32_t* cfg_out,
+                          void* stream) {
+    if (!dev_in || !host_w1 || !host_b1 || !host_w2 || !host_b2 || !dev_out || B < 1 || H < 1 || W < 1 || c1 < 16 || c1 % 16 ||
+        c_mid < 16 || c_mid % 16 || c2 < 1 || in_coff < 0 || in_coff + c1 > in_ld || out_coff < 0 || out_coff + c2 > out_ld ||
+        (act2 != 0 && act2 != 2))
+        return fail(nullptr, VTI_ERR_ARG, "vti_debug_tower2d: bad argument");
+    if (dtype != VTI_F16 && dtype != VTI_F32 && dtype != VTI_H2) return fail(nullptr, VTI_ERR_ARG, "vti_debug_tower2d: bad dtype");
+    if (mrep == 0) mrep = kMrep;
+    if (mrep != kMrep && !(mrep == kTowerMrep && dtype == VTI_H2))
+        return fail(nullptr, VTI_ERR_ARG, "vti_debug_tower2d: no instantiation with this pixel grid");
+    ConvRow r, r2;
+    r.name = "debug.1"; r.c1 = c1; r.c2 = c_mid; r.k = 3; r.s = 1; r.kind = 0; r.h_in = r.h_out = H; r.w_in = r.w_out = W;
+    r2.name = "debug.2"; r2.c1 = c_mid; r2.c2 = c2; r2.k = 1; r2.s = 1; r2.kind = 1; r2.h_in = r2.h_out = H; r2.w_in = r2.w_out = W;
+    const int nrep = c_mid / 16, nt2 = (c2 + 15) / 16;
+    if (!conv_fusable(nrep, nt2)) return fail(nullptr, VTI_ERR_ARG, "vti_debug_tower2d: no fused instantiation for these channel counts");
+    ConvCfg g;
+    choose_conv_cfg(dtype, r, false, B, g, 0, 0, 1, nrep, false, mrep);
+    if (g.TH == 0) return fail(nullptr, VTI_ERR_ARG, "vti_debug_tower2d: no launch configuration fits");
+    g.ntiles2 = nt2; g.gemm_n2 = c2;
+    if (cfg_out) { cfg_out[0] = g.TH; cfg_out[1] = g.TW; cfg_out[2] = g.mrep; cfg_out[3] = g.threads; cfg_out[4] = (int32_t)g.lds; }
+    std::vector<uint8_t> wpk(packed_conv_bytes(r, false, g)), wpk2(packed_stage2_bytes(dtype, r2, nrep));
+    std::vector<float> bias((size_t)g.ntiles_n * 16), bias2((size_t)nt2 * 16);
+    float alpha = 1.f, alpha2 = 1.f;
+    pack_conv(dtype, r, false, g, host_w1, host_b1, wpk.data(), bias.data(), 0, &alpha);
+    pack_conv_stage2(dtype, r2, nrep, host_w2, host_b2, wpk2.data(), bias2.data(), true, &alpha2);
+    void *d_w = nullptr, *d_w2 = nullptr; float *d_b = nullptr, *d_b2 = nullptr;
+    hipStream_t st = (hipStream_t)stream;
+    hipError_t e = hipMalloc(&d_w, wpk.size());
+    if (e == hipSuccess) e = hipMalloc(&d_w2, wpk2.size());
+    if (e == hipSuccess) e = hipMalloc((void**)&d_b, bias.size() * 4);
+    if (e == hipSuccess) e = hipMalloc((void**)&d_b2, bias2.size() * 4);
+    if (e == hipSuccess) e = hipMemcpy(d_w, wpk.data(), wpk.size(), hipMemcpyHostToDevice);
+    if (e == hipSuccess) e = hipMemcpy(d_w2, wpk2.data(), wpk2.size(), hipMemcpyHostToDevice);
+    if (e == hipSuccess) e = hipMemcpy(d_b, bias.data(), bias.size() * 4, hipMemcpyHostToDevice);
+    if (e == hipSuccess) e = hipMemcpy(d_b2, bias2.data(), bias2.size() * 4, hipMemcpyHostToDevice);
+    if (e == hipSuccess) {
+        ConvParams p;
+        fill_conv_params(dtype == VTI_F16 ? 2 : 4, p, r, g, B, dev_in, in_ld, in_coff, nullptr, c_mid, 0, nullptr, 0, 0, d_w, d_b, false, 0, -1);
+        p.alpha = alpha; p.alpha2 = alpha2; p.alpha0 = 1.f;
+        p.w2 = d_w2; p.bias2 = d_b2; p.out2 = dev_out;
+        p.Cout2 = c2; p.ntiles2 = nt2; p.out2_ld = out_ld; p.out2_coff = out_coff; p.act2 = act2; p.out2_f32 = 1; p.nat2 = 1;
+        p.scalar_store2 = scalar_store(c2, out_ld, out_coff);
+        p.out2_bstride = H * W;
+        e = launch_conv(dtype, 3, 1, g.NREP, 0, p, g.lds, st);
+        if (e == hipSuccess) e = hipStreamSynchronize(st);
+    }
+    if (d_w) (void)hipFree(d_w);
+    if (d_w2) (void)hipFree(d_w2);
+    if (d_b) (void)hipFree(d_b);
+    if (d_b2) (void)hipFree(d_b2);
+    if (e != hipSuccess) return hip_fail(nullptr, e, "vti_debug_tower2d");
+    return VTI_OK;
+}
+
+}
diff --git a/vision-textile-inspection_amd/csrc/vti_internal.h b/vision-textile-inspection_amd/csrc/vti_internal.h
--- a/vision-textile-inspection_amd/csrc/vti_internal.h
+++ b/vision-textile-inspection_amd/csrc/vti_internal.h
@@ -40,9 +40,9 @@
     return per_cu;
 }
 
-inline int pk_grid(long tiles, int wgpc, int gy, const char* cap = nullptr) {
+inline int pk_grid(long tiles, int wgpc, int gy, int cap = -1) {
     long G = std::min<long>(tiles, std::max(1, 256 * wgpc / gy));
-    if (cap) G = std::max<long>(1, std::min<long>(G, atoi(cap)));
+    if (cap >= 0) G = std::max<long>(1, std::min<long>(G, cap));
     return (int)(G >= 8 ? G & ~7L : G);
 }
 
@@ -72,6 +72,8 @@
 
 enum OpKind { OP_CONV0, OP_CONV, OP_POOL, OP_UP2, OP_DECODE, OP_FORK, OP_JOIN };
 constexpr int kNumLanes = 10;
+
+constexpr int kMrep = 5, kTowerMrep = 3;
 
 struct ConvCfg {
     int TH = 0, TW = 0;
@@ -90,6 +92,7 @@
     int pk_depth = 2, pk_wstat = 0;
     int pk_cps = 1;
     int threads = 256;
+    int mrep = kMrep;
 };
 
 struct Op {
@@ -147,6 +150,7 @@
     const void* w2; const float* bias2; void* out2;
     int Cout2, ntiles2, out2_ld, out2_coff, act2 , out2_f32, scalar_store2, nat2, out2_bstride;
     int nt;
+    int mrep;
     float* best;
     float dfl_stride;
     int pk, pk_tiles, pk_wgs, pk_xcd, pk_depth, pk_wstat, pk_lin ;
@@ -164,7 +168,7 @@
                        size_t lds_bytes, hipStream_t st);
 bool conv_fusable(int nrep, int nrep2);
 size_t conv_lds_bytes(int ks, int stride, int mode, int TH, int TW, int WN, int NREP);
-bool conv_cfg_fits(int ks, int stride, int mode, int TH, int TW, int WN, int NREP, int threads = 256);
+bool conv_cfg_fits(int ks, int stride, int mode, int TH, int TW, int WN, int NREP, int threads = 256, int mrep = kMrep);
 hipError_t launch_stem_l1(int dtype, const ConvParams& p, hipStream_t st);
 size_t stem_l1_lds_bytes(int dtype);
 void stem_l1_tile(int* th, int* tw);
@@ -337,7 +341,7 @@
                               void* scratch, hipStream_t st);
 
 void choose_conv_cfg(int dtype, const ConvRow& r, bool conv0, int max_batch, ConvCfg& c,
-                     int th = 0, int tw = 0, int wn = 0, int nrep = 0, bool allow_pk = true);
+                     int th = 0, int tw = 0, int wn = 0, int nrep = 0, bool allow_pk = true, int mrep = kMrep);
 void pack_conv(int dtype, const ConvRow& r, bool conv0, const ConvCfg& c, const float* w, const float* b,
                uint8_t* dst_w, float* dst_b, int cin_off = 0, float* alpha = nullptr);
 size_t packed_conv_bytes(const ConvRow& r, bool conv0, const ConvCfg& c);
diff --git a/vision-textile-inspection_amd/engine.py b/vision-textile-inspection_amd/engine.py
--- a/vision-textile-inspection_amd/engine.py
+++ b/vision-textile-inspection_amd/engine.py
@@ -72,7 +72,7 @@
             out.append(dict(name=info.name.decode(), c1=info.c1, c2=info.c2, k=info.k, s=info.s, kind=info.kind,
                             h_in=info.h_in, w_in=info.w_in, h_out=info.h_out, w_out=info.w_out, macs=info.macs,
                             tile=(info.tile_h, info.tile_w), waves_n=info.waves_n, nrep=info.nrep, lds=info.lds_bytes,
-                            fused=bool(info.fused), persistent=bool(info.persistent)))
+                            fused=bool(info.fused), persistent=bool(info.persistent), mrep=info.mrep, threads=info.threads))
         return out
 
     @property
@@ -838,3 +838,22 @@
     if rc != 0:
         raise _lib.VtiError(rc, lib().vti_last_error(None).decode())
     return out, ms.value, dict(tile=(cfg[0], cfg[1]), waves_n=cfg[2], nrep=cfg[3], lds=abs(cfg[4]), pk=cfg[4] < 0)
+
+
+def debug_tower2d(x, w1, b1, w2, b2, dtype="h2", in_coff=0, c1=None, out_coff=0, out_ld=None, act2=2, mrep=0):
+    B, H, W, ld = x.shape
+    w1 = np.ascontiguousarray(to_numpy(w1), dtype=np.float32)
+    b1 = np.ascontiguousarray(to_numpy(b1), dtype=np.float32)
+    w2 = np.ascontiguousarray(to_numpy(w2), dtype=np.float32).reshape(len(b2), -1)
+    b2 = np.ascontiguousarray(to_numpy(b2), dtype=np.float32)
+    c_mid, c2 = w1.shape[0], w2.shape[0]
+    c1 = c1 or w1.shape[1]
+    out_ld = out_ld or (out_coff + c2)
+    out = torch.zeros((B, H, W, out_ld), dtype=torch.float32, device=x.device)
+    cfg = (C.c_int32 * 5)()
+    vp = lambda a: a.ctypes.data_as(C.c_void_p)
+    rc = lib().vti_debug_tower2d(DTYPES[dtype], _ptr(x), B, H, W, ld, in_coff, c1, vp(w1), vp(b1), c_mid, vp(w2), vp(b2), c2, act2,
+                                 _ptr(out), out_ld, out_coff, mrep, cfg, _stream())
+    if rc != 0:
+        raise _lib.VtiError(rc, lib().vti_last_error(None).decode())
+    return out, dict(tile=(cfg[0], cfg[1]), mrep=cfg[2], threads=cfg[3], lds=cfg[4])
```

Result: slower. 16020 (-1.3%).
